# PolyU-IOR/HPR-LP-C

Hardware: AMD Instinct MI355X
Metric: HPR iterations/sec (FP64) (higher is better)
Workload: dtype f64

## Files before the change

### hpr-lp-c_amd/csrc/abi.cpp

```cpp
#include <algorithm>
#include <cmath>
#include <cstdlib>
#include <cstring>
#include <memory>
#include <mutex>
#include <iomanip>
#include <iostream>

#include "hprlp_amd.h"
#include "env.h"
#include "dist.h"
#include "presolve.h"
#include "reorder.h"
#include "solver.h"
#include "version.h"

using namespace hprlp;

struct hprlp_solver {
    Solver s;
    Comm *comm = nullptr;
    Comm *xcomm = nullptr;
    bool sharded = false;
    ~hprlp_solver() {}
// ... 1037 lines not shown
            out[3] = st.clusters; out[4] = st.components; out[5] = st.seconds;
        }
        return 0;
    } catch (const std::exception &e) {
        set_last_error(e.what());
        return -1;
    }
}

extern "C" int hprlp_row_block_plan(int m, int n, const int *rowptr, const int *col, int with_cuts, long out[6]) {
    try {
        if (m <= 0 || n <= 0 || !rowptr || !col || !out) throw std::runtime_error("bad arguments");
        row_block_plan_host(m, n, rowptr, col, with_cuts != 0, out);
        return 0;
    } catch (const std::exception &e) {
        set_last_error(e.what());
        return -1;
    }
}

extern "C" int hprlp_solver_get_scalars(hprlp_solver *h, double out[16]) {
    GUARD_BEGIN
    Solver &s = h->s;
    Ctrl ck;
    HIP_CHECK(hipStreamSynchronize(s.stream));
    HIP_CHECK(hipMemcpy(&ck, s.ctrl.p, sizeof(Ctrl), hipMemcpyDeviceToHost));
    const double v[16] = {s.b_scale, s.c_scale, s.norm_b, s.norm_c, s.norm_b_org, s.norm_c_org, s.sigma, s.lambda_max,
                          s.setup_time, s.scaling_time, s.power_time, static_cast<double>(s.power_iters),
                          static_cast<double>(ck.kx), static_cast<double>(ck.ky), 0, 0};
    for (int i = 0; i < 16; ++i) out[i] = v[i];
    return 0;
    GUARD_END(-1)
}

extern "C" int hprlp_solver_info(hprlp_solver *h, long out[8]) {
    GUARD_BEGIN
    Solver &s = h->s;
    s.finish_tiling();
    out[0] = s.m; out[1] = s.n; out[2] = s.A.view.nnz;
    out[3] = s.A.view.nblk; out[4] = s.AT.view.nblk;
    out[5] = s.A.view.grid(); out[6] = s.AT.view.grid();
    out[7] = (s.A.view.tiled.valid ? 1 : 0) + (s.AT.view.tiled.valid ? 2 : 0) + (s.use_small && !s.comm ? 4 : 0) + (s.perm_r.empty() ? 0 : 8);
    return 0;
    GUARD_END(-1)
}

extern "C" int hprlp_solver_set_detection(hprlp_solver *h, const hprlp_detection *det) {
    GUARD_BEGIN
    if (!h) throw std::runtime_error("null solver");
    if (h->sharded && det)
        throw std::runtime_error("hprlp_solver_set_detection: infeasibility detection runs on one GPU only; a sharded solver "
                                 "(hprlp_solver_create_dist* / _local*) refuses it");
    Detection d;
    detection_from(det, &d);
    h->s.detect = d;
    return 0;
    GUARD_END(-1)
}

extern "C" int hprlp_solver_set_start(hprlp_solver *h, const double *x0, const double *y0) {
    GUARD_BEGIN
    if (!h) throw std::runtime_error("null solver");
    if (h->sharded)
        throw std::runtime_error("hprlp_solver_set_start: warm start runs on one GPU only; a sharded solver (hprlp_solver_create_dist* / "
                                 "_local*) refuses it");
    check_start(x0, h->s.n, "x0");
    check_start(y0, h->s.m, "y0");
    h->s.set_start(x0, y0);
    return 0;
    GUARD_END(-1)
}

extern "C" int hprlp_solver_set_data(hprlp_solver *h, const double *c, const double *obj_constant, const double *AL, const double *AU,
                                     const double *l, const double *u) {
    GUARD_BEGIN
    if (!h) throw std::runtime_error("null solver");
    if (h->sharded)
        throw std::runtime_error("hprlp_solver_set_data: new data for a resident model runs on one GPU only; a sharded solver "
                                 "(hprlp_solver_create_dist* / _local*) refuses it");
    h->s.set_data(c, obj_constant, AL, AU, l, u);
    return 0;
    GUARD_END(-1)
}

extern "C" int hprlp_solver_resolve(hprlp_solver *h, double sigma, const double *x0, const double *y0, HPRLP_results *out,
                                    hprlp_trace_row *trace, int max_trace, int *n_trace) {
    GUARD_BEGIN
    if (!h || !out) throw std::runtime_error("null solver / result");
    if (h->sharded)
        throw std::runtime_error("hprlp_solver_resolve: a re-solve runs on one GPU only; a sharded solver (hprlp_solver_create_dist* / "
                                 "_local*) refuses it");
    if (std::isnan(sigma)) throw std::runtime_error("hprlp_solver_resolve: sigma is NaN");
    check_start(x0, h->s.n, "x0");
    check_start(y0, h->s.m, "y0");
    Solver &s = h->s;
    s.trace = reinterpret_cast<TraceRow *>(trace);
    s.trace_cap = trace ? max_trace : 0;
    try {
        s.resolve(sigma, x0, y0, out);
    } catch (...) {
        s.trace = nullptr;
        s.trace_cap = 0;
        throw;
    }
    if (n_trace) *n_trace = s.trace_n;
    s.trace = nullptr;
    s.trace_cap = 0;
    return 0;
    GUARD_END(-1)
}

extern "C" int hprlp_solver_data_seconds(hprlp_solver *h, double out[3]) {
    GUARD_BEGIN
    if (!h || !out) throw std::runtime_error("null solver / output");
    for (int i = 0; i < 3; ++i) out[i] = h->s.data_time[i];
    return 0;
    GUARD_END(-1)
}

extern "C" int hprlp_solver_get_certificate(hprlp_solver *h, hprlp_certificate *cert) {
    GUARD_BEGIN
    if (!h || !cert) throw std::runtime_error("null solver / certificate");
    if (!export_certificate(h->s.cert, cert, h->s.m, h->s.n)) throw std::runtime_error("host allocation of the certificate failed");
    return 0;
    GUARD_END(-1)
}

extern "C" int hprlp_solver_describe(hprlp_solver *h, char *buf, int cap) {
    GUARD_BEGIN
    if (!h || !buf || cap <= 0) throw std::runtime_error("null solver / buffer");
    Solver &s = h->s;
    s.finish_tiling();
    auto one = [](const char *name, const DeviceMatrix &M) {
        const TiledDev &t = M.view.tiled;
        std::string d = std::string(name) + ": ";
        if (!t.valid) {
            d += "stream kernel (k_spmv_fused, " + std::to_string(M.view.nblk) + " row blocks, " + std::to_string(M.view.nlong) + " split rows)";
            d += no_tiled_note(M.outcome.why);
            return d;
        }
        d += t.n_pieces > 0 ? "tiled, piece form (k_tiled_part + k_tiled_finish, " + std::to_string(t.n_pieces) + " pieces)"
             : t.rem_cap == kPbRemCap ? "tiled, all-remainder form (k_pb_fused, grid " + std::to_string(t.grid) + ")"
                                      : "tiled, fused (k_tiled_fused, grid " + std::to_string(t.grid) + ")";
        d += ", " + std::to_string(t.nsb) + " super-blocks, " + std::to_string(M.tiled.n_steps) + " steps";
        if (t.R != kTileRows || t.T != kTileCols) d += " (" + std::to_string(t.R) + " rows, tiles of " + std::to_string(t.T) + " columns)";
        const double all = static_cast<double>(M.tiled.dense_entries) + static_cast<double>(M.tiled.n_rem);
        if (all > 0) d += ", " + std::to_string(static_cast<int>(100.0 * M.tiled.dense_entries / all + 0.5)) + " % of the entries in staged tiles";
        if (t.f_rk) d += ", source-side run tables";
        if (t.f_work) d += ", pre-pass work list of " + std::to_string(t.n_work) + " workgroups for " + std::to_string(t.n_groups) + " source groups";
        if (t.side_nblk > 0) d += ", long rows aside (" + std::to_string(t.side_nblk) + " blocks through the stream kernel)";
        return d;
    };
    std::string d = one("A", s.A) + "; " + one("A^T", s.AT);
    if (s.use_small && !s.comm) d += "; normal iterations in the single-workgroup kernel (k_small_iterations)";
    if (!s.perm_r.empty()) d += "; locality ordering applied at set-up";
    if (!s.env_at_setup.empty()) d += "; switches: " + s.env_at_setup;
    if (!s.env_ignored_at_setup.empty()) d += "; ignored without HPRLP_TEST_HOOKS=1: " + s.env_ignored_at_setup;
    std::snprintf(buf, static_cast<size_t>(cap), "%s", d.c_str());
    return static_cast<int>(d.size());
    GUARD_END(-1)
}

extern "C" int hprlp_form_select(const hprlp_form_facts *facts, const hprlp_form_hooks *hooks, hprlp_form_decision *out) {
    try {
        if (!facts || !out) throw std::runtime_error("bad arguments");
        const char *missing = "";
        if (!form_select(*facts, hooks ? *hooks : FormHooks(), out, &missing))
            throw std::runtime_error(std::string("the rules ask for a fact that the record marks as not measured: ") + missing);
        return 0;
    } catch (const std::exception &e) {
        set_last_error(e.what());
        return -1;
    }
}

extern "C" int hprlp_solver_form_facts(hprlp_solver *h, int which, hprlp_form_facts out[2]) {
    GUARD_BEGIN
    if (!h || !out || which < 0 || which > 1) throw std::runtime_error("null solver / buffer, or no such matrix");
    h->s.finish_tiling();
    const DeviceMatrix &M = which ? h->s.AT : h->s.A;
    out[0] = M.facts;
    out[1] = M.facts_pb;
    return M.passes;
    GUARD_END(-1)
}

extern "C" int hprlp_tiled_host_check(int m, int n, const int *rowptr, const int *col, int R, int T, double min_dense, long out[6]) {
    try {
        if (m <= 0 || n <= 0 || !rowptr || !col || !out) throw std::runtime_error("bad arguments");
        tiled_host_check(m, n, rowptr, col, R, T, min_dense, out);
        return 0;
    } catch (const std::exception &e) {
        set_last_error(e.what());
        return -1;
    }
}

extern "C" int hprlp_env_switches(char *buf, int cap) {
    int count = 0;
    const EnvEntry *t = env_table(&count);
    std::string d;
    for (int i = 0; i < count; ++i) d += std::string(t[i].name) + "\t" + (t[i].kind == EnvKind::Integrator ? "integrator" : "hook") + "\t" + t[i].what + "\n";
    if (buf && cap > 0) std::snprintf(buf, static_cast<size_t>(cap), "%s", d.c_str());
    return static_cast<int>(d.size());
}

extern "C" int hprlp_solver_time_iterations(hprlp_solver *h, int warmup, int steps, int mode, double *total_ms,
                                            double *xhalf_ms, double *yhalf_ms) {
    GUARD_BEGIN
    Solver &s = h->s;
    if (steps <= 0) throw std::runtime_error("steps must be positive");
    s.run_normal(warmup);
    HIP_CHECK(hipStreamSynchronize(s.stream));
    hipEvent_t e0, e1;
    HIP_CHECK(hipEventCreate(&e0));
    HIP_CHECK(hipEventCreate(&e1));
    double tx = 0, ty = 0;
    float ms = 0;
    if (mode == 0) {
        HIP_CHECK(hipEventRecord(e0, s.stream));
        s.run_normal(steps);
        HIP_CHECK(hipEventRecord(e1, s.stream));
        HIP_CHECK(hipEventSynchronize(e1));
        HIP_CHECK(hipEventElapsedTime(&ms, e0, e1));
    } else if (mode == 2) {
        s.invalidate_far();
        std::vector<hipEvent_t> ev(static_cast<size_t>(steps) * 3);
        for (auto &e : ev) HIP_CHECK(hipEventCreate(&e));
        HIP_CHECK(hipEventRecord(e0, s.stream));
        for (int i = 0; i < steps; ++i) {
            HIP_CHECK(hipEventRecord(ev[3 * i], s.stream));
            launch_spmv_plain(s.AT.view, s.gy.p, s.sn1.p, nullptr, false, nullptr, 0, s.stream);
            HIP_CHECK(hipEventRecord(ev[3 * i + 1], s.stream));
            launch_spmv_plain(s.A.view, s.gxh.p, s.sm1.p, nullptr, false, nullptr, 0, s.stream);
            HIP_CHECK(hipEventRecord(ev[3 * i + 2], s.stream));
        }
        HIP_CHECK(hipEventRecord(e1, s.stream));
        HIP_CHECK(hipEventSynchronize(e1));
        HIP_CHECK(hipEventElapsedTime(&ms, e0, e1));
        for (int i = 0; i < steps; ++i) {
            float a = 0, b = 0;
            HIP_CHECK(hipEventElapsedTime(&a, ev[3 * i], ev[3 * i + 1]));
            HIP_CHECK(hipEventElapsedTime(&b, ev[3 * i + 1], ev[3 * i + 2]));
            tx += a;
            ty += b;
        }
        for (auto &e : ev) (void)hipEventDestroy(e);
    } else {
        std::vector<hipEvent_t> ev(static_cast<size_t>(steps) * 3);
        for (auto &e : ev) HIP_CHECK(hipEventCreate(&e));
        HIP_CHECK(hipEventRecord(e0, s.stream));
        for (int i = 0; i < steps; ++i) s.launch_normal_pair(i + 1 < steps, &ev[3 * static_cast<size_t>(i)], s.x_mode_of(i, steps));
        HIP_CHECK(hipEventRecord(e1, s.stream));
        HIP_CHECK(hipEventSynchronize(e1));
        HIP_CHECK(hipEventElapsedTime(&ms, e0, e1));
        for (int i = 0; i < steps; ++i) {
            float a = 0, b = 0;
            HIP_CHECK(hipEventElapsedTime(&a, ev[3 * i], ev[3 * i + 1]));
            HIP_CHECK(hipEventElapsedTime(&b, ev[3 * i + 1], ev[3 * i + 2]));
            tx += a;
            ty += b;
        }
        for (auto &e : ev) (void)hipEventDestroy(e);
    }
    (void)hipEventDestroy(e0);
    (void)hipEventDestroy(e1);
    if (total_ms) *total_ms = ms;
    if (xhalf_ms) *xhalf_ms = tx;
    if (yhalf_ms) *yhalf_ms = ty;
    return 0;
    GUARD_END(-1)
}
```

### hpr-lp-c_amd/csrc/env.cpp

```cpp
#include "env.h"

#include <cstdlib>
#include <cstring>
#include <stdexcept>

namespace hprlp {

static const EnvEntry kTable[] = {
    {"HPRLP_TEST_HOOKS", EnvKind::Integrator, "1: honour the test hooks below (tests/conftest.py and the tools/ scripts set it)"},
    {"HPRLP_TIMING", EnvKind::Integrator, "wall time of the set-up and solve phases on stderr"},
    {"HPRLP_NO_GRAPH", EnvKind::Integrator, "launch normal iterations eagerly instead of replaying hipGraphs (fall-back)"},
    {"HPRLP_NO_TILED", EnvKind::Integrator, "never build the column-tiled matrix copies: stream kernel everywhere (fall-back)"},
    {"HPRLP_NO_REORDER", EnvKind::Integrator, "no set-up time locality ordering of a large matrix"},
    {"HPRLP_NO_ALLOC_CACHE", EnvKind::Integrator, "do not keep freed device blocks for the next solver of the process"},
    {"HPRLP_DIST_TRANSPORT", EnvKind::Integrator, "shm: hprlp_dist_unique_id names a shared-memory segment (host-staged group of processes on one node) instead of RCCL ids"},
    {"HPRLP_NO_WARM_MODEL", EnvKind::Integrator, "the model constructors do NOT start the HIP runtime / device context / code objects (for a process that forks workers after building its models: a HIP context does not survive fork); the first solve pays for them as in the reference"},
    {"HPRLP_DIST_EXCHANGE", EnvKind::Hook, "sparse | allgather: force the multi-GPU exchange form (same value on every rank)"},
    {"HPRLP_NO_OVERLAP", EnvKind::Integrator, "multi-GPU: shards unsplit, exchange in line on the solver stream"},
    {"HPRLP_DIST_TIMEOUT_S", EnvKind::Integrator, "seconds a rank of the shared-memory transport waits for its peers before it fails (default 120)"},
    {"HPRLP_BATCH_CHUNK", EnvKind::Hook, "solve_batched with 64 or more problems: chunk width of the panels (default 64; narrower chunks map one chunk to each XCD -- measured slower, profiles/r03_tiled_decomposition.md section 6b)"},
    {"HPRLP_BATCH_GRID", EnvKind::Hook, "solve_batched: cap on the row blocks of the normal half-step kernels (read at every call; a small cap makes every workgroup's row loop wrap)"},
    {"HPRLP_BATCH_LAMBDA", EnvKind::Hook, "solve_batched: the batch's lambda_max from the caller (strtod; hand it over as a C99 hex float to keep every bit) instead of 1.01 x the power iteration's estimate (read at every call)"},
    {"HPRLP_COPY_PAUSE_US", EnvKind::Hook, "piece size and pause of the threaded copies of set-up (64 MB, 100 us)"},
    {"HPRLP_COPY_PIECE_MB", EnvKind::Hook, "piece size and pause of the threaded copies of set-up (64 MB, 100 us)"},
    {"HPRLP_DEVICE_TRANSPOSE_MIN", EnvKind::Hook, "build Aᵀ on the host / nonzero threshold of the device transpose (default 4 M)"},
    {"HPRLP_DIST_SELFTEST_FAIL", EnvKind::Hook, "tests only: the set-up self-test of the neighbour exchange reports a failure once (exercises the fall-back to the all-gather)"},
    {"HPRLP_DTON_MAX", EnvKind::Hook, "presolve: cap of the doubleton stage"},
    {"HPRLP_DTON_TRACE", EnvKind::Hook, "presolve: trace the doubleton stage on stderr"},
    {"HPRLP_GEN_FAR", EnvKind::Hook, "benchmark generator: share of a row's entries that fall anywhere (default 0.05)"},
    {"HPRLP_HOST_POWER_START", EnvKind::Hook, "power iteration's start vector made on the host also above 1e6 rows (default there: on the device)"},
    {"HPRLP_HOST_TILING", EnvKind::Hook, "build the tiled copies with the host builder (background threads, default min(16, cores)) instead of on the device"},
    {"HPRLP_HOST_TRANSPOSE", EnvKind::Hook, "build Aᵀ on the host / nonzero threshold of the device transpose (default 4 M)"},
    {"HPRLP_NO_BOUND_CODES", EnvKind::Hook, "the x-half always reads l[j] and u[j], the y-half AL[i] and AU[i] (default: one code byte per column / row says which of them is not a constant; an equality row reads one value)"},
    {"HPRLP_NO_FAR_PUSH", EnvKind::Hook, "always run the remainder pre-pass (k_far_products) instead of the hand-off from the producing half-step's epilogue"},
    {"HPRLP_NO_FAR_WORK", EnvKind::Hook, "the remainder pre-pass with one workgroup per source group also where one group holds several times the mean (default: a work list cuts heavy groups into chunks, tiled.h f_work)"},
    {"HPRLP_NO_PB_LONG_ROWS", EnvKind::Hook, "a matrix kept off the tiled forms for its long rows keeps the stream kernel also where its columns are not popular (default: all-remainder form, Solver::pb_fallback_wanted)"},
    {"HPRLP_NO_FUSED_NORMS", EnvKind::Hook, "the Ruiz row norms by their own passes instead of as a by-product of the preceding scaling pass (same bits)"},
    {"HPRLP_NO_LONG_SIDE", EnvKind::Hook, "a matrix with rows over 1024 entries keeps the stream kernel instead of being tiled with those rows kept aside"},
    {"HPRLP_NO_PB_FALLBACK", EnvKind::Hook, "unstructured large matrices keep the stream kernel instead of the tiled form without dense-tile requirement"},
    {"HPRLP_NO_PB_KERNEL", EnvKind::Hook, "run an all-remainder copy through k_tiled_fused's remainder steps instead of k_pb_fused (A/B)"},
    {"HPRLP_NO_REM2", EnvKind::Hook, "tiled build: no second remainder level"},
    {"HPRLP_NO_SETUP_OVERLAP", EnvKind::Hook, "set-up of a large model in line: no helper threads / copy streams for the value upload, the row blocks, A^T's row pointers and the model vectors (same bits either way)"},
    {"HPRLP_NO_SLAB_CUTS", EnvKind::Hook, "dense rows of a large matrix are not cut at the XCD eighths of the gathered vector (stream kernel)"},
    {"HPRLP_NO_SMALL", EnvKind::Hook, "do not use the single-workgroup kernel for Netlib-scale LPs"},
    {"HPRLP_NO_SMALL_POWER", EnvKind::Hook, "Netlib-scale LPs: power iteration by the regular kernels with the host test every 10th iteration (default: one launch of the single-workgroup kernel)"},
    {"HPRLP_NO_TILED_CR", EnvKind::Hook, "Curtis-Reid passes through the stream kernel also for matrices with a tiled copy (default: tiled kernel on a second value array of -log|a|)"},
    {"HPRLP_NT", EnvKind::Hook, "force default / nontemporal loads of the matrix in the stream kernel"},
    {"HPRLP_OVERLAP_COMM_FIRST", EnvKind::Hook, "tests only: with the in-process rank group, use RCCL's launch order (exchange enqueued before the local SpMV)"},
    {"HPRLP_PB_MIN_COLS", EnvKind::Hook, "gathered-vector length from which an unstructured matrix takes the all-remainder form (default 800 k columns, the crossover measured with k_pb_fused)"},
    {"HPRLP_PB_MIN_NNZ", EnvKind::Hook, "fewest entries for the all-remainder form"},
    {"HPRLP_PB_STAMPS", EnvKind::Hook, "developer build -DHPRLP_PB_PHASE_STAMPS=1: print k_pb_fused's phase times"},
    {"HPRLP_PIECES_ANYWAY", EnvKind::Hook, "attempt the tiled form although neighbouring rows gather from the same lines (<= 0.25 lines per entry) / keep the piece form although an XCD's rows gather from under 3 MB"},
    {"HPRLP_PRESOLVE_MAX_LINKS", EnvKind::Hook, "run one presolve stage alone / cut the chain after n links (tests, debugging)"},
    {"HPRLP_PRESOLVE_OFF", EnvKind::Hook, "switch presolve reductions / stages off (any subset; diagnostics)"},
    {"HPRLP_PRESOLVE_ONLY", EnvKind::Hook, "run one presolve stage alone / cut the chain after n links (tests, debugging)"},
    {"HPRLP_REORDER_CLUSTER", EnvKind::Hook, "knobs of the HOST reference path of the ordering (hprlp_locality_ordering): nodes per cluster, refinement sweeps, trimming percentage"},
    {"HPRLP_REORDER_HOST", EnvKind::Hook, "run the clustering of the locality ordering on the host (the reference form; default: on the device)"},
    {"HPRLP_REORDER_SWEEPS", EnvKind::Hook, "knobs of the HOST reference path of the ordering (hprlp_locality_ordering): nodes per cluster, refinement sweeps, trimming percentage"},
    {"HPRLP_REORDER_TRIM", EnvKind::Hook, "knobs of the HOST reference path of the ordering (hprlp_locality_ordering): nodes per cluster, refinement sweeps, trimming percentage"},
    {"HPRLP_SLACK_PIVOT", EnvKind::Hook, "pivot threshold of the costed slack-column substitution (default 0.5 of the row's largest entry)"},
    {"HPRLP_STORE_X", EnvKind::Hook, "every normal x-half reads and stores x (default for matrices with a tiled copy: inside a run of normal iterations x is rebuilt from x_hat and last_x by the next launch instead of travelling through memory)"},
    {"HPRLP_STREAM_NNZ", EnvKind::Hook, "row-block shape of the stream kernel (≤ 64 rows, ≤ 512 nonzeros per wave)"},
    {"HPRLP_STREAM_ROWS", EnvKind::Hook, "row-block shape of the stream kernel (≤ 64 rows, ≤ 512 nonzeros per wave)"},
    {"HPRLP_TILED_ANYWAY", EnvKind::Hook, "attempt the tiled form although neighbouring rows gather from the same lines (<= 0.25 lines per entry) / keep the piece form although an XCD's rows gather from under 3 MB"},
    {"HPRLP_TILED_MIN_COLS", EnvKind::Hook, "fewest columns for the tiled form (default 800 k, 2^19 for lowered super-blocks; 0 when HPRLP_TILED_MIN_ROWS is given)"},
    {"HPRLP_TILED_MIN_DENSE", EnvKind::Hook, "thresholds of the tiled copy (default 32·8192 rows, 0.5 of the entries in staged tiles)"},
    {"HPRLP_TILED_MIN_ROWS", EnvKind::Hook, "thresholds of the tiled copy (default 32·8192 rows, 0.5 of the entries in staged tiles)"},
    {"HPRLP_TILE_COLS", EnvKind::Hook, "force the tile width / super-block height of the tiled copies (default: Solver::choose_sb_rows)"},
    {"HPRLP_TILE_PIECES", EnvKind::Hook, "piece count of the tiled kernel's piece form (default: the chip's workgroup slots when the matrix has at most that many super-blocks; 0 = off)"},
    {"HPRLP_TILE_ROT", EnvKind::Hook, "alignment period of the rotated tile sweeps (default: mean window width of the matrix; 0 = ascending sweeps, i.e. CSR summation order)"},
    {"HPRLP_TILE_ROWS", EnvKind::Hook, "force the tile width / super-block height of the tiled copies (default: Solver::choose_sb_rows)"},
    {"HPRLP_TILE_STAMPS", EnvKind::Hook, "diagnostic instantiation of the piece kernel: shader-clock time per phase of a step on stderr when the solver is destroyed"},
    {"HPRLP_TILE_THREADS", EnvKind::Hook, "build the tiled copies with the host builder (background threads, default min(16, cores)) instead of on the device"},
    {"HPRLP_TILING_CHECK", EnvKind::Hook, "build them with both builders and fail on the first differing array element"},
    {"HPRLP_WG_TIMES", EnvKind::Hook, "diagnostic: per-workgroup wall-clock stamps of the fused tiled kernel on stderr"},
    {"HPRLP_WG_TIMES_DUMP", EnvKind::Hook, "per-workgroup stamps of the normal half-step kernels only, with the CU each ran on; raw table for tools/wgtimes_analyze.py"},
};

const EnvEntry *env_table(int *count) {
    if (count) *count = static_cast<int>(sizeof(kTable) / sizeof(kTable[0]));
    return kTable;
}

static bool hooks_on() {
    const char *h = std::getenv("HPRLP_TEST_HOOKS");
    return h && h[0] == '1';
}

const char *env_get(const char *name) {
    for (const EnvEntry &e : kTable) {
        if (std::strcmp(e.name, name) != 0) continue;
        if (e.kind == EnvKind::Hook && !hooks_on()) return nullptr;
        return std::getenv(name);
    }
    throw std::logic_error(std::string("environment switch missing from env.cpp's table: ") + name);
}

std::string env_in_effect(std::string *ignored_out) {
    std::string on, off;
    const bool hooks = hooks_on();
    for (const EnvEntry &e : kTable) {
        const char *v = std::getenv(e.name);
        if (!v || std::strcmp(e.name, "HPRLP_TEST_HOOKS") == 0) continue;
        std::string &dst = (e.kind == EnvKind::Hook && !hooks) ? off : on;
        if (!dst.empty()) dst += ' ';
        dst += std::string(e.name) + "=" + v;
    }
    if (ignored_out) *ignored_out = off;
    return on;
}

}
```

### hpr-lp-c_amd/csrc/kernels.h

```cpp
#pragma once

#include <hip/hip_runtime.h>

#include "tiled.h"

namespace hprlp {

constexpr int kWave = 64;
constexpr int kWavesPerBlock = 4;
constexpr int kThreads = kWave * kWavesPerBlock;
constexpr int kStreamW = 512;
constexpr int kStreamRows = 64;
constexpr int kLongRow = 64;
constexpr int kSplitRow = 4096;
constexpr int kNumScalars = 32;

enum Slot : int {
    S_CX = 0,
    S_YOBJ_Y = 1,
    S_XZ = 2,
    S_RD2 = 3,
    S_RP2 = 4,
    S_ADX_DY = 5,
    S_DY2 = 6,
    S_DX2 = 7,
    S_MOVE_X2 = 8,
    S_MOVE_Y2 = 9,
    S_LU2 = 10,
    S_PW_ZZ = 11,
    S_PW_QZ = 12,
    S_PW_ERR2 = 13,
    S_NB2 = 14,
    S_NC2 = 15,
    S_TMP0 = 16,
    S_TMP1 = 17,
    S_SMALL_PW_LAMBDA = 18,
    S_SMALL_PW_ITERS = 19,
    S_RAY_DY = 20,
    S_RAY_CD = 21,
    S_RAY_VY = 22,
    S_RAY_WD = 23,
    S_RAY_YN = 24,
    S_RAY_DN = 25,
    S_RAY_DZ = 26,
    S_RAY_VZ = 27,
    S_RAY_WQ = 28,
    S_DATA_B_ORG = 20,
    S_DATA_C_ORG = 21,
    S_DATA_B_PRE = 22,
    S_DATA_C_PRE = 23,
    S_DATA_NB = 24,
    S_DATA_NC = 25,
};

struct CsrDev {
    int rows = 0, cols = 0;
    int nnz = 0;
    int nt = 1;
    const int *rowptr = nullptr;
    const int *col = nullptr;
    double *val = nullptr;
    const int4 *blk = nullptr;
    int nblk = 0;
    TiledDev tiled;
    const int4 *longrows = nullptr;
    int nlong = 0;
    double *long_partial = nullptr;
    int csr_grid() const { return (nblk + kWavesPerBlock - 1) / kWavesPerBlock; }
    int finish_grid() const { return (nlong + kThreads - 1) / kThreads; }
    int tiled_finish_grid() const { return (rows + kThreads - 1) / kThreads; }
    int grid() const { return tiled.valid ? (tiled.n_pieces > 0 ? tiled_finish_grid() : tiled.grid) : csr_grid() + finish_grid(); }
};

struct Ctrl {
    double sigma, lam_sigma, inv_lam_sigma, inv_sigma;
    int kx, ky;
    int pad0, pad1;
};

struct FarPush {
    const int *gptr = nullptr;
    const double *val = nullptr;
    const int *pos = nullptr;
    const uint16_t *lcol = nullptr;
    double *P = nullptr;
    const int *rptr = nullptr, *rk = nullptr, *rp = nullptr;
};

struct XHalfArgs {
    const double *y_full;
    double *x, *x_hat;
    const double *l, *u, *c, *last_x;
    double *x_bar, *z_bar, *x_temp;
    Ctrl *ctrl;
    double *partials;
    int stride;
    FarPush push;
    bool far_ready = false;
    const unsigned char *lu_code = nullptr;
    int x_mode = 0;
};
constexpr int kXRebuild = 1, kXNoStore = 2;
constexpr unsigned kLoadL = 1u, kLoadU = 2u, kZeroL = 4u;
void launch_bound_codes(int n, const double *l, const double *u, unsigned char *code, hipStream_t s);

struct YHalfArgs {
    const double *xhat_full;
    double *y;
    const double *AL, *AU, *last_y;
    double *y_bar, *y_obj, *y_temp;
    Ctrl *ctrl;
    double *partials;
    int stride;
    FarPush push;
    bool far_ready = false;
    const unsigned char *row_code = nullptr;
};
constexpr unsigned kLoadLo = 1u, kLoadHi = 2u, kRowEq = 4u;
void launch_row_codes(int m, const double *AL, const double *AU, unsigned char *code, hipStream_t s);

struct FinalizeItem {
    const double *partials;
    int count;
    int slot;
    int max = 0;
};
struct FinalizeArgs {
    FinalizeItem item[8];
    int n;
};

bool launch_x_half(const CsrDev &AT, const XHalfArgs &a, bool check, hipStream_t s);
bool launch_y_half(const CsrDev &A, const YHalfArgs &a, bool check, hipStream_t s);
FarPush far_push_of(const CsrDev &consumer);
void launch_x_half_base(const CsrDev &AT_remote, const XHalfArgs &a, const double *base, hipStream_t s);
void launch_y_half_base(const CsrDev &A_remote, const YHalfArgs &a, const double *base, hipStream_t s);

void launch_resid_d(const CsrDev &AT, const double *ybar_full, const double *c, const double *z_bar,
                    const double *col_norm, double *partials, hipStream_t s);
void launch_resid_p(const CsrDev &A, const double *xbar_full, const double *xtemp_full, const double *AL,
                    const double *AU, const double *row_norm, const double *y_temp, bool with_gap,
                    double *partials, int stride, hipStream_t s);
void launch_gap(const CsrDev &A, const double *xtemp_full, const double *y_temp, double *partials, hipStream_t s);
bool launch_spmv_push(const CsrDev &M, const double *v_full, double *out, const FarPush &push, hipStream_t s);
void launch_spmv_plain(const CsrDev &M, const double *v_full, double *out, const double *q, bool with_dots,
                       double *partials, int stride, hipStream_t s, bool far_ready = false);

void launch_finalize(const FinalizeArgs &f, double *scalars, hipStream_t s);

constexpr int kRayFormAccs = 6;
struct RayFormArgs {
    int n, m;
    const double *x_bar, *y_bar;
    double *prev_x, *prev_y, *ds, *ys;
    const double *l, *u, *c, *col_norm, *AL, *AU, *row_norm;
    double b_scale, c_scale;
};
void launch_ray_form(const RayFormArgs &a, double *partials, int nblocks, hipStream_t s);
void launch_ray_col(const CsrDev &AT, const double *ys_full, const double *l, const double *u, const double *col_norm, double b_scale,
                    double c_scale, double *partials, hipStream_t s);
void launch_ray_row(const CsrDev &A, const double *ds_full, const double *AL, const double *AU, const double *row_norm, double b_scale,
                    double *partials, hipStream_t s);

struct StartInArgs {
    int n, m;
    const double *x0, *y0;
    const int *pc, *pr;
    const double *l, *u, *col_norm, *AL, *AU, *row_norm;
    double b_scale, c_scale;
    double *x, *last_x, *x_hat, *x_bar, *y, *last_y, *y_bar;
};
void launch_start_in(const StartInArgs &a, hipStream_t s);
void launch_start_col(const CsrDev &AT, const double *ybar_full, const double *c, const double *l, const double *u,
                      const double *x_bar, double *z_bar, double *partials, hipStream_t s);
void launch_start_row(const CsrDev &A, const double *xbar_full, const double *AL, const double *AU, const double *y_bar,
                      double *y_obj, double *partials, hipStream_t s);

void launch_movement(int n, int m, const double *x_bar, const double *last_x, double *x_temp, const double *y_bar,
                     const double *last_y, double *y_temp, double *partials, int stride, int nblocks, hipStream_t s);
void launch_restart_copy(int n, int m, const double *x_bar, double *x, double *last_x, const double *y_bar,
                         double *y, double *last_y, Ctrl *ctrl, hipStream_t s);
void launch_lu(int n, const double *x_bar, const double *l, const double *u, const double *col_norm, double *x_temp,
               double *partials, int nblocks, hipStream_t s);
void launch_set_ctrl(Ctrl *ctrl, double sigma, double lambda_max, int reset_k, hipStream_t s);

void launch_cr_log_update(const CsrDev &M, const double *other_full, double *result, hipStream_t s, const double *tval_log = nullptr,
                          const double *fval_log = nullptr);
bool cr_runs_tiled(const CsrDev &M);
void launch_exp_clamp(double *v, int n, hipStream_t s);
void launch_row_norm(const CsrDev &M, double *result, int norm, hipStream_t s);
double launch_line_density(const int *rowptr, const int *col, int rows, hipStream_t s);
int launch_longest_row(const int *rowptr, int rows, hipStream_t s, int limit = 0, long *entries_in_long = nullptr);
int launch_heaviest_block(const int *rowptr, int rows, int height, hipStream_t s);
void launch_scale_matrix(const CsrDev &M, const double *rowvec, const double *colvec_full, bool row_first,
                         bool divide, hipStream_t s, double *next_max_norm = nullptr);
void launch_vec_scale(double *x, const double *s, int n, bool divide, hipStream_t s_);
void launch_vec_scal(double *x, double a, int n, hipStream_t s);
void launch_fill(double *x, double a, int n, hipStream_t s);
void launch_bnorm2(const double *AL, const double *AU, int m, double *partials, int nblocks, hipStream_t s);
void launch_norm2(const double *x, int n, double *partials, int nblocks, hipStream_t s);

void launch_check_columns(long nnz, int cols, const int *col, int *bad, hipStream_t s);
void launch_pw_start(int m, unsigned long long seed, long long offset, double *z, hipStream_t s);
void launch_pw_normalize(const double *z, double *q, int m, const double *scalars, hipStream_t s);
void launch_pw_err(const double *z, const double *q, int m, const double *scalars, double *partials, int nblocks,
                   hipStream_t s);

struct DataInArgs {
    int m, nc, nb;
    const double *AL_in, *AU_in, *c_in, *l_in, *u_in;
    const int *pc, *pr;
    const double *row_norm, *col_norm;
    double *AL, *AU, *c, *l, *u;
    double *partials;
    int stride;
};
void launch_data_in(const DataInArgs &a, hipStream_t s);
struct DataBcArgs {
    int m, nc, nb;
    int use_bc;
    const double *scalars;
    double *AL, *AU, *c, *l, *u;
    unsigned char *row_code, *lu_code;
    double *partials;
    int stride;
};
void launch_data_bc(const DataBcArgs &a, hipStream_t s);

void launch_unscale(int n, int m, const double *x_bar, const double *y_bar, const double *z_bar,
                    const double *col_norm, const double *row_norm, double b_scale, double c_scale, double *xo,
                    double *yo, double *zo, hipStream_t s);

constexpr int kSmallMaxK = 12;
constexpr int kSmallMaxR = 2;
constexpr int kSmallMaxRow = 256;
struct SmallArgs {
    int m, n, nnz;
    const int *A_rowptr, *AT_rowptr;
    const double *AT_val;
    const int *ent_ij;
    const int *ent_posA;
    const int *order_x, *order_y;
    double *x, *x_hat, *y;
    const double *l, *u, *c, *last_x, *AL, *AU, *last_y;
    Ctrl *ctrl;
};
bool small_path_fits(int m, int n, long nnz, int max_row_A, int max_row_AT);
void launch_small_iterations(const SmallArgs &a, int count, hipStream_t s);
void launch_small_power(const SmallArgs &a, const double *z0, int max_iter, double tol, double *out, hipStream_t s);

void device_transpose(int rows, int cols, long nnz, const int *rowptr, const int *col, const double *val, int *trp,
                      int *tci, double *tv, hipStream_t s);

void device_split_columns(int rows, long nnz, const int *rowptr, const int *col, const double *val, int lo, int hi, DBuf<int> &rp_loc,
                          DBuf<int> &col_loc, DBuf<double> &val_loc, DBuf<int> &rp_rem, DBuf<int> &col_rem, DBuf<double> &val_rem,
                          hipStream_t s);

void launch_pack(const double *src, const int *idx, double *dst, int n, hipStream_t s);
void launch_scatter(double *dst, const int *idx, const double *src, int n, hipStream_t s);

constexpr int kReduceBlocks = 512;

}
```

### hpr-lp-c_amd/csrc/kernels.hip

```cpp
#include "kernels.h"

#include <algorithm>
#include <vector>
#include <cmath>
#include <type_traits>

namespace hprlp {

__device__ __forceinline__ double wave_sum(double v) {
#pragma unroll
    for (int off = 32; off > 0; off >>= 1) v += __shfl_xor(v, off, kWave);
    return v;
}

__device__ __forceinline__ double wave_max(double v) {
#pragma unroll
    for (int off = 32; off > 0; off >>= 1) v = fmax(v, __shfl_xor(v, off, kWave));
    return v;
}

template <int NACC, int NW, int NMAX = 0>
__device__ __forceinline__ void block_store_partials_in(double (&acc)[NACC], double *partials, int stride, double (*red)[NACC > 0 ? NACC : 1]) {
    const int wave = threadIdx.x >> 6, lane = threadIdx.x & 63;
#pragma unroll
// ... 442 lines not shown
            const int el = tid + k * NT;
            if (el < cnt) prod[el] = pv[k];
        }
        uint32_t code[K];
        {
            const int shift = K * tid - min(K * tid, max(cnt - K, 0));
#pragma unroll
            for (int u = 0; u < K; ++u) code[u] = cv[u];
            if (shift > 0 && shift < K) {
#pragma unroll
                for (int u = 0; u < K; ++u) {
                    uint32_t c = 0;
#pragma unroll
                    for (int q = 0; q < K; ++q) c = (q == u + shift) ? cv[q] : c;
                    code[u] = c;
                }
            }
        }
        if (s + 1 < s1) issue(nxt);
        lds_barrier();
        const int nv = min(max(cnt - K * tid, 0), K);
        uint32_t row[K];
        double pr[K];
#pragma unroll
        for (int u = 0; u < K; ++u) {
            const bool ok = u < nv;
            row[u] = ok ? (code[u] & 0xffffu) : (u == 0 ? NOROW : row[u - 1]);
            pr[u] = ok ? prod[code[u] >> 16] : 0.0;
        }
        double run = pr[0], head = 0.0;
        bool single = true;
#pragma unroll
        for (int u = 1; u < K; ++u) {
            if (row[u] != row[u - 1]) {
                if (single) {
                    head = run;
                    single = false;
                } else {
                    acc[row[u - 1]] += run;
                }
                run = pr[u];
            } else {
                run += pr[u];
            }
        }
        const uint32_t rf = row[0], rl = row[K - 1];
        const uint32_t rl_prev = __shfl_up(rl, 1, 64);
        const bool open_in = lane > 0 && rf == rl_prev && rf != NOROW;
        double v = run;
        int f = (single && open_in) ? 0 : 1;
#pragma unroll
        for (int off = 1; off < 64; off <<= 1) {
            const double vu = __shfl_up(v, off, 64);
            const int fu = __shfl_up(f, off, 64);
            if (lane >= off && !f) {
                v += vu;
                f |= fu;
            }
        }
        const double v_prev = __shfl_up(v, 1, 64);
        const double carry = open_in ? v_prev : 0.0;
        const int next_open = __shfl_down(static_cast<int>(open_in), 1, 64);
        if (!single) acc[rf] += carry + head;
        const double tail = single ? carry + run : run;
        if (lane == 63) {
            bnd_row[wave] = rl;
            bnd_val[wave] = tail;
        } else if (!next_open && rl != NOROW) {
            acc[rl] += tail;
        }
        lds_barrier();
        if (tid < NW) {
            const uint32_t rw = bnd_row[tid];
            bool last_one = rw != NOROW;
            double tot = 0.0;
#pragma unroll
            for (int w = 0; w < NW; ++w) {
                const bool same = bnd_row[w] == rw;
                if (w <= tid && same) tot += bnd_val[w];
                if (w > tid && same) last_one = false;
            }
            if (last_one) acc[rw] += tot;
        }
        st = nxt;
    }
}

template <class Epi, bool PUSH>
__device__ __forceinline__ void epilogue_rows(const Epi &epi, double *acc, double (&racc)[Epi::NACC > 0 ? Epi::NACC : 1], int r0, int nr, int tid) {
    constexpr int NT = kTileThreads, B = 4;
    for (int i0 = tid; i0 < nr; i0 += B * NT) {
        typename Epi::Row rw[B];
        double sv[B][1];
#pragma unroll
        for (int u = 0; u < B; ++u) {
            const int i = min(i0 + u * NT, nr - 1);
            rw[u] = epi.load_row(r0 + i);
            sv[u][0] = acc[i];
        }
#pragma unroll
        for (int u = 0; u < B; ++u) {
            const int i = i0 + u * NT;
            if (i < nr) {
                if constexpr (PUSH) acc[i] = epi.apply(r0 + i, rw[u], sv[u], racc);
                else epi.apply(r0 + i, rw[u], sv[u], racc);
            }
        }
    }
}

__device__ __forceinline__ void push_products(const FarPush &f, const double *vals, int pb, int pe, int tid) {
    constexpr int NT = kTileThreads, U = 4;
    if (pb >= pe) return;
    double a4[U];
    int p4[U];
    uint16_t c4[U];
    auto load_batch = [&](int k0) {
#pragma unroll
        for (int u = 0; u < U; ++u) {
            const int z = min(k0 + u * NT, pe - 1);
            a4[u] = __builtin_nontemporal_load(f.val + z);
            p4[u] = __builtin_nontemporal_load(f.pos + z);
            c4[u] = __builtin_nontemporal_load(f.lcol + z);
        }
    };
    int k = pb + tid;
    load_batch(k);
    for (; k < pe; k += U * NT) {
        double prd[U];
        int ps[U];
#pragma unroll
        for (int u = 0; u < U; ++u) {
            prd[u] = a4[u] * vals[c4[u]];
            ps[u] = p4[u];
        }
        const int kn = k + U * NT;
        if (kn < pe) load_batch(kn);
#pragma unroll
        for (int u = 0; u < U; ++u)
            if (k + u * NT < pe) f.P[ps[u]] = prd[u];
    }
}

__device__ __forceinline__ int run_position(const int *tab_k, const int *tab_p, int nr, int k) {
    int lo = 0, hi = nr - 1;
    while (lo < hi) {
        const int mid = (lo + hi + 1) >> 1;
        if (tab_k[mid] <= k) lo = mid;
        else hi = mid - 1;
    }
    return tab_p[lo] + (k - tab_k[lo]);
}

__device__ __forceinline__ void push_products_runs(const FarPush &f, const double *vals, int *tab, int g, int pb, int pe, int tid) {
    constexpr int NT = kTileThreads, U = 4;
    if (pb >= pe) return;
    const int r0 = f.rptr[g], nr = f.rptr[g + 1] - r0;
    int *tab_k = tab, *tab_p = tab + kPbRunTabCap;
    double a4[U];
    uint16_t c4[U];
    auto load_batch = [&](int k0) {
#pragma unroll
        for (int u = 0; u < U; ++u) {
            const int z = min(k0 + u * NT, pe - 1);
            a4[u] = __builtin_nontemporal_load(f.val + z);
            c4[u] = __builtin_nontemporal_load(f.lcol + z);
        }
    };
    int k = pb + tid;
    load_batch(k);
    for (int i = tid; i < nr; i += NT) {
        tab_k[i] = f.rk[r0 + i];
        tab_p[i] = f.rp[r0 + i];
    }
    lds_barrier();
    int ps[U];
#pragma unroll
    for (int u = 0; u < U; ++u) ps[u] = run_position(tab_k, tab_p, nr, min(k + u * NT, pe - 1));
    for (; k < pe; k += U * NT) {
        double prd[U];
        int pc[U];
#pragma unroll
        for (int u = 0; u < U; ++u) {
            prd[u] = a4[u] * vals[c4[u]];
            pc[u] = ps[u];
        }
        const int kn = k + U * NT;
        if (kn < pe) load_batch(kn);
#pragma unroll
        for (int u = 0; u < U; ++u)
            if (k + u * NT < pe) f.P[pc[u]] = prd[u];
        if (kn < pe) {
#pragma unroll
            for (int u = 0; u < U; ++u) ps[u] = run_position(tab_k, tab_p, nr, min(kn + u * NT, pe - 1));
        }
    }
}

template <class Epi, bool REP, bool PUSH = false, bool NARROW = false>
__global__ void __launch_bounds__(kTileThreads, 4) k_tiled_fused(CsrDev A, Epi epi) {
    static_assert(Epi::NV == 1, "the tiled kernel stages one gathered vector");
    constexpr int NT = kTileThreads, RMAX = kTileRows, T = kTileCols;
    constexpr int NACC = Epi::NACC;
    __shared__ double acc[RMAX];
    __shared__ __attribute__((aligned(16))) double ytile[T];
    const TiledDev &t = A.tiled;
    const int tid = threadIdx.x;
    const int R = t.R;
    const int per = t.per, slots = gridDim.x / 8;
    const int slot = blockIdx.x / 8;
    double racc[NACC > 0 ? NACC : 1];
#pragma unroll
    for (int i = 0; i < (NACC > 0 ? NACC : 1); ++i) racc[i] = 0.0;
    epi.begin();
    int wg_round = 0;
    const bool wg_stamp = t.wgtimes && tid == 0 && (t.wg_filter == 0 || (PUSH && NACC == 0));
    if (wg_stamp) t.wgtimes[blockIdx.x * 8] = wall_clock64();
    for (int q = slot; q < per; q += slots) {
        const int sb = (blockIdx.x % 8) * per + q;
        if (sb >= t.nsb) break;
        const double *__restrict__ vec = epi.gv[0];
        lds_barrier();
        const int ncols = A.cols;
        for (int i = tid; i < R; i += NT) acc[i] = 0.0;
        const int s0 = t.sb_ptr[sb], smid = t.sb_mid[sb], s1 = t.sb_ptr[sb + 1];
        if (s0 < smid) tiled_sweep<HPRLP_SWEEP_ED, HPRLP_SWEEP_TD, REP, false, LogTerm<Epi>::value, NARROW ? kTileColsNarrow : kTileCols>(t, s0, smid - s0, t.steps[s0].rot, smid - s0, vec, ncols, acc, ytile, tid);
        remainder_steps<kTileRemK>(t, smid, s1, acc, ytile, ytile + kTileRemCap, tid);
        lds_barrier();
        const int r0 = sb * R;
        const int nr = min(R, A.rows - r0);
        int pb = 0, pe = 0;
        if constexpr (PUSH) {
            pb = epi.push.gptr[sb];
            pe = epi.push.gptr[sb + 1];
        }
        epilogue_rows<Epi, PUSH>(epi, acc, racc, r0, nr, tid);
        if constexpr (PUSH) {
            lds_barrier();
            push_products(epi.push, acc, pb, pe, tid);
        }
        if (wg_stamp && ++wg_round <= 5) t.wgtimes[blockIdx.x * 8 + wg_round] = wall_clock64();
    }
    if (wg_stamp) {
        t.wgtimes[blockIdx.x * 8 + 7] = wall_clock64();
        const unsigned hw = __builtin_amdgcn_s_getreg((31 << 11) | 4), xcc = __builtin_amdgcn_s_getreg((31 << 11) | 20);
        t.wgtimes[blockIdx.x * 8 + 6] = (static_cast<unsigned long long>(xcc & 0xfu) << 32) | hw;
    }
    if constexpr (NACC > 0) {
        __syncthreads();
        block_store_partials_in<NACC, kTileThreads / kWave, MaxAccs<Epi>::value>(racc, epi.partials, epi.stride, reinterpret_cast<double(*)[NACC]>(ytile));
    }
}

template <class Epi, bool PUSH = false>
__global__ void __launch_bounds__(kTileThreads, 4) k_pb_fused(CsrDev A, Epi epi) {
    static_assert(Epi::NV == 1, "one gathered vector");
    constexpr int NT = kTileThreads, K = kPbRemK, CAP = kPbRemCap, NW = kTileThreads / 64;
    constexpr int NACC = Epi::NACC;
    __shared__ double acc[kPbRowsMax];
    __shared__ __attribute__((aligned(16))) double prod[CAP];
    __shared__ double bnd[3 * NW];
    const TiledDev &t = A.tiled;
    const int tid = threadIdx.x;
    const int R = t.R;
    const int per = t.per, slots = gridDim.x / 8;
    const int slot = blockIdx.x / 8;
    double racc[NACC > 0 ? NACC : 1];
#pragma unroll
    for (int i = 0; i < (NACC > 0 ? NACC : 1); ++i) racc[i] = 0.0;
    epi.begin();
#if HPRLP_PB_PHASE_STAMPS
    unsigned long long ph[8] = {0, 0, 0, 0, 0, 0, 0, 0}, tq = wall_clock64(), tk0 = tq;
#define PB_STAMP(i) do { const unsigned long long now_ = wall_clock64(); ph[i] += now_ - tq; tq = now_; } while (0)
#else
#define PB_STAMP(i) do { } while (0)
#endif
    for (int q = slot; q < per; q += slots) {
        const int sb = (blockIdx.x % 8) * per + q;
        if (sb >= t.nsb) break;
        lds_barrier();
        for (int i = tid; i < R; i += NT) acc[i] = 0.0;
        const int smid = t.sb_mid[sb], s1 = t.sb_ptr[sb + 1];
        remainder_steps<K>(t, smid, s1, acc, prod, bnd, tid);
        lds_barrier();
        PB_STAMP(4);
        const int r0 = sb * R;
        const int nr = min(R, A.rows - r0);
        int pb = 0, pe = 0;
        if constexpr (PUSH) {
            pb = epi.push.gptr[sb];
            pe = epi.push.gptr[sb + 1];
        }
        epilogue_rows<Epi, PUSH>(epi, acc, racc, r0, nr, tid);
        PB_STAMP(5);
        if constexpr (PUSH) {
            lds_barrier();
            if (epi.push.rk) push_products_runs(epi.push, acc, reinterpret_cast<int *>(prod), sb, pb, pe, tid);
            else push_products(epi.push, acc, pb, pe, tid);
        }
        PB_STAMP(6);
    }
#if HPRLP_PB_PHASE_STAMPS
    if (t.wgtimes && tid == 0 && PUSH && NACC == 0) {
        ph[7] = wall_clock64() - tk0;
        for (int i = 0; i < 8; ++i) t.wgtimes[blockIdx.x * 8 + i] = ph[i];
    }
#endif
#undef PB_STAMP
    if constexpr (NACC > 0) {
        __syncthreads();
        block_store_partials_in<NACC, kTileThreads / kWave, MaxAccs<Epi>::value>(racc, epi.partials, epi.stride, reinterpret_cast<double(*)[NACC]>(prod));
    }
}

template <bool REP, bool STAMP = false, bool NARROW = false>
__global__ void __launch_bounds__(kTileThreads, 4) k_tiled_part(CsrDev A, const double *__restrict__ vec) {
    constexpr int NT = kTileThreads, RMAX = kTileRows, T = kTileCols;
    __shared__ double acc[RMAX];
    __shared__ __attribute__((aligned(16))) double ytile[T];
    const TiledDev &t = A.tiled;
    const int tid = threadIdx.x;
    const int R = t.R;
    const int per = (t.n_pieces + 7) / 8;
    const int pc = (blockIdx.x % 8) * per + blockIdx.x / 8;
    if (pc >= t.n_pieces) return;
    for (int sg = t.piece_ptr[pc]; sg < t.piece_ptr[pc + 1]; ++sg) {
        const int4 d = t.segs[sg];
        const int sb = d.x;
        lds_barrier();
        for (int i = tid; i < R; i += NT) acc[i] = 0.0;
        const int s0 = t.sb_ptr[sb], smid = t.sb_mid[sb], s1 = t.sb_ptr[sb + 1];
        unsigned long long *st = STAMP ? t.stamps + static_cast<size_t>(pc) * 16 : nullptr;
        unsigned long long c0 = 0, c1 = 0, c2 = 0;
        if (STAMP) c0 = __builtin_amdgcn_s_memtime();
        if (d.z > 0) tiled_sweep<3, 2, REP, STAMP, false, NARROW ? kTileColsNarrow : kTileCols>(t, s0, smid - s0, d.y, d.z, vec, A.cols, acc, ytile, tid, st);
        if (STAMP) c1 = __builtin_amdgcn_s_memtime();
        if (d.w) remainder_steps<kTileRemK>(t, smid, s1, acc, ytile, ytile + kTileRemCap, tid);
        lds_barrier();
        if (STAMP) c2 = __builtin_amdgcn_s_memtime();
        double *out = t.parts + static_cast<size_t>(sg) * R;
        for (int i = tid; i < R; i += NT) out[i] = acc[i];
        if (STAMP && tid == 0) {
            st[8] += c1 - c0;
            st[9] += c2 - c1;
            st[10] += __builtin_amdgcn_s_memtime() - c2;
        }
    }
}

template <class Epi>
__global__ void __launch_bounds__(kThreads) k_tiled_finish(CsrDev A, Epi epi) {
    constexpr int NACC = Epi::NACC;
    const int R = A.tiled.R;
    double racc[NACC > 0 ? NACC : 1];
#pragma unroll
    for (int i = 0; i < (NACC > 0 ? NACC : 1); ++i) racc[i] = 0.0;
    epi.begin();
    const int r = blockIdx.x * kThreads + threadIdx.x;
    if (r < A.rows) {
        const int sb = r / R;
        const int a = A.tiled.slot_ptr[sb], b = A.tiled.slot_ptr[sb + 1];
        const double *p = A.tiled.parts + (r - sb * R);
        double sum = 0.0;
        for (int k = a; k < b; ++k) sum = (k == a) ? p[static_cast<size_t>(k) * R] : sum + p[static_cast<size_t>(k) * R];
        const double sv[1] = {sum};
        typename Epi::Row rw = epi.load_row(r);
        epi.apply(r, rw, sv, racc);
    }
    if constexpr (NACC > 0) block_store_partials<NACC, kWavesPerBlock, MaxAccs<Epi>::value>(racc, epi.partials, epi.stride);
}

__global__ void __launch_bounds__(kThreads) k_tiled_refresh(long n, const int *perm, const double *csr_val, double *out) {
    const long i = static_cast<long>(blockIdx.x) * kThreads + threadIdx.x;
    if (i < n) {
        const int p = perm[i];
        out[i] = p >= 0 ? csr_val[p] : 0.0;
    }
}

void launch_tiled_refresh(const DeviceTiled &t, const double *csr_val, hipStream_t s) {
    if (t.n_tile > 0)
        hipLaunchKernelGGL(k_tiled_refresh, dim3(static_cast<unsigned>((t.n_tile + kThreads - 1) / kThreads)), dim3(kThreads), 0, s,
                           t.n_tile, t.tperm.p, csr_val, t.tval.p);
    if (t.n_rem > 0 && t.f_val.p)
        hipLaunchKernelGGL(k_tiled_refresh, dim3(static_cast<unsigned>((t.n_rem + kThreads - 1) / kThreads)), dim3(kThreads), 0, s,
                           t.n_rem, t.f_perm.p, csr_val, t.f_val.p);
}

__global__ void __launch_bounds__(kThreads) k_tiled_refresh_log(long n, const int *perm, const double *csr_val, double *out) {
    const long i = static_cast<long>(blockIdx.x) * kThreads + threadIdx.x;
    if (i < n) {
        const int p = perm[i];
        out[i] = p >= 0 ? -log(fmax(fabs(csr_val[p]), 1e-300)) : __builtin_nan("");
    }
}

void launch_tiled_refresh_log(const DeviceTiled &t, const double *csr_val, double *tval_log, double *fval_log, hipStream_t s) {
    if (t.n_tile > 0)
        hipLaunchKernelGGL(k_tiled_refresh_log, dim3(static_cast<unsigned>((t.n_tile + kThreads - 1) / kThreads)), dim3(kThreads), 0, s,
                           t.n_tile, t.tperm.p, csr_val, tval_log);
    if (t.n_rem > 0 && t.f_val.p)
        hipLaunchKernelGGL(k_tiled_refresh_log, dim3(static_cast<unsigned>((t.n_rem + kThreads - 1) / kThreads)), dim3(kThreads), 0, s,
                           t.n_rem, t.f_perm.p, csr_val, fval_log);
}

__device__ __forceinline__ bool far_work_item(const TiledDev &t, int &g, int &b, int &e) {
    const int items = t.f_work ? t.n_work : t.n_groups;
    const int per = (items + 7) / 8;
    const int w = (blockIdx.x % 8) * per + blockIdx.x / 8;
    if (w >= items) return false;
    if (t.f_work) {
        const int4 d = t.f_work[w];
        g = d.x; b = d.y; e = d.z;
    } else {
        g = w; b = t.f_gptr[w]; e = t.f_gptr[w + 1];
    }
    return b < e;
}

template <bool LOGTERM = false>
__global__ void __launch_bounds__(kFarThreads) k_far_products(TiledDev t, const double *__restrict__ vec, int ncols) {
    __shared__ double v[kFarGroup];
    const int G = t.G;
    int g, b, e;
    if (!far_work_item(t, g, b, e)) return;
    const int c0 = g * G, tid = threadIdx.x;
    const int w = min(G, ncols - c0);
    constexpr int U = 4;
    double a[U];
    int pos[U];
    uint16_t lc[U];
    int k = b + tid;
    auto load_batch = [&](int k0) {
#pragma unroll
        for (int u = 0; u < U; ++u) {
            const int q = min(k0 + u * kFarThreads, e - 1);
            a[u] = __builtin_nontemporal_load(t.f_val + q);
            pos[u] = __builtin_nontemporal_load(t.f_pos + q);
            lc[u] = __builtin_nontemporal_load(t.f_lcol + q);
        }
    };
    load_batch(k);
    {
        constexpr int S = kFarGroup / kFarThreads;
        double sv[S];
#pragma unroll
        for (int i = 0; i < S; ++i)
            if (i * kFarThreads < G) sv[i] = vec[c0 + min(tid + i * kFarThreads, w - 1)];
#pragma unroll
        for (int i = 0; i < S; ++i)
            if (i * kFarThreads < G) v[tid + i * kFarThreads] = sv[i];
    }
    __syncthreads();
    for (; k < e; k += U * kFarThreads) {
        double pr[U];
        int ps[U];
#pragma unroll
        for (int u = 0; u < U; ++u) {
            pr[u] = LOGTERM ? a[u] - v[lc[u]] : a[u] * v[lc[u]];
            ps[u] = pos[u];
        }
        const int kn = k + U * kFarThreads;
        if (kn < e) load_batch(kn);
#pragma unroll
        for (int u = 0; u < U; ++u)
            if (k + u * kFarThreads < e) t.P[ps[u]] = pr[u];
    }
}

template <bool LOGTERM = false>
__global__ void __launch_bounds__(kFarThreads) k_far_products_runs(TiledDev t, const double *__restrict__ vec, int ncols) {
    __shared__ double v[kPbRowsMax];
    __shared__ int tab[2 * kPbRunTabCap];
    const int G = t.G;
    int g, b, e;
    if (!far_work_item(t, g, b, e)) return;
    const int c0 = g * G, tid = threadIdx.x;
    const int w = min(G, ncols - c0);
    const int r0 = t.f_rptr[g], nr = t.f_rptr[g + 1] - r0;
    int *tab_k = tab, *tab_p = tab + kPbRunTabCap;
    constexpr int U = 4;
    double a[U];
    uint16_t lc[U];
    int k = b + tid;
    auto load_batch = [&](int k0) {
#pragma unroll
        for (int u = 0; u < U; ++u) {
            const int q = min(k0 + u * kFarThreads, e - 1);
            a[u] = __builtin_nontemporal_load(t.f_val + q);
            lc[u] = __builtin_nontemporal_load(t.f_lcol + q);
        }
    };
    load_batch(k);
    for (int i = tid; i < G; i += kFarThreads) v[i] = vec[c0 + min(i, w - 1)];
    for (int i = tid; i < nr; i += kFarThreads) {
        tab_k[i] = t.f_rk[r0 + i];
        tab_p[i] = t.f_rp[r0 + i];
    }
    __syncthreads();
    int ps[U];
#pragma unroll
    for (int u = 0; u < U; ++u) ps[u] = run_position(tab_k, tab_p, nr, min(k + u * kFarThreads, e - 1));
    for (; k < e; k += U * kFarThreads) {
        double pr[U];
        int pc[U];
#pragma unroll
        for (int u = 0; u < U; ++u) {
            pr[u] = LOGTERM ? a[u] - v[lc[u]] : a[u] * v[lc[u]];
            pc[u] = ps[u];
        }
        const int kn = k + U * kFarThreads;
        if (kn < e) load_batch(kn);
#pragma unroll
        for (int u = 0; u < U; ++u)
            if (k + u * kFarThreads < e) t.P[pc[u]] = pr[u];
        if (kn < e) {
#pragma unroll
            for (int u = 0; u < U; ++u) ps[u] = run_position(tab_k, tab_p, nr, min(kn + u * kFarThreads, e - 1));
        }
    }
}

template <bool LOGTERM>
static void launch_far_products(const TiledDev &t, const double *vec, int ncols, hipStream_t s) {
    const dim3 grid(((t.f_work ? t.n_work : t.n_groups) + 7) / 8 * 8);
    if (t.f_rk && t.G <= kPbRowsMax) hipLaunchKernelGGL(k_far_products_runs<LOGTERM>, grid, dim3(kFarThreads), 0, s, t, vec, ncols);
    else hipLaunchKernelGGL(k_far_products<LOGTERM>, grid, dim3(kFarThreads), 0, s, t, vec, ncols);
}


template <bool CHECK, bool STREAMED = false>
struct XEpi {
    static constexpr int NV = 1;
    static constexpr int NACC = CHECK ? 3 : 0;
    const double *gv[1];
    double *x, *x_hat;
    const double *l, *u, *c, *last_x;
    double *x_bar, *z_bar, *x_temp;
    Ctrl *ctrl;
    double *partials;
    int stride;
    double sigma, f1, f2;
    FarPush push;
    const unsigned char *lu_code;
    int x_mode;
    double f1p, f2p;
    static constexpr bool kPublishes = true;
    static constexpr bool kSkipsX = !CHECK && STREAMED;
    struct Row {
        double xi, ci, li, ui, lx;
    };
    __device__ __forceinline__ void begin() {
        const int k = ctrl->kx;
        sigma = ctrl->sigma;
        f1 = 1.0 / (static_cast<double>(k) + 2.0);
        f2 = 1.0 - f1;
        f1p = 1.0 / (static_cast<double>(k - 1) + 2.0);
        f2p = 1.0 - f1p;
        if (blockIdx.x == 0 && threadIdx.x == 0) ctrl->ky = k;
    }
    __device__ __forceinline__ Row load_row(int r) const {
        constexpr bool NT = STREAMED && HPRLP_EPI_NT >= 1;
        auto ld = [](const double *p) { return NT ? __builtin_nontemporal_load(p) : *p; };
        double li, ui;
        if (lu_code) {
            const unsigned cd = NT ? __builtin_nontemporal_load(lu_code + r) : lu_code[r];
            li = (cd & kLoadL) ? ld(l + r) : ((cd & kZeroL) ? 0.0 : -__builtin_huge_val());
            ui = (cd & kLoadU) ? ld(u + r) : __builtin_huge_val();
        } else {
            li = ld(l + r);
            ui = ld(u + r);
        }
        const double lx = ld(last_x + r);
        if constexpr (kSkipsX) {
            if (x_mode & kXRebuild) return Row{f2p * ld(x_hat + r) + f1p * lx, ld(c + r), li, ui, lx};
        }
        return Row{ld(x + r), ld(c + r), li, ui, lx};
    }
    __device__ __forceinline__ double apply(int r, const Row &w, const double (&s)[1], double (&acc)[CHECK ? 3 : 1]) const {
        const double gc = s[0] - w.ci;
        const double zt = w.xi + sigma * gc;
        const double xb = fmin(w.ui, fmax(w.li, zt));
        const double xh = 2.0 * xb - w.xi;
        const double xn = f2 * xh + f1 * w.lx;
        {
            if constexpr (STREAMED && HPRLP_EPI_NT >= 2) __builtin_nontemporal_store(xh, x_hat + r);
            else x_hat[r] = xh;
            if (!kSkipsX || !(x_mode & kXNoStore)) {
                if constexpr (STREAMED && HPRLP_EPI_NT >= 1) __builtin_nontemporal_store(xn, x + r);
                else x[r] = xn;
            }
        }
        if constexpr (CHECK) {
            const double zb = (xb - zt) / sigma;
            const double dx = xb - xh;
            z_bar[r] = zb;
            x_bar[r] = xb;
            x_temp[r] = dx;
            acc[0] += w.ci * xb;
            acc[1] += xb * zb;
            acc[2] += dx * dx;
        }
        return xh;
    }
};

template <bool CHECK, bool STREAMED = false>
struct YEpi {
    static constexpr int NV = 1;
    static constexpr int NACC = CHECK ? 2 : 0;
    const double *gv[1];
    double *y;
    const double *AL, *AU, *last_y;
    double *y_bar, *y_obj, *y_temp;
    Ctrl *ctrl;
    double *partials;
    int stride;
    double fact1, fact2, hf1, hf2;
    FarPush push;
    const unsigned char *row_code;
    static constexpr bool kPublishes = true;
    struct Row {
        double yi, lo, hi, ly;
    };
    __device__ __forceinline__ void begin() {
        const int k = ctrl->ky;
        fact1 = ctrl->lam_sigma;
        fact2 = ctrl->inv_lam_sigma;
        hf1 = 1.0 / (static_cast<double>(k) + 2.0);
        hf2 = 1.0 - hf1;
        if (blockIdx.x == 0 && threadIdx.x == 0) ctrl->kx = k + 1;
    }
    __device__ __forceinline__ Row load_row(int r) const {
        constexpr bool NT = STREAMED && HPRLP_EPI_NT >= 1;
        auto ld = [](const double *p) { return NT ? __builtin_nontemporal_load(p) : *p; };
        double lo, hi;
        if (row_code) {
            const unsigned cd = NT ? __builtin_nontemporal_load(row_code + r) : row_code[r];
            hi = (cd & kLoadHi) ? ld(AU + r) : __builtin_huge_val();
            lo = (cd & kLoadLo) ? ld(AL + r) : ((cd & kRowEq) ? hi : -__builtin_huge_val());
        } else {
            lo = ld(AL + r);
            hi = ld(AU + r);
        }
        return Row{ld(y + r), lo, hi, ld(last_y + r)};
    }
    __device__ __forceinline__ double apply(int r, const Row &w, const double (&s)[1], double (&acc)[CHECK ? 2 : 1]) const {
        const double v = s[0] - fact1 * w.yi;
        const double d = fmax(w.lo - v, fmin(w.hi - v, 0.0));
        const double yb = fact2 * d;
        const double yh = 2.0 * yb - w.yi;
        const double yn = hf2 * yh + hf1 * w.ly;
        if constexpr (STREAMED && HPRLP_EPI_NT >= 2) __builtin_nontemporal_store(yn, y + r);
        else y[r] = yn;
        if constexpr (CHECK) {
            const double dy = yb - yh;
            const double yo = v + d;
            y_temp[r] = dy;
            y_bar[r] = yb;
            y_obj[r] = yo;
            acc[0] += yo * yb;
            acc[1] += dy * dy;
        }
        return yn;
    }
};

struct RdEpi {
    static constexpr int NV = 1;
    static constexpr int NACC = 1;
    const double *gv[1];
    const double *c, *z_bar, *col_norm;
    double *partials;
    int stride;
    struct Row {
        double ci, zi, cn;
    };
    __device__ __forceinline__ void begin() {}
    __device__ __forceinline__ Row load_row(int r) const { return Row{c[r], z_bar[r], col_norm[r]}; }
    __device__ __forceinline__ void apply(int, const Row &w, const double (&s)[1], double (&acc)[1]) const {
        const double rd = (w.ci - s[0] - w.zi) * w.cn;
        acc[0] += rd * rd;
    }
};

template <bool GAP>
struct RpEpi {
    static constexpr int NV = GAP ? 2 : 1;
    static constexpr int NACC = GAP ? 2 : 1;
    const double *gv[GAP ? 2 : 1];
    const double *AL, *AU, *row_norm, *y_temp;
    double *partials;
    int stride;
    struct Row {
        double lo, hi, rn, dy;
    };
    __device__ __forceinline__ void begin() {}
    __device__ __forceinline__ Row load_row(int r) const {
        return Row{AL[r], AU[r], row_norm[r], GAP ? y_temp[r] : 0.0};
    }
    __device__ __forceinline__ void apply(int, const Row &w, const double (&s)[GAP ? 2 : 1],
                                          double (&acc)[GAP ? 2 : 1]) const {
        const double v = s[0];
        const double rp = fmax(fmin(w.hi - v, 0.0), w.lo - v) * w.rn;
        acc[0] += rp * rp;
        if constexpr (GAP) acc[1] += s[1] * w.dy;
    }
};

struct GapEpi {
    static constexpr int NV = 1;
    static constexpr int NACC = 1;
    const double *gv[1];
    const double *y_temp;
    double *partials;
    int stride;
    struct Row {
        double dy;
    };
    __device__ __forceinline__ void begin() {}
    __device__ __forceinline__ Row load_row(int r) const { return Row{y_temp[r]}; }
// ... 106 lines not shown
        const double z = ((d > 0.0 && isfinite(w.lo)) || (d < 0.0 && isfinite(w.hi))) ? d : 0.0;
        z_bar[r] = z;
        acc[0] += w.ci * w.xb;
        acc[1] += (z > 0.0 ? w.lo : (z < 0.0 ? w.hi : 0.0)) * z;
    }
};

struct StartRowEpi {
    static constexpr int NV = 1;
    static constexpr int NACC = 1;
    const double *gv[1];
    const double *AL, *AU, *y_bar;
    double *y_obj;
    double *partials;
    int stride;
    struct Row {
        double lo, hi, yb;
    };
    __device__ __forceinline__ void begin() {}
    __device__ __forceinline__ Row load_row(int r) const { return Row{AL[r], AU[r], y_bar[r]}; }
    __device__ __forceinline__ void apply(int r, const Row &w, const double (&s)[1], double (&acc)[1]) const {
        const double yo = w.yb > 0.0 ? w.lo : (w.yb < 0.0 ? w.hi : fmin(fmax(s[0], w.lo), w.hi));
        y_obj[r] = yo;
        acc[0] += yo * w.yb;
    }
};

template <class Epi>
__global__ void __launch_bounds__(kThreads) k_long_finish(CsrDev A, Epi epi, int main_grid) {
    constexpr int NV = Epi::NV;
    constexpr int NACC = Epi::NACC;
    double acc[NACC > 0 ? NACC : 1];
#pragma unroll
    for (int i = 0; i < (NACC > 0 ? NACC : 1); ++i) acc[i] = 0.0;
    epi.begin();
    const int i = blockIdx.x * kThreads + threadIdx.x;
    if (i < A.nlong) {
        const int4 d = A.longrows[i];
        double s[NV];
#pragma unroll
        for (int v = 0; v < NV; ++v) s[v] = 0.0;
        for (int c = d.y; c < d.z; ++c) {
#pragma unroll
            for (int v = 0; v < NV; ++v) s[v] += A.long_partial[static_cast<size_t>(c) * 2 + v];
        }
        typename Epi::Row rw = epi.load_row(d.x);
        epi.apply(d.x, rw, s, acc);
    }
    if constexpr (NACC > 0) {
        block_store_partials<NACC, kWavesPerBlock, MaxAccs<Epi>::value>(acc, epi.partials + main_grid, epi.stride);
    }
}

template <class Epi, class = void>
struct Publishes : std::false_type {};
template <class Epi>
struct Publishes<Epi, std::void_t<decltype(Epi::kPublishes)>> : std::true_type {};

template <class Epi>
struct WithBase : Epi {
    const double *base;
    struct Row {
        typename Epi::Row w;
        double b;
    };
    __device__ __forceinline__ Row load_row(int r) const { return Row{Epi::load_row(r), base[r]}; }
    __device__ __forceinline__ auto apply(int r, const Row &w, const double (&s)[1], double (&acc)[Epi::NACC > 0 ? Epi::NACC : 1]) const {
        const double t[1] = {w.b + s[0]};
        return Epi::apply(r, w.w, t, acc);
    }
};

struct SideEpi {
    static constexpr int NV = 1;
    static constexpr int NACC = 0;
    const double *gv[1];
    const int *rows;
    double *base;
    struct Row {};
    __device__ __forceinline__ void begin() {}
    __device__ __forceinline__ Row load_row(int) const { return Row{}; }
    __device__ __forceinline__ void apply(int r, const Row &, const double (&s)[1], double (&)[1]) const { base[rows[r]] = s[0]; }
};

template <class Epi>
static bool launch_tiled(const CsrDev &M, const Epi &e, hipStream_t s, bool far_ready);

template <class Epi>
static bool launch_fused(const CsrDev &M, const Epi &e, hipStream_t s, bool far_ready = false) {
    if (M.nblk <= 0) return false;
    if constexpr (Epi::NV == 1) {
        if (M.tiled.valid) {
            if (M.tiled.side_nblk > 0) {
                CsrDev S = M;
                S.tiled.valid = false;
                S.blk = M.tiled.side_blk;
                S.nblk = M.tiled.side_nblk;
                S.longrows = M.tiled.side_long;
                S.nlong = M.tiled.side_nlong;
                S.long_partial = M.tiled.side_partial;
                SideEpi se{{e.gv[0]}, M.tiled.side_rows, M.tiled.base};
                hipLaunchKernelGGL(k_spmv_fused<SideEpi>, dim3(S.csr_grid()), dim3(kThreads), 0, s, S, se);
                if (S.nlong > 0) hipLaunchKernelGGL(k_long_finish<SideEpi>, dim3(S.finish_grid()), dim3(kThreads), 0, s, S, se, S.csr_grid());
                WithBase<Epi> wb{e, M.tiled.base};
                return launch_tiled(M, wb, s, far_ready);
            }
            return launch_tiled(M, e, s, far_ready);
        }
    }
    hipLaunchKernelGGL(k_spmv_fused<Epi>, dim3(M.csr_grid()), dim3(kThreads), 0, s, M, e);
    if (M.nlong > 0)
        hipLaunchKernelGGL(k_long_finish<Epi>, dim3(M.finish_grid()), dim3(kThreads), 0, s, M, e, M.csr_grid());
    return false;
}

template <class Epi>
static bool launch_tiled(const CsrDev &M, const Epi &e, hipStream_t s, bool far_ready) {
    if (M.tiled.n_groups > 0 && !far_ready)
        launch_far_products<false>(M.tiled, e.gv[0], M.cols, s);
    const bool narrow = M.tiled.T == kTileColsNarrow;
    if (M.tiled.rem_cap == kPbRemCap) {
        if constexpr (Publishes<Epi>::value) {
            if (e.push.gptr) {
                hipLaunchKernelGGL((k_pb_fused<Epi, true>), dim3(M.tiled.grid), dim3(kTileThreads), 0, s, M, e);
                return true;
            }
        }
        hipLaunchKernelGGL((k_pb_fused<Epi, false>), dim3(M.tiled.grid), dim3(kTileThreads), 0, s, M, e);
        return false;
    }
    if (M.tiled.n_pieces > 0) {
        const dim3 grid((M.tiled.n_pieces + 7) / 8 * 8);
        if (narrow) hipLaunchKernelGGL((k_tiled_part<false, false, true>), grid, dim3(kTileThreads), 0, s, M, e.gv[0]);
        else if (M.tiled.stamps) hipLaunchKernelGGL((k_tiled_part<false, true>), grid, dim3(kTileThreads), 0, s, M, e.gv[0]);
        else if (M.tiled.repeats) hipLaunchKernelGGL(k_tiled_part<true>, grid, dim3(kTileThreads), 0, s, M, e.gv[0]);
        else hipLaunchKernelGGL(k_tiled_part<false>, grid, dim3(kTileThreads), 0, s, M, e.gv[0]);
        hipLaunchKernelGGL(k_tiled_finish<Epi>, dim3(M.tiled_finish_grid()), dim3(kThreads), 0, s, M, e);
        return false;
    }
    if constexpr (Publishes<Epi>::value) {
        if (e.push.gptr) {
            if (narrow) hipLaunchKernelGGL((k_tiled_fused<Epi, false, true, true>), dim3(M.tiled.grid), dim3(kTileThreads), 0, s, M, e);
            else if (M.tiled.repeats) hipLaunchKernelGGL((k_tiled_fused<Epi, true, true>), dim3(M.tiled.grid), dim3(kTileThreads), 0, s, M, e);
            else hipLaunchKernelGGL((k_tiled_fused<Epi, false, true>), dim3(M.tiled.grid), dim3(kTileThreads), 0, s, M, e);
            return true;
        }
    }
    if (narrow) hipLaunchKernelGGL((k_tiled_fused<Epi, false, false, true>), dim3(M.tiled.grid), dim3(kTileThreads), 0, s, M, e);
    else if (M.tiled.repeats) hipLaunchKernelGGL((k_tiled_fused<Epi, true>), dim3(M.tiled.grid), dim3(kTileThreads), 0, s, M, e);
    else hipLaunchKernelGGL((k_tiled_fused<Epi, false>), dim3(M.tiled.grid), dim3(kTileThreads), 0, s, M, e);
    return false;
}

FarPush far_push_of(const CsrDev &consumer) {
    FarPush f;
    if (consumer.tiled.valid && consumer.tiled.n_groups > 0) {
        f.gptr = consumer.tiled.f_gptr;
        f.val = consumer.tiled.f_val;
        f.pos = consumer.tiled.f_pos;
        f.lcol = consumer.tiled.f_lcol;
        f.P = consumer.tiled.P;
        if (consumer.tiled.f_rk) {
            f.rptr = consumer.tiled.f_rptr;
            f.rk = consumer.tiled.f_rk;
            f.rp = consumer.tiled.f_rp;
        }
    }
    return f;
}

bool launch_x_half(const CsrDev &AT, const XHalfArgs &a, bool check, hipStream_t s) {
    if (check) {
        XEpi<true> e{{a.y_full}, a.x, a.x_hat, a.l, a.u, a.c, a.last_x, a.x_bar, a.z_bar, a.x_temp, a.ctrl, a.partials, a.stride, 0, 0, 0, a.push, a.lu_code};
        return launch_fused(AT, e, s, a.far_ready);
    }
    if (AT.tiled.valid) {
        XEpi<false, true> e{{a.y_full}, a.x, a.x_hat, a.l, a.u, a.c, a.last_x, nullptr, nullptr, nullptr, a.ctrl, nullptr, 0, 0, 0, 0, a.push, a.lu_code, a.x_mode};
        return launch_fused(AT, e, s, a.far_ready);
    }
    XEpi<false> e{{a.y_full}, a.x, a.x_hat, a.l, a.u, a.c, a.last_x, nullptr, nullptr, nullptr, a.ctrl, nullptr, 0, 0, 0, 0, a.push, a.lu_code};
    return launch_fused(AT, e, s, a.far_ready);
}

bool launch_y_half(const CsrDev &A, const YHalfArgs &a, bool check, hipStream_t s) {
    if (check) {
        YEpi<true> e{{a.xhat_full}, a.y, a.AL, a.AU, a.last_y, a.y_bar, a.y_obj, a.y_temp, a.ctrl, a.partials, a.stride, 0, 0, 0, 0, a.push, a.row_code};
        return launch_fused(A, e, s, a.far_ready);
    }
    if (A.tiled.valid) {
        YEpi<false, true> e{{a.xhat_full}, a.y, a.AL, a.AU, a.last_y, nullptr, nullptr, nullptr, a.ctrl, nullptr, 0, 0, 0, 0, 0, a.push, a.row_code};
        return launch_fused(A, e, s, a.far_ready);
    }
    YEpi<false> e{{a.xhat_full}, a.y, a.AL, a.AU, a.last_y, nullptr, nullptr, nullptr, a.ctrl, nullptr, 0, 0, 0, 0, 0, a.push, a.row_code};
    return launch_fused(A, e, s, a.far_ready);
}


void launch_x_half_base(const CsrDev &AT_remote, const XHalfArgs &a, const double *base, hipStream_t s) {
    WithBase<XEpi<false>> e{{{a.y_full}, a.x, a.x_hat, a.l, a.u, a.c, a.last_x, nullptr, nullptr, nullptr, a.ctrl, nullptr, 0, 0, 0, 0, FarPush{}, a.lu_code}, base};
    launch_fused(AT_remote, e, s);
}

void launch_y_half_base(const CsrDev &A_remote, const YHalfArgs &a, const double *base, hipStream_t s) {
    WithBase<YEpi<false>> e{{{a.xhat_full}, a.y, a.AL, a.AU, a.last_y, nullptr, nullptr, nullptr, a.ctrl, nullptr, 0, 0, 0, 0, 0, FarPush{}}, base};
    launch_fused(A_remote, e, s);
}

void launch_resid_d(const CsrDev &AT, const double *ybar_full, const double *c, const double *z_bar,
                    const double *col_norm, double *partials, hipStream_t s) {
    RdEpi e{{ybar_full}, c, z_bar, col_norm, partials, AT.grid()};
    launch_fused(AT, e, s);
}

void launch_resid_p(const CsrDev &A, const double *xbar_full, const double *xtemp_full, const double *AL,
                    const double *AU, const double *row_norm, const double *y_temp, bool with_gap,
                    double *partials, int stride, hipStream_t s) {
    if (with_gap && A.tiled.valid) {
        RpEpi<false> e{{xbar_full}, AL, AU, row_norm, nullptr, partials, stride};
        launch_fused(A, e, s);
        GapEpi g{{xtemp_full}, y_temp, partials + stride, stride};
        launch_fused(A, g, s);
    } else if (with_gap) {
        RpEpi<true> e{{xbar_full, xtemp_full}, AL, AU, row_norm, y_temp, partials, stride};
        launch_fused(A, e, s);
    } else {
        RpEpi<false> e{{xbar_full}, AL, AU, row_norm, nullptr, partials, stride};
        launch_fused(A, e, s);
    }
}

void launch_gap(const CsrDev &A, const double *xtemp_full, const double *y_temp, double *partials, hipStream_t s) {
    GapEpi e{{xtemp_full}, y_temp, partials, A.grid()};
    launch_fused(A, e, s);
}

bool launch_spmv_push(const CsrDev &M, const double *v_full, double *out, const FarPush &push, hipStream_t s) {
    PlainPushEpi e{{v_full}, out, push};
    return launch_fused(M, e, s);
}

void launch_spmv_plain(const CsrDev &M, const double *v_full, double *out, const double *q, bool with_dots,
                       double *partials, int stride, hipStream_t s, bool far_ready) {
    if (with_dots) {
        PlainEpi<true> e{{v_full}, out, q, partials, stride};
        launch_fused(M, e, s, far_ready);
    } else if (far_ready) {
        PlainEpi<false> e{{v_full}, out, nullptr, nullptr, 0};
        launch_fused(M, e, s, true);
    } else {
        PlainEpi<false> e{{v_full}, out, nullptr, nullptr, 0};
        launch_fused(M, e, s);
    }
}

void launch_ray_col(const CsrDev &AT, const double *ys_full, const double *l, const double *u, const double *col_norm, double b_scale,
                    double c_scale, double *partials, hipStream_t s) {
    RayColEpi e{{ys_full}, l, u, col_norm, b_scale, c_scale, partials, AT.grid()};
    launch_fused(AT, e, s);
}

void launch_ray_row(const CsrDev &A, const double *ds_full, const double *AL, const double *AU, const double *row_norm, double b_scale,
                    double *partials, hipStream_t s) {
    RayRowEpi e{{ds_full}, AL, AU, row_norm, b_scale, partials, A.grid()};
    launch_fused(A, e, s);
}

void launch_start_col(const CsrDev &AT, const double *ybar_full, const double *c, const double *l, const double *u,
                      const double *x_bar, double *z_bar, double *partials, hipStream_t s) {
    StartColEpi e{{ybar_full}, c, l, u, x_bar, z_bar, partials, AT.grid()};
    launch_fused(AT, e, s);
}

void launch_start_row(const CsrDev &A, const double *xbar_full, const double *AL, const double *AU, const double *y_bar,
                      double *y_obj, double *partials, hipStream_t s) {
    StartRowEpi e{{xbar_full}, AL, AU, y_bar, y_obj, partials, A.grid()};
    launch_fused(A, e, s);
}

static_assert(kWavesPerBlock == 4, "k_finalize's sum adds the four waves' partials in a fixed order");
__global__ void __launch_bounds__(kThreads) k_finalize(FinalizeArgs f, double *scalars) {
    const FinalizeItem it = f.item[blockIdx.x];
    __shared__ double red[kWavesPerBlock];
    if (it.max) {
        double v = 0.0;
        for (int i = threadIdx.x; i < it.count; i += kThreads) v = fmax(v, it.partials[i]);
        v = wave_max(v);
        if ((threadIdx.x & 63) == 0) red[threadIdx.x >> 6] = v;
        __syncthreads();
        if (threadIdx.x == 0) {
            double m = red[0];
            for (int w = 1; w < kWavesPerBlock; ++w) m = fmax(m, red[w]);
            scalars[it.slot] = m;
        }
        return;
    }
    double v = 0.0;
    for (int i = threadIdx.x; i < it.count; i += kThreads) v += it.partials[i];
    v = wave_sum(v);
    if ((threadIdx.x & 63) == 0) red[threadIdx.x >> 6] = v;
    __syncthreads();
    if (threadIdx.x == 0) scalars[it.slot] = ((red[0] + red[1]) + red[2]) + red[3];
}

void launch_finalize(const FinalizeArgs &f, double *scalars, hipStream_t s) {
    if (f.n <= 0) return;
    hipLaunchKernelGGL(k_finalize, dim3(f.n), dim3(kThreads), 0, s, f, scalars);
}

__global__ void __launch_bounds__(kThreads) k_movement(int n, int m, const double *x_bar, const double *last_x,
                                                      double *x_temp, const double *y_bar, const double *last_y,
                                                      double *y_temp, double *partials, int stride) {
    double acc[2] = {0.0, 0.0};
    const int tid = blockIdx.x * kThreads + threadIdx.x, nth = gridDim.x * kThreads;
    for (int i = tid; i < n; i += nth) {
        const double d = 1.0 * x_bar[i] + (-1.0) * last_x[i];
        x_temp[i] = d;
        acc[0] += d * d;
    }
    for (int i = tid; i < m; i += nth) {
        const double d = 1.0 * y_bar[i] + (-1.0) * last_y[i];
        y_temp[i] = d;
        acc[1] += d * d;
    }
    block_store_partials<2>(acc, partials, stride);
}

void launch_movement(int n, int m, const double *x_bar, const double *last_x, double *x_temp, const double *y_bar,
                     const double *last_y, double *y_temp, double *partials, int stride, int nblocks, hipStream_t s) {
    hipLaunchKernelGGL(k_movement, dim3(nblocks), dim3(kThreads), 0, s, n, m, x_bar, last_x, x_temp, y_bar, last_y,
                       y_temp, partials, stride);
// ... 425 lines not shown
        const int j = lane + kWave * t;
        if (j < nz) {
            c[t] = __builtin_nontemporal_load(col + j);
            v[t] = __builtin_nontemporal_load(val + j);
        }
    }
    int rs = 0, re = 0;
    if (lane < nr) {
        rs = M.rowptr[r0 + lane] - k0;
        re = M.rowptr[r0 + lane + 1] - k0;
    }
#pragma unroll
    for (int t = 0; t < PER; ++t)
        if (lane + kWave * t < nz) cv[t] = colvec[c[t]];
    if (lane < nr) {
        const double rv = rowvec[r0 + lane];
        for (int j = rs; j < re; ++j) rsv[wave][j] = rv;
    }
    wave_lds_sync();
#pragma unroll
    for (int t = 0; t < PER; ++t) {
        const int j = lane + kWave * t;
        if (j < nz) {
            const double nv = scale_entry<ROW_FIRST, DIVIDE>(v[t], rsv[wave][j], cv[t]);
            __builtin_nontemporal_store(nv, val + j);
            if (NEXT) rsv[wave][j] = fabs(nv);
        }
    }
    if (NEXT) {
        wave_lds_sync();
        if (lane < nr) {
            double acc = 0.0;
            for (int j = rs; j < re; ++j) {
                const double a = rsv[wave][j];
                if (acc < a) acc = a;
            }
            next_norm[r0 + lane] = norm_result(acc);
        }
    }
}

template <bool ROW_FIRST, bool DIVIDE, bool NEXT>
__global__ void __launch_bounds__(kThreads) k_scale_long_rows(CsrDev M, const double *rowvec, const double *colvec, double *next_norm) {
    __shared__ double red[kWavesPerBlock];
    const int r = M.longrows[blockIdx.x].x;
    const double rv = rowvec[r];
    double acc = 0.0;
    for (int k = M.rowptr[r] + threadIdx.x; k < M.rowptr[r + 1]; k += kThreads) {
        const double nv = scale_entry<ROW_FIRST, DIVIDE>(M.val[k], rv, colvec[M.col[k]]);
        M.val[k] = nv;
        if (NEXT && acc < fabs(nv)) acc = fabs(nv);
    }
    if (NEXT) {
#pragma unroll
        for (int off = 32; off > 0; off >>= 1) {
            const double o = __shfl_xor(acc, off);
            if (acc < o) acc = o;
        }
        if ((threadIdx.x & 63) == 0) red[threadIdx.x >> 6] = acc;
        __syncthreads();
        if (threadIdx.x == 0) {
            for (int w = 1; w < kWavesPerBlock; ++w)
                if (acc < red[w]) acc = red[w];
            next_norm[r] = norm_result(acc);
        }
    }
}

template <bool ROW_FIRST, bool DIVIDE, bool NEXT>
static void launch_scale_matrix_t(const CsrDev &M, const double *rowvec, const double *colvec_full, double *next_norm, hipStream_t s) {
    hipLaunchKernelGGL((k_scale_matrix<ROW_FIRST, DIVIDE, NEXT>), dim3(M.csr_grid()), dim3(kThreads), 0, s, M, rowvec, colvec_full, next_norm);
    if (M.nlong > 0)
        hipLaunchKernelGGL((k_scale_long_rows<ROW_FIRST, DIVIDE, NEXT>), dim3(M.nlong), dim3(kThreads), 0, s, M, rowvec, colvec_full, next_norm);
}

void launch_scale_matrix(const CsrDev &M, const double *rowvec, const double *colvec_full, bool row_first,
                         bool divide, hipStream_t s, double *next_max_norm) {
    if (M.rows <= 0 || M.nblk <= 0) return;
    if (next_max_norm) {
        if (row_first && divide) launch_scale_matrix_t<true, true, true>(M, rowvec, colvec_full, next_max_norm, s);
        else if (row_first && !divide) launch_scale_matrix_t<true, false, true>(M, rowvec, colvec_full, next_max_norm, s);
        else if (!row_first && divide) launch_scale_matrix_t<false, true, true>(M, rowvec, colvec_full, next_max_norm, s);
        else launch_scale_matrix_t<false, false, true>(M, rowvec, colvec_full, next_max_norm, s);
        return;
    }
    if (row_first && divide) launch_scale_matrix_t<true, true, false>(M, rowvec, colvec_full, nullptr, s);
    else if (row_first && !divide) launch_scale_matrix_t<true, false, false>(M, rowvec, colvec_full, nullptr, s);
    else if (!row_first && divide) launch_scale_matrix_t<false, true, false>(M, rowvec, colvec_full, nullptr, s);
    else launch_scale_matrix_t<false, false, false>(M, rowvec, colvec_full, nullptr, s);
}

__global__ void __launch_bounds__(kThreads) k_vec_scale(double *x, const double *s, int n, int divide) {
    const int i = blockIdx.x * kThreads + threadIdx.x;
    if (i < n) x[i] = divide ? x[i] / s[i] : x[i] * s[i];
}
void launch_vec_scale(double *x, const double *sv, int n, bool divide, hipStream_t s) {
    if (n <= 0) return;
    hipLaunchKernelGGL(k_vec_scale, dim3((n + kThreads - 1) / kThreads), dim3(kThreads), 0, s, x, sv, n, divide ? 1 : 0);
}

__global__ void __launch_bounds__(kThreads) k_vec_scal(double *x, double a, int n) {
    const int i = blockIdx.x * kThreads + threadIdx.x;
    if (i < n) x[i] = x[i] * a;
}
void launch_vec_scal(double *x, double a, int n, hipStream_t s) {
    if (n <= 0) return;
    hipLaunchKernelGGL(k_vec_scal, dim3((n + kThreads - 1) / kThreads), dim3(kThreads), 0, s, x, a, n);
}

__global__ void __launch_bounds__(kThreads) k_fill(double *x, double a, int n) {
    const int i = blockIdx.x * kThreads + threadIdx.x;
    if (i < n) x[i] = a;
}
void launch_fill(double *x, double a, int n, hipStream_t s) {
    if (n <= 0) return;
    hipLaunchKernelGGL(k_fill, dim3((n + kThreads - 1) / kThreads), dim3(kThreads), 0, s, x, a, n);
}

__global__ void __launch_bounds__(kThreads) k_bnorm2(const double *AL, const double *AU, int m, double *partials) {
    double acc[1] = {0.0};
    const int tid = blockIdx.x * kThreads + threadIdx.x, nth = gridDim.x * kThreads;
    for (int i = tid; i < m; i += nth) {
        double a = AL[i], b = AU[i];
        a = isinf(a) ? 0.0 : a;
        b = isinf(b) ? 0.0 : b;
        const double v = fmax(fabs(a), fabs(b));
        acc[0] += v * v;
    }
    block_store_partials<1>(acc, partials, gridDim.x);
}
void launch_bnorm2(const double *AL, const double *AU, int m, double *partials, int nblocks, hipStream_t s) {
    hipLaunchKernelGGL(k_bnorm2, dim3(nblocks), dim3(kThreads), 0, s, AL, AU, m, partials);
}

__global__ void __launch_bounds__(kThreads) k_norm2(const double *x, int n, double *partials) {
    double acc[1] = {0.0};
    const int tid = blockIdx.x * kThreads + threadIdx.x, nth = gridDim.x * kThreads;
    for (int i = tid; i < n; i += nth) acc[0] += x[i] * x[i];
    block_store_partials<1>(acc, partials, gridDim.x);
}
void launch_norm2(const double *x, int n, double *partials, int nblocks, hipStream_t s) {
    hipLaunchKernelGGL(k_norm2, dim3(nblocks), dim3(kThreads), 0, s, x, n, partials);
}

__global__ void __launch_bounds__(kThreads) k_bound_codes(int n, const double *l, const double *u, unsigned char *code) {
    const int j = blockIdx.x * kThreads + threadIdx.x;
    if (j >= n) return;
    const double lj = l[j], uj = u[j];
    const bool l_zero = __double_as_longlong(lj) == 0, l_minf = lj == -__builtin_huge_val(), u_pinf = uj == __builtin_huge_val();
    code[j] = static_cast<unsigned char>((l_zero || l_minf ? 0u : kLoadL) | (u_pinf ? 0u : kLoadU) | (l_zero ? kZeroL : 0u));
}
void launch_bound_codes(int n, const double *l, const double *u, unsigned char *code, hipStream_t s) {
    if (n > 0) hipLaunchKernelGGL(k_bound_codes, dim3((n + kThreads - 1) / kThreads), dim3(kThreads), 0, s, n, l, u, code);
}

__global__ void __launch_bounds__(kThreads) k_row_codes(int m, const double *AL, const double *AU, unsigned char *code) {
    const int i = blockIdx.x * kThreads + threadIdx.x;
    if (i >= m) return;
    const double lo = AL[i], hi = AU[i];
    const bool lo_minf = lo == -__builtin_huge_val(), hi_pinf = hi == __builtin_huge_val();
    const bool eq = !hi_pinf && __double_as_longlong(lo) == __double_as_longlong(hi);
    code[i] = static_cast<unsigned char>((lo_minf || eq ? 0u : kLoadLo) | (hi_pinf ? 0u : kLoadHi) | (eq ? kRowEq : 0u));
}
void launch_row_codes(int m, const double *AL, const double *AU, unsigned char *code, hipStream_t s) {
    if (m > 0) hipLaunchKernelGGL(k_row_codes, dim3((m + kThreads - 1) / kThreads), dim3(kThreads), 0, s, m, AL, AU, code);
}

__global__ void __launch_bounds__(kThreads) k_check_columns(long nnz, int cols, const int *__restrict__ col, int *bad) {
    const long stride = static_cast<long>(gridDim.x) * kThreads;
    int b = 0;
    for (long k = static_cast<long>(blockIdx.x) * kThreads + threadIdx.x; k < nnz; k += stride) b |= (col[k] < 0 || col[k] >= cols);
    if (b) *bad = 1;
}
void launch_check_columns(long nnz, int cols, const int *col, int *bad, hipStream_t s) {
    if (nnz > 0) hipLaunchKernelGGL(k_check_columns, dim3(static_cast<unsigned>(std::min<long>((nnz + kThreads - 1) / kThreads, 8192))), dim3(kThreads), 0, s, nnz, cols, col, bad);
}

__global__ void __launch_bounds__(kThreads) k_pw_start(int m, unsigned long long seed, long long offset, double *z) {
    const int i = blockIdx.x * kThreads + threadIdx.x;
    if (i >= m) return;
    auto mix = [](unsigned long long x) {
        unsigned long long v = x + 0x9E3779B97F4A7C15ULL;
        v = (v ^ (v >> 30)) * 0xBF58476D1CE4E5B9ULL;
        v = (v ^ (v >> 27)) * 0x94D049BB133111EBULL;
        return v ^ (v >> 31);
    };
    const unsigned long long base = seed * 0x100000001B3ULL, g = static_cast<unsigned long long>(offset + i);
    const unsigned long long h1 = mix(base + 2 * g), h2 = mix(base + 2 * g + 1);
    const double two53 = 1.0 / 9007199254740992.0, twopi = 6.283185307179586476925286766559;
    const double u1 = static_cast<double>((h1 >> 11) + 1) * two53, u2 = static_cast<double>(h2 >> 11) * two53;
    z[i] = sqrt(-2.0 * log(u1)) * cos(twopi * u2) + 1e-8;
}
void launch_pw_start(int m, unsigned long long seed, long long offset, double *z, hipStream_t s) {
    if (m > 0) hipLaunchKernelGGL(k_pw_start, dim3((m + kThreads - 1) / kThreads), dim3(kThreads), 0, s, m, seed, offset, z);
}

__global__ void __launch_bounds__(kThreads) k_pw_normalize(const double *z, double *q, int m, const double *scalars) {
    const double invn = 1.0 / sqrt(scalars[S_PW_ZZ] + 2.220446049250313e-16);
    const int tid = blockIdx.x * kThreads + threadIdx.x, nth = gridDim.x * kThreads;
    for (int i = tid; i < m; i += nth) q[i] = invn * z[i];
}
void launch_pw_normalize(const double *z, double *q, int m, const double *scalars, hipStream_t s) {
    hipLaunchKernelGGL(k_pw_normalize, dim3(vec_grid(m)), dim3(kThreads), 0, s, z, q, m, scalars);
}

__global__ void __launch_bounds__(kThreads) k_pw_err(const double *z, const double *q, int m, const double *scalars,
                                                    double *partials) {
    const double lambda = scalars[S_PW_QZ];
    double acc[1] = {0.0};
    const int tid = blockIdx.x * kThreads + threadIdx.x, nth = gridDim.x * kThreads;
    for (int i = tid; i < m; i += nth) {
        const double d = -lambda * q[i] + 1.0 * z[i];
        acc[0] += d * d;
    }
    block_store_partials<1>(acc, partials, gridDim.x);
}
void launch_pw_err(const double *z, const double *q, int m, const double *scalars, double *partials, int nblocks,
                   hipStream_t s) {
    hipLaunchKernelGGL(k_pw_err, dim3(nblocks), dim3(kThreads), 0, s, z, q, m, scalars, partials);
}

__global__ void __launch_bounds__(kThreads) k_ray_form(RayFormArgs a, double *partials) {
    double acc[kRayFormAccs] = {0.0, 0.0, 0.0, 0.0, 0.0, 0.0};
    const int tid = blockIdx.x * kThreads + threadIdx.x, nth = gridDim.x * kThreads;
    for (int j = tid; j < a.n; j += nth) {
        const double xb = a.x_bar[j];
        const double ds = xb - a.prev_x[j];
        a.prev_x[j] = xb;
        a.ds[j] = ds;
        const double cn = a.col_norm[j];
        const double d = (ds / cn) * a.b_scale;
        acc[1] += ((a.c[j] * cn) * a.c_scale) * d;
        if (isfinite(a.l[j])) acc[3] = fmax(acc[3], -d);
        if (isfinite(a.u[j])) acc[3] = fmax(acc[3], d);
        acc[5] = fmax(acc[5], fabs(d));
    }
    for (int i = tid; i < a.m; i += nth) {
        const double yb = a.y_bar[i];
        const double ys = yb - a.prev_y[i];
        a.prev_y[i] = yb;
        a.ys[i] = ys;
        const double rn = a.row_norm[i];
        const double y = (ys / rn) * a.c_scale;
        if (y > 0.0) {
            const double lo = a.AL[i];
            if (isfinite(lo)) acc[0] += ((lo * rn) * a.b_scale) * y;
            else acc[2] = fmax(acc[2], y);
        } else if (y < 0.0) {
            const double hi = a.AU[i];
            if (isfinite(hi)) acc[0] += ((hi * rn) * a.b_scale) * y;
            else acc[2] = fmax(acc[2], -y);
        }
        acc[4] = fmax(acc[4], fabs(y));
    }
    block_store_partials<kRayFormAccs, kWavesPerBlock, 4>(acc, partials, gridDim.x);
}
void launch_ray_form(const RayFormArgs &a, double *partials, int nblocks, hipStream_t s) {
    hipLaunchKernelGGL(k_ray_form, dim3(nblocks), dim3(kThreads), 0, s, a, partials);
}

__global__ void __launch_bounds__(kThreads) k_start_in(StartInArgs a) {
    const int tid = blockIdx.x * kThreads + threadIdx.x, nth = gridDim.x * kThreads;
    for (int j = tid; j < a.n; j += nth) {
        const double v = a.x0 ? a.x0[a.pc ? a.pc[j] : j] : 0.0;
        const double xs = fmin(fmax((v * a.col_norm[j]) / a.b_scale, a.l[j]), a.u[j]);
        a.x[j] = xs;
        a.last_x[j] = xs;
        a.x_hat[j] = xs;
        a.x_bar[j] = xs;
    }
    for (int i = tid; i < a.m; i += nth) {
        const double v = a.y0 ? a.y0[a.pr ? a.pr[i] : i] : 0.0;
        double ys = (v * a.row_norm[i]) / a.c_scale;
        if (!isfinite(a.AL[i])) ys = fmin(ys, 0.0);
        if (!isfinite(a.AU[i])) ys = fmax(ys, 0.0);
        a.y[i] = ys;
        a.last_y[i] = ys;
        a.y_bar[i] = ys;
    }
}
void launch_start_in(const StartInArgs &a, hipStream_t s) {
    hipLaunchKernelGGL(k_start_in, dim3(vec_grid(a.n > a.m ? a.n : a.m)), dim3(kThreads), 0, s, a);
}

__global__ void __launch_bounds__(kThreads) k_data_in(DataInArgs a) {
    double acc[4] = {0.0, 0.0, 0.0, 0.0};
    const int tid = blockIdx.x * kThreads + threadIdx.x, nth = gridDim.x * kThreads;
    for (int i = tid; i < a.m; i += nth) {
        const int src = a.pr ? a.pr[i] : i;
        const double lo = a.AL_in[src], hi = a.AU_in[src], rn = a.row_norm[i];
        const double v = fmax(fabs(isinf(lo) ? 0.0 : lo), fabs(isinf(hi) ? 0.0 : hi));
        acc[0] += v * v;
        const double los = lo / rn, his = hi / rn;
        a.AL[i] = los;
        a.AU[i] = his;
        const double w = fmax(fabs(isinf(los) ? 0.0 : los), fabs(isinf(his) ? 0.0 : his));
        acc[2] += w * w;
    }
    for (int j = tid; j < a.nc; j += nth) {
        const double v = a.c_in[a.pc ? a.pc[j] : j];
        acc[1] += v * v;
        const double vs = v / a.col_norm[j];
        a.c[j] = vs;
        acc[3] += vs * vs;
    }
    for (int j = tid; j < a.nb; j += nth) {
// ... 122 lines not shown
```

### hpr-lp-c_amd/csrc/solver.cpp

```cpp
#include "solver.h"
#include "env.h"

#include <algorithm>
#include <cmath>
#include <cstdio>
#include <cstdlib>
#include <cstring>
#include <functional>
#include <iomanip>
#include <iostream>
#include <limits>
#include <thread>

#include "dist.h"
#include "reorder.h"

namespace hprlp {

constexpr int kMaxGraphIters = 64;
constexpr int kDeviceStartRows = 1000000;
constexpr int kPowerBlockKey = -10;

struct RowCuts {
    std::vector<int> rows;
// ... 1161 lines not shown
        launch_vec_scale(c.p, t2, n_loc, true, stream);
        launch_vec_scale(l.p, t2, n_loc, false, stream);
        launch_vec_scale(u.p, t2, n_loc, false, stream);
    }

    if (prm.use_bc_scaling) {
        b_scale = 1.0 + std::sqrt(bnorm_sq(this));
        c_scale = 1.0 + std::sqrt(reduce_sum_sq(c.p, n_loc));
        const double bs = 1.0 / b_scale, cs = 1.0 / c_scale;
        launch_vec_scal(AU.p, bs, m_loc, stream);
        launch_vec_scal(AL.p, bs, m_loc, stream);
        launch_vec_scal(l.p, bs, n_loc, stream);
        launch_vec_scal(u.p, bs, n_loc, stream);
        launch_vec_scal(c.p, cs, n_loc, stream);
    } else {
        b_scale = 1.0;
        c_scale = 1.0;
    }
    norm_b = std::sqrt(bnorm_sq(this));
    norm_c = std::sqrt(reduce_sum_sq(c.p, n_loc));
    finish_tiling();
    A.refresh_tiled(stream);
    AT.refresh_tiled(stream);
    refresh_bound_codes();
    HIP_CHECK(hipMemsetAsync(gsm.p, 0, sizeof(double) * m_pad, stream));
    HIP_CHECK(hipMemsetAsync(gsn.p, 0, sizeof(double) * n_pad, stream));
    HIP_CHECK(hipStreamSynchronize(stream));
    scaling_time = time_since(t0);
    scaled = true;
}

double Solver::power_iteration(int max_iter, double tol, int *iters) {
    finish_tiling();
    invalidate_far();
    const auto t0 = time_now();
    double *q = gsm.p + row_off, *ATq = gsn.p + col_off, *z = sm1.p;
    const bool host_start = env_get("HPRLP_HOST_POWER_START") != nullptr;
    if (m_loc > kDeviceStartRows && perm_r.empty() && !host_start) {
        launch_pw_start(m_loc, 1ULL, row_off, z, stream);
    } else {
        std::vector<double> z0(static_cast<size_t>(std::max(m_loc, 1)));
        power_start_vector(m_loc, 1ULL, row_off, z0.data());
        if (!perm_r.empty()) {
            std::vector<double> zp(z0.size());
            for (int i = 0; i < m_loc; ++i) zp[i] = z0[perm_r[i]];
            z0.swap(zp);
        }
        HIP_CHECK(hipMemcpyAsync(z, z0.data(), sizeof(double) * m_loc, hipMemcpyHostToDevice, stream));
        HIP_CHECK(hipStreamSynchronize(stream));
    }
    const bool no_small_power = env_get("HPRLP_NO_SMALL_POWER") != nullptr;
    if (use_small && !comm && !no_small_power) {
        const SmallArgs a{m, n, A.view.nnz, A.view.rowptr, AT.view.rowptr, AT.view.val, small_ij.p, small_posA.p,
                          small_order_x.p, small_order_y.p, x.p, x_hat, y, l.p, u.p, c.p, last_x.p, AL.p, AU.p, last_y.p, ctrl.p};
        HIP_CHECK(hipMemsetAsync(scal.p + S_SMALL_PW_LAMBDA, 0, 2 * sizeof(double), stream));
        launch_small_power(a, z, max_iter, tol, scal.p + S_SMALL_PW_LAMBDA, stream);
        fetch_scalars();
        const double lambda_dev = scal_h[S_SMALL_PW_LAMBDA];
        const int done_dev = static_cast<int>(scal_h[S_SMALL_PW_ITERS]);
        if (done_dev > 0 && std::isfinite(lambda_dev) && lambda_dev > 0.0) {
            if (iters) *iters = done_dev;
            power_iters = done_dev;
            power_time = time_since(t0);
            return lambda_dev;
        }
        if (verbose) std::cerr << "[hprlp] single-launch power iteration returned lambda = " << lambda_dev << " after " << done_dev
                               << " iterations: falling back to the regular kernels" << std::endl;
    }
    launch_norm2(z, m_loc, part_v.p, kReduceBlocks, stream);
    FinalizeArgs f0{};
    f0.n = 1;
    f0.item[0] = {part_v.p, kReduceBlocks, S_PW_ZZ};
    launch_finalize(f0, scal.p, stream);
    allreduce_slots(this, S_PW_ZZ, 1);

    double lambda = 1.0;
    int done = max_iter;
    const int gridA = A.view.grid();
    auto one_iteration = [&]() {
        launch_pw_normalize(z, q, m_loc, scal.p, stream);
        gather(gsm.p, true);
        const bool push_pays = A.view.tiled.valid && static_cast<double>(A.tiled.n_rem) >= 0.3 * static_cast<double>(A.view.nnz);
        const bool handed = launch_spmv_push(AT.view, gsm.p, ATq, push_pays ? push_into(A, AT) : FarPush{}, stream);
        gather(gsn.p, false);
        launch_spmv_plain(A.view, gsn.p, z, q, true, part_y.p, stride_y, stream, handed);
        FinalizeArgs f{};
        f.n = 2;
        f.item[0] = {part_y.p, gridA, S_PW_ZZ};
        f.item[1] = {part_y.p + stride_y, gridA, S_PW_QZ};
        launch_finalize(f, scal.p, stream);
        allreduce_slots(this, S_PW_ZZ, 2);
    };
    auto error_terms = [&]() {
        launch_pw_err(z, q, m_loc, scal.p, part_v.p, kReduceBlocks, stream);
        FinalizeArgs fe{};
        fe.n = 1;
        fe.item[0] = {part_v.p, kReduceBlocks, S_PW_ERR2};
        launch_finalize(fe, scal.p, stream);
        allreduce_slots(this, S_PW_ERR2, 1);
    };
    hipGraphExec_t block = nullptr;
    if (use_graph && max_iter >= 10) {
        auto it = graphs.find(kPowerBlockKey);
        if (it != graphs.end()) {
            block = it->second;
        } else {
            hipGraph_t g = nullptr;
            HIP_CHECK(hipStreamBeginCapture(stream, hipStreamCaptureModeThreadLocal));
            for (int k = 0; k < 10; ++k) one_iteration();
            error_terms();
            HIP_CHECK(hipStreamEndCapture(stream, &g));
            HIP_CHECK(hipGraphInstantiate(&block, g, nullptr, nullptr, 0));
            HIP_CHECK(hipGraphDestroy(g));
            graphs[kPowerBlockKey] = block;
        }
    }
    for (int i = 1; i <= max_iter; ++i) {
        if (block && i % 10 == 1 && i + 9 <= max_iter) {
            HIP_CHECK(hipGraphLaunch(block, stream));
            i += 9;
        } else {
            one_iteration();
            if (i % 10 == 0) error_terms();
        }
        if (i % 10 == 0) {
            fetch_scalars();
            lambda = scal_h[S_PW_QZ];
            const double err = std::sqrt(scal_h[S_PW_ERR2]);
            if (err < tol) {
                done = i;
                break;
            }
        }
    }
    if (iters) *iters = done;
    power_iters = done;
    HIP_CHECK(hipMemsetAsync(gsm.p, 0, sizeof(double) * m_pad, stream));
    HIP_CHECK(hipMemsetAsync(gsn.p, 0, sizeof(double) * n_pad, stream));
    HIP_CHECK(hipStreamSynchronize(stream));
    power_time = time_since(t0);
    return lambda;
}

void Solver::set_sigma_lambda(double sigma_, double lambda_, bool reset_k) {
    sigma = sigma_;
    lambda_max = lambda_;
    launch_set_ctrl(ctrl.p, sigma, lambda_max, reset_k ? 1 : 0, stream);
}

void Solver::read_hooks() {
    hook_no_far_push = env_get("HPRLP_NO_FAR_PUSH") && env_get("HPRLP_NO_FAR_PUSH")[0] == '1';
    hook_no_bound_codes = env_get("HPRLP_NO_BOUND_CODES") != nullptr;
    hook_store_x = env_get("HPRLP_STORE_X") != nullptr;
}

void Solver::refresh_bound_codes() {
    if (hook_no_bound_codes) return;
    if (n_loc > 0) {
        if (lu_code.n != static_cast<size_t>(n_loc)) lu_code.alloc(static_cast<size_t>(n_loc));
        launch_bound_codes(n_loc, l.p, u.p, lu_code.p, stream);
    }
    if (m_loc > 0) {
        if (row_code.n != static_cast<size_t>(m_loc)) row_code.alloc(static_cast<size_t>(m_loc));
        launch_row_codes(m_loc, AL.p, AU.p, row_code.p, stream);
    }
}

void Solver::reset_iterates() {
    if (y_exchange_pending) throw std::runtime_error("reset_iterates: an exchange is still pending");
    invalidate_far();
    auto zero = [&](double *p, size_t n) {
        if (p && n > 0) HIP_CHECK(hipMemsetAsync(p, 0, sizeof(double) * n, stream));
    };
    zero(x.p, x.n); zero(last_x.p, last_x.n); zero(z_bar.p, z_bar.n);
    zero(last_y.p, last_y.n); zero(y_obj.p, y_obj.n); zero(y_temp.p, y_temp.n);
    zero(gy.p, gy.n); zero(gyb.p, gyb.n); zero(gsm.p, gsm.n);
    zero(gxh.p, gxh.n); zero(gxb.p, gxb.n); zero(gxt.p, gxt.n); zero(gsn.p, gsn.n);
    zero(sm1.p, sm1.n); zero(sn1.p, sn1.n);
    zero(scal.p, scal.n);
    HIP_CHECK(hipMemsetAsync(ctrl.p, 0, sizeof(Ctrl), stream));
    HIP_CHECK(hipStreamSynchronize(stream));
}

void Solver::init_iteration_state() {
    finish_tiling();
    invalidate_far();
    refresh_bound_codes();
    if (overlap_enabled && !overlap_ready) prepare_overlap();
    const double s0 = (norm_b > 1e-8 && norm_c > 1e-8) ? norm_b / norm_c : 1.0;
    set_sigma_lambda(s0, lambda_max, true);
}

static void split_shard(const DeviceMatrix &M, int lo, int hi, Solver::SplitShard *out, hipStream_t s) {
    const int rows = M.view.rows, cols = M.view.cols;
    device_split_columns(rows, M.view.nnz, M.rowptr.p, M.col.p, M.val.p, lo, hi, out->loc.rowptr, out->loc.col, out->loc.val,
                         out->rem.rowptr, out->rem.col, out->rem.val, s);
    std::vector<int> rp(static_cast<size_t>(rows) + 1);
    out->loc.rowptr.download(rp.data(), rp.size());
    out->loc.describe(rows, cols, rp.data(), nullptr, nullptr);
    out->rem.rowptr.download(rp.data(), rp.size());
    out->rem.describe(rows, cols, rp.data(), nullptr, nullptr);
    out->loc.finish_tiling(s);
    out->rem.finish_tiling(s);
    out->part.alloc_zero(static_cast<size_t>(std::max(rows, 1)));
    if (out->loc.view.tiled.valid) out->loc.view.tiled.grid = 8 * out->loc.view.tiled.per;
}

void Solver::ensure_comm_stream() {
    if (!comm_stream) {
        int prio_low = 0, prio_high = 0;
        HIP_CHECK(hipDeviceGetStreamPriorityRange(&prio_low, &prio_high));
        HIP_CHECK(hipStreamCreateWithPriority(&comm_stream, hipStreamDefault, prio_high));
        HIP_CHECK(hipEventCreateWithFlags(&ev_ready, hipEventDisableTiming));
        HIP_CHECK(hipEventCreateWithFlags(&ev_done_x, hipEventDisableTiming));
        HIP_CHECK(hipEventCreateWithFlags(&ev_done_y, hipEventDisableTiming));
    }
}

void Solver::prepare_overlap() {
    finish_tiling();
    HIP_CHECK(hipStreamSynchronize(stream));
    ensure_comm_stream();
    ovAT.reset(new SplitShard);
    split_shard(AT, row_off, row_off + m_loc, ovAT.get(), stream);
    ovA.reset(new SplitShard);
    split_shard(A, col_off, col_off + n_loc, ovA.get(), stream);
    HIP_CHECK(hipDeviceSynchronize());
    overlap_ready = true;
}

FarPush Solver::push_into(const DeviceMatrix &consumer, const DeviceMatrix &producer) const {
    const TiledDev &pt = producer.view.tiled;
    if (hook_no_far_push || comm || !pt.valid || pt.n_pieces > 0) return FarPush{};
    if (consumer.view.tiled.valid && consumer.view.tiled.G != pt.R) return FarPush{};
    return far_push_of(consumer.view);
}

int Solver::x_mode_of(int i, int count) const {
    if (hook_store_x || overlap_enabled || !AT.view.tiled.valid) return 0;
    return (i > 0 ? kXRebuild : 0) | (i + 1 < count ? kXNoStore : 0);
}

void Solver::launch_normal_pair(bool more_follow, hipEvent_t *ev, int x_mode) {
    XHalfArgs xa{gy.p, x.p, x_hat, l.p, u.p, c.p, last_x.p, nullptr, nullptr, nullptr, ctrl.p, nullptr, 0};
    xa.lu_code = lu_code.p;
    xa.x_mode = x_mode;
    YHalfArgs ya{gxh.p, y, AL.p, AU.p, last_y.p, nullptr, nullptr, nullptr, ctrl.p, nullptr, 0};
    ya.row_code = row_code.p;
    if (ev) HIP_CHECK(hipEventRecord(ev[0], stream));
    if (!overlap_enabled) {
        xa.push = push_into(A, AT);
        xa.far_ready = far_AT_ready;
        far_A_ready = launch_x_half(AT.view, xa, false, stream);
        if (ev) HIP_CHECK(hipEventRecord(ev[1], stream));
        gather(gxh.p, false);
        ya.push = push_into(AT, A);
        ya.far_ready = far_A_ready;
        far_AT_ready = launch_y_half(A.view, ya, false, stream);
        if (ev) HIP_CHECK(hipEventRecord(ev[2], stream));
        gather(gy.p, true);
        return;
    }
    invalidate_far();
    if (!overlap_ready) prepare_overlap();
    auto exchange_beside = [&](double *gbuf, bool is_m, hipEvent_t done, const CsrDev *local, double *part) {
        HIP_CHECK(hipEventRecord(ev_ready, stream));
        const bool spmv_first = overlap_spmv_first;
        if (local && spmv_first) launch_spmv_plain(*local, gbuf, part, nullptr, false, nullptr, 0, stream);
        HIP_CHECK(hipStreamWaitEvent(comm_stream, ev_ready, 0));
        gather_on(gbuf, is_m, comm_stream);
        HIP_CHECK(hipEventRecord(done, comm_stream));
        if (local && !spmv_first) launch_spmv_plain(*local, gbuf, part, nullptr, false, nullptr, 0, stream);
    };
    if (y_exchange_pending) {
        if (!overlap_spmv_first)
            launch_spmv_plain(ovAT->loc.view, gy.p, ovAT->part.p, nullptr, false, nullptr, 0, stream);
        HIP_CHECK(hipStreamWaitEvent(stream, ev_done_y, 0));
        launch_x_half_base(ovAT->rem.view, xa, ovAT->part.p, stream);
        y_exchange_pending = false;
    } else {
        launch_x_half(AT.view, xa, false, stream);
    }
    if (ev) HIP_CHECK(hipEventRecord(ev[1], stream));
    exchange_beside(gxh.p, false, ev_done_x, &ovA->loc.view, ovA->part.p);
    HIP_CHECK(hipStreamWaitEvent(stream, ev_done_x, 0));
    launch_y_half_base(ovA->rem.view, ya, ovA->part.p, stream);
    if (ev) HIP_CHECK(hipEventRecord(ev[2], stream));
    exchange_beside(gy.p, true, ev_done_y, more_follow && overlap_spmv_first ? &ovAT->loc.view : nullptr, ovAT->part.p);
    if (more_follow) y_exchange_pending = true;
    else HIP_CHECK(hipStreamWaitEvent(stream, ev_done_y, 0));
}

void Solver::step(bool check) {
    finish_tiling();
    if (!check) {
        launch_normal_pair();
        return;
    }
    XHalfArgs xa{gy.p, x.p, x_hat, l.p, u.p, c.p, last_x.p, x_bar, z_bar.p, x_temp, ctrl.p, part_x.p, stride_x};
    xa.lu_code = lu_code.p;
    xa.push = push_into(A, AT);
    xa.far_ready = far_AT_ready;
    far_A_ready = launch_x_half(AT.view, xa, true, stream);
    gather(gxh.p, false);
    YHalfArgs ya{gxh.p, y, AL.p, AU.p, last_y.p, y_bar, y_obj.p, y_temp.p, ctrl.p, part_y.p, stride_y};
    ya.row_code = row_code.p;
    ya.push = push_into(AT, A);
    ya.far_ready = far_A_ready;
    far_AT_ready = launch_y_half(A.view, ya, true, stream);
    gather(gy.p, true);
    FinalizeArgs f{};
    const int gx = AT.view.grid(), gyy = A.view.grid();
    f.n = 5;
    f.item[0] = {part_x.p, gx, S_CX};
    f.item[1] = {part_x.p + stride_x, gx, S_XZ};
    f.item[2] = {part_x.p + 2 * static_cast<size_t>(stride_x), gx, S_DX2};
    f.item[3] = {part_y.p, gyy, S_YOBJ_Y};
    f.item[4] = {part_y.p + stride_y, gyy, S_DY2};
    launch_finalize(f, scal.p, stream);
}

hipGraphExec_t Solver::graph_for(int len) {
    auto it = graphs.find(len);
    if (it != graphs.end()) return it->second;
    hipGraph_t g = nullptr;
    hipGraphExec_t ge = nullptr;
    far_AT_ready = false;
    HIP_CHECK(hipStreamBeginCapture(stream, hipStreamCaptureModeThreadLocal));
    for (int i = 0; i < len; ++i) launch_normal_pair(false, nullptr, x_mode_of(i, len));
    HIP_CHECK(hipStreamEndCapture(stream, &g));
    graph_end_A = far_A_ready;
    graph_end_AT = far_AT_ready;
    invalidate_far();
    HIP_CHECK(hipGraphInstantiate(&ge, g, nullptr, nullptr, 0));
    HIP_CHECK(hipGraphDestroy(g));
    graphs[len] = ge;
    return ge;
}

void Solver::run_normal(int count) {
    if (count <= 0) return;
    finish_tiling();
    if (use_small && !comm) {
        const SmallArgs a{m, n, A.view.nnz, A.view.rowptr, AT.view.rowptr, AT.view.val, small_ij.p, small_posA.p,
                          small_order_x.p, small_order_y.p, x.p, x_hat, y, l.p, u.p, c.p, last_x.p, AL.p, AU.p, last_y.p, ctrl.p};
        launch_small_iterations(a, count, stream);
        return;
    }
    if (!use_graph) {
        for (int i = 0; i < count; ++i) launch_normal_pair(i + 1 < count, nullptr, x_mode_of(i, count));
        return;
    }
    while (count > 0) {
        const int len = std::min(count, kMaxGraphIters);
        HIP_CHECK(hipGraphLaunch(graph_for(len), stream));
        far_A_ready = graph_end_A;
        far_AT_ready = graph_end_AT;
        count -= len;
    }
}

void Solver::run_normal_then_check(int count) {
    run_normal(count);
    step(true);
}

static double weighted_norm_from(Solver *s, double dot_adx_dy, double dy2, double dx2) {
    const double dot_prod = 2.0 * dot_adx_dy;
    double wn = s->sigma * (s->lambda_max * dy2) + dx2 / s->sigma + dot_prod;
    if (wn < 0) {
        if (s->verbose)
            std::cout << "The estimated maximum eigenvalue is too small! Current value is " << s->lambda_max << "\n";
        s->lambda_max = -(dot_prod + dx2 / s->sigma) / (s->sigma * dy2) * 1.05;
        if (s->verbose) std::cout << "The new estimated maximum eigenvalue is " << s->lambda_max << "\n";
        wn = std::sqrt(-(dot_prod + dx2 / s->sigma) * 0.05);
        s->set_sigma_lambda(s->sigma, s->lambda_max, false);
    } else {
        wn = std::sqrt(wn);
    }
    return wn;
}

void Solver::compute_residuals(int iter, bool compute_gap, Residuals *r, RestartState *rs, bool *ray) {
    invalidate_far();
    finish_tiling();
    const int gx = AT.view.grid(), gyy = A.view.grid();
    const int rstride = std::max(stride_x, stride_y);
    gather(gyb.p, true);
    gather(gxb.p, false);
    if (compute_gap) gather(gxt.p, false);
    FinalizeArgs f{};
    launch_resid_d(AT.view, gyb.p, c.p, z_bar.p, col_norm.p, part_x.p, stream);
    f.item[f.n++] = {part_x.p, gx, S_RD2};
    launch_resid_p(A.view, gxb.p, gxt.p, AL.p, AU.p, row_norm.p, y_temp.p, compute_gap, part_r.p, rstride, stream);
    f.item[f.n++] = {part_r.p, gyy, S_RP2};
    if (compute_gap) f.item[f.n++] = {part_r.p + rstride, gyy, S_ADX_DY};
    if (iter == 0) {
        launch_lu(n_loc, x_bar, l.p, u.p, col_norm.p, x_temp, part_v.p, kReduceBlocks, stream);
// ... 200 lines not shown
    FinalizeArgs f{};
    const int form_slots[kRayFormAccs] = {S_RAY_DY, S_RAY_CD, S_RAY_VY, S_RAY_WD, S_RAY_YN, S_RAY_DN};
    for (int k = 0; k < kRayFormAccs; ++k) f.item[f.n++] = {pf + static_cast<size_t>(k) * kReduceBlocks, kReduceBlocks, form_slots[k], k >= 2};
    launch_finalize(f, scal.p, stream);
    invalidate_far();
    launch_ray_col(AT.view, ray_y.p, l.p, u.p, col_norm.p, b_scale, c_scale, pc, stream);
    launch_ray_row(A.view, ray_d.p, AL.p, AU.p, row_norm.p, b_scale, pr, stream);
    FinalizeArgs g{};
    g.item[g.n++] = {pc, gx, S_RAY_DZ, 0};
    g.item[g.n++] = {pc + gx, gx, S_RAY_VZ, 1};
    g.item[g.n++] = {pr, gyy, S_RAY_WQ, 1};
    launch_finalize(g, scal.p, stream);
    return true;
}

RayScalars Solver::ray_scalars() {
    return RayScalars{scal_h[S_RAY_DY] + scal_h[S_RAY_DZ], std::max(scal_h[S_RAY_VY], scal_h[S_RAY_VZ]), scal_h[S_RAY_CD],
                      std::max(scal_h[S_RAY_WD], scal_h[S_RAY_WQ]), scal_h[S_RAY_YN], scal_h[S_RAY_DN]};
}

void Solver::collect_certificate(int kind, int iter) {
    cert = Certificate();
    std::vector<double> rn(static_cast<size_t>(m_loc)), cn(static_cast<size_t>(n_loc));
    HIP_CHECK(hipMemcpyAsync(rn.data(), row_norm.p, sizeof(double) * m_loc, hipMemcpyDeviceToHost, stream));
    HIP_CHECK(hipMemcpyAsync(cn.data(), col_norm.p, sizeof(double) * n_loc, hipMemcpyDeviceToHost, stream));
    auto unpermute = [](std::vector<double> &v, const std::vector<int> &perm) {
        if (perm.empty() || v.empty()) return;
        const std::vector<double> tmp(v);
        for (size_t i = 0; i < perm.size(); ++i) v[perm[i]] = tmp[i];
    };
    if (kind == 1) {
        invalidate_far();
        launch_spmv_plain(AT.view, ray_y.p, sn1.p, nullptr, false, nullptr, 0, stream);
        cert.y.resize(static_cast<size_t>(m_loc));
        cert.z.resize(static_cast<size_t>(n_loc));
        HIP_CHECK(hipMemcpyAsync(cert.y.data(), ray_y.p, sizeof(double) * m_loc, hipMemcpyDeviceToHost, stream));
        HIP_CHECK(hipMemcpyAsync(cert.z.data(), sn1.p, sizeof(double) * n_loc, hipMemcpyDeviceToHost, stream));
    } else {
        cert.d.resize(static_cast<size_t>(n_loc));
        HIP_CHECK(hipMemcpyAsync(cert.d.data(), ray_d.p, sizeof(double) * n_loc, hipMemcpyDeviceToHost, stream));
    }
    HIP_CHECK(hipStreamSynchronize(stream));
    finish_certificate(&cert, kind, iter, ray_scalars(), rn.data(), cn.data(), b_scale, c_scale);
    unpermute(cert.y, perm_r);
    unpermute(cert.z, perm_c);
    unpermute(cert.d, perm_c);
}

void Solver::set_start(const double *x0, const double *y0) {
    if (comm) throw std::runtime_error("warm start runs on one GPU only (sharded solver)");
    if (y_exchange_pending) throw std::runtime_error("set_start: an exchange is still pending");
    const auto t0 = time_now();
    finish_tiling();
    invalidate_far();
    DBuf<double> dx, dy;
    DBuf<int> dpc, dpr;
    if (x0 && n_loc > 0) {
        dx.alloc(static_cast<size_t>(n_loc));
        HIP_CHECK(hipMemcpyAsync(dx.p, x0, sizeof(double) * n_loc, hipMemcpyHostToDevice, stream));
    }
    if (y0 && m_loc > 0) {
        dy.alloc(static_cast<size_t>(m_loc));
        HIP_CHECK(hipMemcpyAsync(dy.p, y0, sizeof(double) * m_loc, hipMemcpyHostToDevice, stream));
    }
    if (!perm_c.empty() && dx.p) {
        dpc.alloc(perm_c.size());
        HIP_CHECK(hipMemcpyAsync(dpc.p, perm_c.data(), sizeof(int) * perm_c.size(), hipMemcpyHostToDevice, stream));
    }
    if (!perm_r.empty() && dy.p) {
        dpr.alloc(perm_r.size());
        HIP_CHECK(hipMemcpyAsync(dpr.p, perm_r.data(), sizeof(int) * perm_r.size(), hipMemcpyHostToDevice, stream));
    }
    const StartInArgs a{n_loc, m_loc, dx.p, dy.p, dpc.p, dpr.p, l.p, u.p, col_norm.p, AL.p, AU.p, row_norm.p, b_scale, c_scale,
                        x.p, last_x.p, x_hat, x_bar, y, last_y.p, y_bar};
    launch_start_in(a, stream);
    const int gx = AT.view.grid(), gyy = A.view.grid();
    launch_start_col(AT.view, gyb.p, c.p, l.p, u.p, x_bar, z_bar.p, part_x.p, stream);
    launch_start_row(A.view, gxb.p, AL.p, AU.p, y_bar, y_obj.p, part_r.p, stream);
    FinalizeArgs f{};
    f.item[f.n++] = {part_x.p, gx, S_CX};
    f.item[f.n++] = {part_x.p + gx, gx, S_XZ};
    f.item[f.n++] = {part_r.p, gyy, S_YOBJ_Y};
    launch_finalize(f, scal.p, stream);
    HIP_CHECK(hipStreamSynchronize(stream));
    start_time = time_since(t0);
}

void Solver::set_data(const double *c_, const double *obj_constant_, const double *AL_, const double *AU_, const double *l_, const double *u_) {
    if (comm) throw std::runtime_error("new data for a resident model runs on one GPU only (sharded solver)");
    if (!scaled) throw std::runtime_error("set_data: the solver has not been scaled yet (hprlp_solver_scale comes first)");
    const bool bounds = AL_ || AU_ || l_ || u_;
    if (bounds && !(AL_ && AU_ && l_ && u_))
        throw std::runtime_error("set_data: AL, AU, l and u are given together or not at all (b_scale couples them)");
    auto no_nan = [](const double *v, long len, const char *what) {
        for (long i = 0; v && i < len; ++i)
            if (std::isnan(v[i])) throw std::runtime_error(std::string("set_data: ") + what + "[" + std::to_string(i) + "] is NaN");
    };
    no_nan(c_, n, "c"); no_nan(AL_, m, "AL"); no_nan(AU_, m, "AU"); no_nan(l_, n, "l"); no_nan(u_, n, "u");
    if (obj_constant_ && std::isnan(*obj_constant_)) throw std::runtime_error("set_data: obj_constant is NaN");
    data_time[0] = data_time[1] = data_time[2] = 0.0;
    if (obj_constant_) obj_constant = *obj_constant_;
    if (!c_ && !bounds) return;
    const auto t0 = time_now();
    const int mb = bounds ? m_loc : 0, nb = bounds ? n_loc : 0, nc = c_ ? n_loc : 0;
    const size_t total = 2 * static_cast<size_t>(mb) + 2 * static_cast<size_t>(nb) + static_cast<size_t>(nc);
    if (data_stage.n < total) data_stage.alloc(total);
    double *dAL = data_stage.p, *dAU = dAL + mb, *dl = dAU + mb, *du = dl + nb, *dc = du + nb;
    const struct { const double *src; double *dst; int len; } parts[5] = {{AL_, dAL, mb}, {AU_, dAU, mb}, {l_, dl, nb}, {u_, du, nb}, {c_, dc, nc}};
    if (total * sizeof(double) < kDeviceCacheMinBytes) {
        data_pack.resize(total);
        for (const auto &q : parts)
            if (q.len > 0) std::memcpy(data_pack.data() + (q.dst - data_stage.p), q.src, sizeof(double) * q.len);
        HIP_CHECK(hipMemcpyAsync(data_stage.p, data_pack.data(), sizeof(double) * total, hipMemcpyHostToDevice, stream));
    } else {
        for (const auto &q : parts)
            if (q.len > 0) HIP_CHECK(hipMemcpyAsync(q.dst, q.src, sizeof(double) * q.len, hipMemcpyHostToDevice, stream));
    }
    if (!perm_r.empty() && !perm_r_dev.p) {
        perm_r_dev.alloc(perm_r.size());
        perm_c_dev.alloc(perm_c.size());
        HIP_CHECK(hipMemcpyAsync(perm_r_dev.p, perm_r.data(), sizeof(int) * perm_r.size(), hipMemcpyHostToDevice, stream));
        HIP_CHECK(hipMemcpyAsync(perm_c_dev.p, perm_c.data(), sizeof(int) * perm_c.size(), hipMemcpyHostToDevice, stream));
    }
    if (!data_part.p) data_part.alloc_zero(static_cast<size_t>(4) * kReduceBlocks);
    unsigned char *rc = nullptr, *lc = nullptr;
    if (!hook_no_bound_codes && bounds) {
        if (row_code.n != static_cast<size_t>(m_loc) || lu_code.n != static_cast<size_t>(n_loc)) {
            for (auto &kv : graphs) (void)hipGraphExecDestroy(kv.second);
            graphs.clear();
            HIP_CHECK(hipStreamSynchronize(stream));
            row_code.alloc(static_cast<size_t>(m_loc));
            lu_code.alloc(static_cast<size_t>(n_loc));
        }
        rc = row_code.p;
        lc = lu_code.p;
    }
    data_time[0] = time_since(t0);
    const auto t1 = time_now();
    const DataInArgs in{mb, nc, nb, dAL, dAU, dc, dl, du, perm_c_dev.p, perm_r_dev.p, row_norm.p, col_norm.p,
                        AL.p, AU.p, c.p, l.p, u.p, data_part.p, kReduceBlocks};
    launch_data_in(in, stream);
    FinalizeArgs f{};
    if (bounds) {
        f.item[f.n++] = {data_part.p, kReduceBlocks, S_DATA_B_ORG};
        f.item[f.n++] = {data_part.p + 2 * static_cast<size_t>(kReduceBlocks), kReduceBlocks, S_DATA_B_PRE};
    }
    if (c_) {
        f.item[f.n++] = {data_part.p + kReduceBlocks, kReduceBlocks, S_DATA_C_ORG};
        f.item[f.n++] = {data_part.p + 3 * static_cast<size_t>(kReduceBlocks), kReduceBlocks, S_DATA_C_PRE};
    }
    launch_finalize(f, scal.p, stream);
    const DataBcArgs bc{mb, nc, nb, prm.use_bc_scaling ? 1 : 0, scal.p, AL.p, AU.p, c.p, l.p, u.p, rc, lc, data_part.p, kReduceBlocks};
    launch_data_bc(bc, stream);
    FinalizeArgs g{};
    if (bounds) g.item[g.n++] = {data_part.p, kReduceBlocks, S_DATA_NB};
    if (c_) g.item[g.n++] = {data_part.p + kReduceBlocks, kReduceBlocks, S_DATA_NC};
    launch_finalize(g, scal.p, stream);
    fetch_scalars();
    if (bounds) {
        norm_b_org = 1.0 + std::sqrt(scal_h[S_DATA_B_ORG]);
        b_scale = prm.use_bc_scaling ? 1.0 + std::sqrt(scal_h[S_DATA_B_PRE]) : 1.0;
        norm_b = std::sqrt(scal_h[S_DATA_NB]);
    }
    if (c_) {
        norm_c_org = 1.0 + std::sqrt(scal_h[S_DATA_C_ORG]);
        c_scale = prm.use_bc_scaling ? 1.0 + std::sqrt(scal_h[S_DATA_C_PRE]) : 1.0;
        norm_c = std::sqrt(scal_h[S_DATA_NC]);
    }
    invalidate_far();
    if (data_stage.cap_bytes >= kDeviceCacheMinBytes) data_stage.release();
    data_time[1] = time_since(t1);
    data_time[2] = time_since(t0);
    data_since_run += data_time[2];
}

void Solver::resolve(double sigma_, const double *x0, const double *y0, HPRLP_results *out) {
    if (comm) throw std::runtime_error("re-solve runs on one GPU only (sharded solver)");
    reset_iterates();
    init_iteration_state();
    if (sigma_ > 0.0) set_sigma_lambda(sigma_, lambda_max, true);
    if (x0 || y0) set_start(x0, y0);
    time_base = data_since_run;
    try {
        solve_loop(out);
    } catch (...) {
        time_base = -1.0;
        throw;
    }
    time_base = -1.0;
    collect_solution(out);
}

}
```

### hpr-lp-c_amd/csrc/solver.h

```cpp
#pragma once

#include <string>
#include <vector>

#include <functional>
#include <future>
#include <map>
#include <memory>

#include "common.h"
#include "env.h"
#include "dist.h"
#include "kernels.h"
#include "hpr_rules.h"
#include "form_select.h"

namespace hprlp {

HPRLP_batched_results solve_batched_impl(const LP_info_cpu *model, int batch_size, const HPRLP_FLOAT *C, const HPRLP_FLOAT *AL,
                                         const HPRLP_FLOAT *AU, const HPRLP_FLOAT *l, const HPRLP_FLOAT *u,
                                         const HPRLP_FLOAT *obj_constants, const HPRLP_parameters *param, const Detection *det,
                                         std::vector<Certificate> *certs, const HPRLP_FLOAT *X0 = nullptr,
                                         const HPRLP_FLOAT *Y0 = nullptr);
HPRLP_batched_results make_batched_error(const char *status, int m, int n, int B);

struct TraceRow {
    int iter, restart_flag;
    double err_Rp, err_Rd, primal_obj, dual_obj, gap, kkt, sigma, current_gap, lambda_max;
};

struct DeviceMatrix {
    DBuf<int> rowptr, col;
    DBuf<double> val;
    DBuf<int4> blk, longrows;
    DBuf<double> long_partial;
    DeviceTiled tiled;
    int sb_rows = kTileRows, far_group = kTileRows;
    int rem_cap = kTileRemCap;
    int tile_cols = kTileCols;
    CsrDev view;
    std::future<std::shared_ptr<TiledHost>> tiling;
    int planned_grid = 0;
    void upload(int rows, int cols, const int *rp, const int *ci, const double *v, std::shared_ptr<void> keep = nullptr);
    void describe(int rows, int cols, const int *rp, const int *ci, std::shared_ptr<void> keep, double min_dense_override = -1.0);
    void describe_when(int rows, int cols, long nnz, std::shared_future<const int *> rp_ready, const int *ci, std::shared_ptr<void> keep,
                       double min_dense_override, std::future<void> *values_ready);
    void build_tiled_copy(int rows, int cols, int nnz, double long_row_share, const std::function<const int *()> &host_rp, const int *ci,
                          std::shared_ptr<void> keep, double min_dense_override, const std::function<void()> &join_values, struct PhaseTimer &pt);
    int longest_row = 0;
    FormOutcome outcome;
    FormFacts facts = blank_form_facts(), facts_pb = blank_form_facts();
    int passes = 0;
    double xcd_gather_bytes = 0.0;
    void finish_tiling(hipStream_t s);
    void refresh_tiled(hipStream_t s);
};

std::vector<int4> build_row_blocks(int rows, const int *rowptr, std::vector<int4> *longrows);
void row_block_plan_host(int rows, int cols, const int *rp, const int *ci, bool with_cuts, long out[6]);

struct HaloPlan {
    bool sparse = false;
    int nsend = 0, nrecv = 0;
    long total_requests = 0;
    DBuf<int> send_idx, recv_idx;
    DBuf<double> sendbuf, recvbuf;
    std::vector<P2P> ops;
    void build(Comm *comm, const int *cols, long nnz, int total, int chunk, hipStream_t s);
};

struct Solver {
    HPRLP_parameters prm;
    int m = 0, n = 0;
    int m_loc = 0, n_loc = 0;
    int row_off = 0, col_off = 0;
    int m_pad = 0, n_pad = 0;
    double obj_constant = 0.0;
    bool verbose = true;
    hipStream_t stream = nullptr;
    Comm *comm = nullptr;
    Comm *xcomm = nullptr;

    DeviceMatrix A, AT;
    std::vector<int> perm_r, perm_c;
    double reorder_time = 0.0, reorder_before = 0.0, reorder_after = 0.0;
    bool allow_reorder = true;
    bool try_reorder(const LP_info_cpu *model);
    void choose_sb_rows(const LP_info_cpu *model);
    void choose_pb_rows(DeviceMatrix &M, DeviceMatrix &other, int rows, int other_rows);
    bool pb_fallback_wanted(DeviceMatrix &M, const int *other_rowptr, int other_rows);
    bool far_A_ready = false, far_AT_ready = false;
    bool graph_end_A = false, graph_end_AT = false;
    void invalidate_far() { far_A_ready = far_AT_ready = false; }
    FarPush push_into(const DeviceMatrix &consumer, const DeviceMatrix &producer) const;
    HaloPlan halo_m, halo_n;
    DBuf<double> AL, AU, l, u, c, row_norm, col_norm;
    DBuf<unsigned char> row_code;
    DBuf<unsigned char> lu_code;
    void refresh_bound_codes();
    DBuf<double> x, last_x, z_bar, last_y, y_obj, y_temp;
    DBuf<double> gy, gxh, gxb, gyb, gxt, gsn, gsm;
    double *y = nullptr, *x_hat = nullptr, *x_bar = nullptr, *y_bar = nullptr, *x_temp = nullptr;
    DBuf<double> sm1, sn1;
    DBuf<Ctrl> ctrl;
    DBuf<double> scal;
    HBuf<double> scal_h;
    DBuf<double> part_x, part_y, part_r, part_v;
    int stride_x = 0, stride_y = 0;

    double b_scale = 1, c_scale = 1, norm_b = 0, norm_c = 0, norm_b_org = 1, norm_c_org = 1;
    double sigma = 1.0, lambda_max = 1.0;
    double setup_time = 0, scaling_time = 0, power_time = 0;
    double fetch_enqueue_s = 0, fetch_wait_s = 0;
    long fetches = 0;
    int power_iters = 0;
    bool use_graph = true;
    bool use_small = false;
    int max_row_A = 0, max_row_AT = 0;
    DBuf<int> small_order_x, small_order_y;
    DBuf<int> small_ij, small_posA;

    Detection detect;
    DBuf<double> ray_prev_x, ray_prev_y, ray_d, ray_y, ray_part;
    bool ray_have_prev = false;
    Certificate cert;
    void ray_begin();
    bool ray_test();
    RayScalars ray_scalars();
    void collect_certificate(int kind, int iter);

    void set_start(const double *x0, const double *y0);
    double start_time = 0.0;

    void set_data(const double *c_, const double *obj_constant_, const double *AL_, const double *AU_, const double *l_, const double *u_);
    void resolve(double sigma_, const double *x0, const double *y0, HPRLP_results *out);
    double data_time[3] = {0.0, 0.0, 0.0};
    double data_since_run = 0.0;
    double time_base = -1.0;
    bool scaled = false;
    DBuf<double> data_stage, data_part;
    DBuf<int> perm_r_dev, perm_c_dev;
    std::vector<double> data_pack;

    std::map<int, hipGraphExec_t> graphs;
    TraceRow *trace = nullptr;
    int trace_cap = 0, trace_n = 0;

    Solver() = default;
    ~Solver();
    Solver(const Solver &) = delete;

    void setup(const LP_info_cpu *model, const HPRLP_parameters *param);
    void setup_shard(int m_glob, int n_glob, int row_off_, int m_loc_, int col_off_, int n_loc_, const int *Arp,
                     const int *Aci, const double *Av, const int *ATrp, const int *ATci, const double *ATv,
                     const double *AL_, const double *AU_, const double *l_, const double *u_, const double *c_,
                     double obj_constant_, const HPRLP_parameters *param, Comm *comm_);
    void scale();
    double power_iteration(int max_iter, double tol, int *iters);
    void init_iteration_state();
    void set_sigma_lambda(double sigma_, double lambda_, bool reset_k);
    void reset_iterates();
    void step(bool check);
    void run_normal(int count);
    void run_normal_then_check(int count);
    void fetch_scalars();
    void compute_residuals(int iter, bool compute_gap, Residuals *r, RestartState *rs, bool *ray = nullptr);
    double weighted_norm_after_restart();
    void update_sigma_and_restart(RestartState *rs, const Residuals &r);
    void solve_loop(HPRLP_results *out);
    void collect_solution(HPRLP_results *out);
    double reduce_sum_sq(const double *v, int n_local);
    void verify_exchange();
    void gather(double *gbuf, bool is_m) { gather_on(gbuf, is_m, stream); }
    void gather_on(double *gbuf, bool is_m, hipStream_t s);

    struct SplitShard {
        DeviceMatrix loc, rem;
        DBuf<double> part;
    };
    std::unique_ptr<SplitShard> ovA, ovAT;
    hipStream_t comm_stream = nullptr;
    hipEvent_t ev_ready = nullptr, ev_done_x = nullptr, ev_done_y = nullptr;
    std::string env_at_setup, env_ignored_at_setup;
    bool hook_no_far_push = false, hook_no_bound_codes = false, hook_store_x = false;
    void read_hooks();
    bool overlap_enabled = false, overlap_ready = false, y_exchange_pending = false;
    bool overlap_spmv_first = false;
    void prepare_overlap();
    void ensure_comm_stream();
    void allreduce_scalars();
    void finish_tiling();

    void launch_normal_pair(bool more_follow = false, hipEvent_t *ev = nullptr, int x_mode = 0);
    int x_mode_of(int i, int count) const;

   private:
    void alloc_work();
    hipGraphExec_t graph_for(int len);
};

}
```

### hpr-lp-c_amd/csrc/tiled.h

```cpp
#pragma once

#include <hip/hip_runtime.h>

#include <cstdint>
#include <vector>

#include "common.h"

namespace hprlp {

constexpr int kTileThreads = 512;
constexpr int kTileRows = 8192;
constexpr int kTileCols = 2048;
constexpr int kTileColsNarrow = 1024;
constexpr int kTileChunk = 4;
constexpr int kTileStepCap = kTileThreads * kTileChunk;
constexpr int kTileRemK = 4;
constexpr int kTileRemCap = (kTileThreads - 4) * kTileRemK;
constexpr int kTileRemRun = 16;
#ifndef HPRLP_PB_REM_K
#define HPRLP_PB_REM_K 8
#endif
constexpr int kPbRemK = HPRLP_PB_REM_K;
constexpr int kPbRemCap = kTileThreads * kPbRemK;
constexpr int kPbRowsMax = 4096;
constexpr int kPbRunTabCap = 3072;
constexpr int kTileMaxRow = 1024;
constexpr int kTileDenseMin = 256;
static_assert(kTileRemCap % kTileRemK == 0 && kTileRemCap + (kTileThreads / 64) * 3 / 2 <= kTileCols, "tile buffer too small for the remainder scratch");
constexpr int kTileRowBits = 13;
constexpr int kTileRowsMin = 1024;
static_assert((1 << kTileRowBits) == kTileRows && kTileCols <= (1 << (24 - kTileRowBits)) && kTileChunk == 4,
              "entry codes are 24 bits: 13 of local row, 11 of local column, four per chunk");
inline uint32_t tile_code(int lcol, int row) { return (static_cast<uint32_t>(lcol) << kTileRowBits) | static_cast<uint32_t>(row); }

struct PackLayout {
    int n1 = 0, n2 = 0, n3 = 0, n4 = 0;
    int u3 = 0, u2 = 0, r1 = 0, c2 = 0;
    __host__ __device__ void set(int a1, int a2, int a3, int a4) {
        n1 = a1; n2 = a2; n3 = a3; n4 = a4;
        u3 = n1 < n3 ? n1 : n3;
        c2 = (n2 + 1) / 2;
        const int left = n1 - u3;
        u2 = (n2 & 1) ? (left < 2 ? left : 2) : 0;
        r1 = left - u2;
    }
    __host__ __device__ int entries() const { return kTileChunk * (n4 + n3 + c2 + (r1 + 3) / 4); }
    __host__ __device__ int pos(int L, int j) const {
        if (L == 4) return 4 * j;
        if (L == 3) return 4 * (n4 + j);
        if (L == 2) return 4 * (n4 + n3 + j / 2) + 2 * (j & 1);
        if (j < u3) return 4 * (n4 + j) + 3;
        j -= u3;
        if (j < u2) return 4 * (n4 + n3 + n2 / 2) + 2 + j;
        j -= u2;
        return 4 * (n4 + n3 + c2) + j;
    }
    __host__ __device__ int pads_after(int L, int j) const {
        if (L == 3) return j >= u3 ? 1 : 0;
        if (L == 2) return ((n2 & 1) && j == n2 - 1) ? (u2 == 0 ? 2 : 0) : 0;
        if (L == 1) {
            if (j < u3) return 0;
            j -= u3;
            if (j < u2) return (u2 == 1) ? 1 : 0;
            j -= u2;
            return (j == r1 - 1) ? (4 - (r1 & 3)) & 3 : 0;
        }
        return 0;
    }
};

#ifndef HPRLP_TILE_LAYERS
#define HPRLP_TILE_LAYERS 4
#endif
#ifndef HPRLP_TILE_LAYER_MIN
#define HPRLP_TILE_LAYER_MIN 1024
#endif
constexpr int kTileLayers = HPRLP_TILE_LAYERS;
constexpr int kTileLayerMin = HPRLP_TILE_LAYER_MIN;

constexpr int kTileResidentPerCu = 2;
constexpr int kFarGroup = kTileRows;
constexpr int kFarThreads = 512;
constexpr long kFarWorkMin = 32768;
constexpr long kFarWorkOverMean = 4;

struct TileStep {
    int col0;
    int e_begin;
    int e_end;
    int rot;
};

struct TiledDev {
    bool valid = false;
    int R = kTileRows;
    int rem_cap = kTileRemCap;
    int T = kTileCols;
    int G = kTileRows;
    int nsb = 0;
    int per = 0;
    int grid = 0;
    bool repeats = false;
    int n_pieces = 0;
    const int *piece_ptr = nullptr;
    const int4 *segs = nullptr;
    const int *slot_ptr = nullptr;
    double *parts = nullptr;
    const int4 *side_blk = nullptr;
    int side_nblk = 0;
    const int4 *side_long = nullptr;
    int side_nlong = 0;
    double *side_partial = nullptr;
    const int *side_rows = nullptr;
    double *base = nullptr;
    unsigned long long *stamps = nullptr;
    unsigned long long *wgtimes = nullptr;
    int wg_filter = 0;
    const int *sb_ptr = nullptr;
    const int *sb_mid = nullptr;
    const TileStep *steps = nullptr;
    const double *tval = nullptr;
    const uint32_t *tidx3 = nullptr;
    double *P = nullptr;
    const uint32_t *rq = nullptr;
    int n_groups = 0;
    const int *f_gptr = nullptr;
    const double *f_val = nullptr;
    const int *f_pos = nullptr;
    const uint16_t *f_lcol = nullptr;
    const int *f_rptr = nullptr;
    const int *f_rk = nullptr;
    const int *f_rp = nullptr;
    int f_maxruns = 0;
    const int4 *f_work = nullptr;
    int n_work = 0;
};

struct TiledHost {
    std::vector<int> sb_ptr, sb_mid;
    std::vector<TileStep> steps;
    struct Piece {
        std::vector<uint32_t> tidx;
        std::vector<int> tperm;
        std::vector<int> rcol, rperm;
        std::vector<uint16_t> rrow;
    };
    std::vector<Piece> pieces;
    size_t n_tile = 0, n_rem = 0;
    long dense_entries = 0;
    long padding = 0;
};

bool build_tiled(int rows, int cols, const int *rowptr, const int *col, TiledHost *out, int min_rows,
                 double min_dense_fraction, int R = kTileRows, int T = kTileCols, int rem_cap = kTileRemCap);

void tiled_host_check(int rows, int cols, const int *rp, const int *ci, int R, int T, double min_dense, long out[6]);

void compact_without_rows(long nnz, int rows, const int *rp_dev, const int *rp_c_dev, const int *col_dev, int *col_c, int *map_c, hipStream_t s);

struct DeviceTiled {
    DBuf<int> sb_ptr, sb_mid, tperm, rperm, rcol;
    DBuf<TileStep> steps;
    DBuf<uint32_t> tidx;
    DBuf<uint32_t> tidx3;
    DBuf<uint16_t> rrow;
    DBuf<double> tval;
    DBuf<double> P, f_val;
    DBuf<uint32_t> rq;
    DBuf<int> f_gptr, f_pos, f_perm;
    DBuf<int> f_rptr, f_rk, f_rp;
    DBuf<int4> f_work;
    DBuf<uint16_t> f_lcol;
    TiledDev view;
    long n_tile = 0, n_rem = 0;
    double rem_top_share = 0.0;
    long dense_entries = 0, padding = 0;
    int n_steps = 0;
    void upload(const TiledHost &h, int R = kTileRows, int T = kTileCols, int rem_cap = kTileRemCap);
    void pack_indices(hipStream_t s);
    void build_far(int cols, hipStream_t s, int G = kTileRows);
    void finish_schedule(hipStream_t s);
    int rot_period = 0;
    DBuf<double> parts;
    DBuf<int> piece_ptr, slot_ptr;
    DBuf<unsigned long long> stamps;
    void dump_stamps() const;
    DBuf<unsigned long long> wgtimes;
    DBuf<int4> side_blk, side_long;
    DBuf<int> side_rows;
    DBuf<double> side_partial, base;
    void set_side(int rows, const int *rowptr_host, const std::vector<int> &long_rows);
    void compose_perms(const int *map_dev, hipStream_t s);
    void dump_wgtimes() const;
    DBuf<int4> segs;
    bool build_on_device(int rows, int cols, long nnz, const int *rowptr, const int *col, int min_rows,
                         double min_dense_fraction, hipStream_t s, int R = kTileRows, int T = kTileCols, int rem_cap = kTileRemCap);
    void compare_with(const TiledHost &h) const;
};

void launch_tiled_refresh(const DeviceTiled &t, const double *csr_val, hipStream_t s);
void launch_tiled_refresh_log(const DeviceTiled &t, const double *csr_val, double *tval_log, double *fval_log, hipStream_t s);

}
```

### hpr-lp-c_amd/csrc/tiled_build.hip

```cpp
#include <algorithm>
#include <functional>
#include <cstdlib>
#include <hipcub/hipcub.hpp>

#include <vector>

#include "common.h"
#include "env.h"
#include "kernels.h"
#include "tiled.h"

namespace hprlp {

namespace {

constexpr int K = kTileChunk;
constexpr int kRowBits = kTileRowBits;

__device__ __forceinline__ int row_of_entry(const int *__restrict__ rowptr, int rows, int k) {
    int lo = 0, hi = rows;
    while (hi - lo > 1) {
        const int mid = lo + ((hi - lo) >> 1);
        if (rowptr[mid] <= k) lo = mid;
        else hi = mid;
// ... 650 lines not shown
    f_lcol[f] = static_cast<uint16_t>(rcol[e] - g * G);
    f_perm[f] = rperm[e];
}

__global__ void __launch_bounds__(kThreads) k_far_gptr(int ngroups, int n, const unsigned long long *__restrict__ skey, int *__restrict__ gptr) {
    const int g = blockIdx.x * kThreads + threadIdx.x;
    if (g > ngroups) return;
    int lo = 0, hi = n;
    while (lo < hi) {
        const int mid = lo + ((hi - lo) >> 1);
        if (static_cast<int>(skey[mid] >> 32) < g) lo = mid + 1;
        else hi = mid;
    }
    gptr[g] = lo;
}

__global__ void __launch_bounds__(kThreads) k_far_run_flags(int n, const unsigned long long *__restrict__ skey, const int *__restrict__ f_pos,
                                                           int *__restrict__ flag) {
    const int f = blockIdx.x * kThreads + threadIdx.x;
    if (f >= n) return;
    flag[f] = (f == 0 || (skey[f] >> 32) != (skey[f - 1] >> 32) || f_pos[f] != f_pos[f - 1] + 1) ? 1 : 0;
}

__global__ void __launch_bounds__(kThreads) k_far_run_fill(int n, const int *__restrict__ flag, const int *__restrict__ run_excl,
                                                          const int *__restrict__ f_pos, int *__restrict__ rk, int *__restrict__ rp) {
    const int f = blockIdx.x * kThreads + threadIdx.x;
    if (f >= n || !flag[f]) return;
    rk[run_excl[f]] = f;
    rp[run_excl[f]] = f_pos[f];
}

__global__ void __launch_bounds__(kThreads) k_far_rptr(int ngroups, int n, int nruns, const int *__restrict__ gptr, const int *__restrict__ run_excl,
                                                      int *__restrict__ rptr, int *__restrict__ maxruns) {
    const int g = blockIdx.x * kThreads + threadIdx.x;
    if (g > ngroups) return;
    const int f = gptr[g];
    rptr[g] = f < n ? run_excl[f] : nruns;
    if (g < ngroups) {
        const int f1 = gptr[g + 1];
        const int r1 = f1 < n ? run_excl[f1] : nruns;
        atomicMax(maxruns, r1 - rptr[g]);
    }
}

void sort_pairs(DBuf<unsigned long long> &kin, DBuf<unsigned long long> &kout, DBuf<int> &vin, DBuf<int> &vout, int n, int end_bit, hipStream_t s) {
    size_t bytes = 0;
    HIP_CHECK(hipcub::DeviceRadixSort::SortPairs(nullptr, bytes, kin.p, kout.p, vin.p, vout.p, n, 0, end_bit, s));
    DBuf<char> tmp(bytes + 16);
    HIP_CHECK(hipcub::DeviceRadixSort::SortPairs(tmp.p, bytes, kin.p, kout.p, vin.p, vout.p, n, 0, end_bit, s));
    HIP_CHECK(hipStreamSynchronize(s));
}

int bits_for(long v) {
    int b = 1;
    while ((1L << b) <= v) ++b;
    return b;
}

}

void DeviceTiled::build_far(int cols, hipStream_t s, int G) {
    static_assert(kFarGroup <= 65536 && kTileRemCap <= 65536 && kTileRows <= 65536, "16-bit local columns, slots and rows");
    if (G < 64 || G > kFarGroup) throw std::runtime_error("remainder lists: unsupported source-group size");
    view.G = G;
    view.P = nullptr;
    view.rq = nullptr;
    view.n_groups = 0;
    if (!view.valid || n_rem <= 0) {
        rcol.release(); rrow.release(); rperm.release();
        return;
    }
    const int n = static_cast<int>(n_rem), nsb = view.nsb;
    const int ngroups = (cols + G - 1) / G;
    DBuf<int> step_of(static_cast<size_t>(n)), sb_of(static_cast<size_t>(n));
    const char *no2 = env_get("HPRLP_NO_REM2");
    hipLaunchKernelGGL(k_far_step_of, dim3(nsb), dim3(kThreads), 0, s, nsb, sb_ptr.p, sb_mid.p, steps.p, rrow.p, step_of.p, sb_of.p, !(no2 && no2[0] == '1'));
    if (env_get("HPRLP_TIMING")) {
        std::vector<TileStep> hs(static_cast<size_t>(n_steps));
        std::vector<int> hp(static_cast<size_t>(nsb) + 1), hm(static_cast<size_t>(nsb));
        HIP_CHECK(hipStreamSynchronize(s));
        steps.download(hs.data(), hs.size());
        sb_ptr.download(hp.data(), hp.size());
        sb_mid.download(hm.data(), hm.size());
        long rem_steps = 0, marked = 0, most = 0;
        for (int sb = 0; sb < nsb; ++sb) {
            most = std::max<long>(most, hp[sb + 1] - hm[sb]);
            for (int q = hm[sb]; q < hp[sb + 1]; ++q) {
                ++rem_steps;
                marked += hs[q].col0 != 0;
            }
        }
        std::fprintf(stderr, "[timing]   remainder: %ld steps (most in one super-block: %ld), %ld with a long run of one row\n", rem_steps, most, marked);
    }
    DBuf<unsigned long long> kin(static_cast<size_t>(n)), kout(static_cast<size_t>(n));
    DBuf<int> vin(static_cast<size_t>(n)), e_of_p(static_cast<size_t>(n));
    hipLaunchKernelGGL(k_far_key_p, dim3(grid_for(n)), dim3(kThreads), 0, s, n, G, sb_of.p, rcol.p, kin.p, vin.p);
    sort_pairs(kin, kout, vin, e_of_p, n, 32 + bits_for(nsb), s);
    sb_of.release();
    DBuf<int> p_sorted(static_cast<size_t>(n));
    hipLaunchKernelGGL(k_far_key_q, dim3(grid_for(n)), dim3(kThreads), 0, s, n, step_of.p, e_of_p.p, kin.p, vin.p);
    sort_pairs(kin, kout, vin, p_sorted, n, 32 + bits_for(n_steps), s);
    rq.alloc_zero(static_cast<size_t>(n) + 8);
    hipLaunchKernelGGL(k_far_fill_q, dim3(grid_for(n)), dim3(kThreads), 0, s, n, kout.p, p_sorted.p, steps.p, rrow.p, rq.p);
    HIP_CHECK(hipStreamSynchronize(s));
    step_of.release();
    hipLaunchKernelGGL(k_far_key_f, dim3(grid_for(n)), dim3(kThreads), 0, s, n, G, e_of_p.p, rcol.p, kin.p, vin.p);
    sort_pairs(kin, kout, vin, p_sorted, n, 32 + bits_for(ngroups), s);
    f_pos.alloc_zero(static_cast<size_t>(n) + 8);
    f_lcol.alloc_zero(static_cast<size_t>(n) + 8);
    f_perm.alloc(static_cast<size_t>(n) + 8);
    f_val.alloc_zero(static_cast<size_t>(n) + 8);
    f_gptr.alloc(static_cast<size_t>(ngroups) + 1);
    hipLaunchKernelGGL(k_far_fill_f, dim3(grid_for(n)), dim3(kThreads), 0, s, n, G, kout.p, p_sorted.p, rcol.p, rperm.p, f_pos.p, f_lcol.p, f_perm.p);
    hipLaunchKernelGGL(k_far_gptr, dim3(grid_for(ngroups + 1)), dim3(kThreads), 0, s, ngroups, n, kout.p, f_gptr.p);
    P.alloc_zero(static_cast<size_t>(n) + 8);
    HIP_CHECK(hipStreamSynchronize(s));
    {
        std::vector<int> gp(static_cast<size_t>(ngroups) + 1);
        f_gptr.download(gp.data(), gp.size());
        const long cap = std::max<long>(kFarWorkMin, kFarWorkOverMean * static_cast<long>(n) / std::max(ngroups, 1));
        int heaviest = 0;
        for (int g = 0; g < ngroups; ++g) heaviest = std::max(heaviest, gp[g + 1] - gp[g]);
        {
            std::vector<int> sz(static_cast<size_t>(ngroups));
            for (int g = 0; g < ngroups; ++g) sz[g] = gp[g + 1] - gp[g];
            const int k = std::max(1, std::min(ngroups, static_cast<int>((2L << 20) / (8L * G))));
            std::nth_element(sz.begin(), sz.begin() + (k - 1), sz.end(), std::greater<int>());
            long top = 0;
            for (int g = 0; g < k; ++g) top += sz[g];
            rem_top_share = static_cast<double>(top) / static_cast<double>(n);
        }
        view.f_work = nullptr;
        view.n_work = 0;
        f_work.release();
        if (heaviest > cap && !env_get("HPRLP_NO_FAR_WORK")) {
            std::vector<int4> wl;
            wl.reserve(static_cast<size_t>(ngroups) + 64);
            for (int g = 0; g < ngroups; ++g) {
                const long b = gp[g], e = gp[g + 1];
                if (e <= b) continue;
                const long parts = (e - b + cap - 1) / cap, per = (e - b + parts - 1) / parts;
                for (long q = b; q < e; q += per) wl.push_back(make_int4(g, static_cast<int>(q), static_cast<int>(std::min(e, q + per)), 0));
            }
            f_work.alloc(wl.size());
            f_work.upload(wl.data(), wl.size());
            view.f_work = f_work.p;
            view.n_work = static_cast<int>(wl.size());
            if (env_get("HPRLP_TIMING"))
                std::fprintf(stderr, "[timing]   pre-pass work list: %d workgroups for %d source groups (heaviest group %d entries, chunks of at most %ld)\n",
                             view.n_work, ngroups, heaviest, cap);
        }
    }
    view.f_rptr = view.f_rk = view.f_rp = nullptr;
    view.f_maxruns = 0;
    if (view.rem_cap == kPbRemCap) {
        DBuf<int> flag(static_cast<size_t>(n)), excl(static_cast<size_t>(n));
        hipLaunchKernelGGL(k_far_run_flags, dim3(grid_for(n)), dim3(kThreads), 0, s, n, kout.p, f_pos.p, flag.p);
        size_t bytes = 0;
        HIP_CHECK(hipcub::DeviceScan::ExclusiveSum(nullptr, bytes, flag.p, excl.p, n, s));
        {
            DBuf<char> tmp(bytes + 16);
            HIP_CHECK(hipcub::DeviceScan::ExclusiveSum(tmp.p, bytes, flag.p, excl.p, n, s));
            HIP_CHECK(hipStreamSynchronize(s));
        }
        int last_excl = 0, last_flag = 0;
        HIP_CHECK(hipMemcpy(&last_excl, excl.p + (n - 1), sizeof(int), hipMemcpyDeviceToHost));
        HIP_CHECK(hipMemcpy(&last_flag, flag.p + (n - 1), sizeof(int), hipMemcpyDeviceToHost));
        const int nruns = last_excl + last_flag;
        f_rk.alloc(static_cast<size_t>(nruns) + 8);
        f_rp.alloc(static_cast<size_t>(nruns) + 8);
        f_rptr.alloc(static_cast<size_t>(ngroups) + 1);
        DBuf<int> mx;
        mx.alloc_zero(1);
        hipLaunchKernelGGL(k_far_run_fill, dim3(grid_for(n)), dim3(kThreads), 0, s, n, flag.p, excl.p, f_pos.p, f_rk.p, f_rp.p);
        hipLaunchKernelGGL(k_far_rptr, dim3(grid_for(ngroups + 1)), dim3(kThreads), 0, s, ngroups, n, nruns, f_gptr.p, excl.p, f_rptr.p, mx.p);
        int h_mx = 0;
        HIP_CHECK(hipMemcpyAsync(&h_mx, mx.p, sizeof(int), hipMemcpyDeviceToHost, s));
        HIP_CHECK(hipStreamSynchronize(s));
        if (h_mx > 0 && h_mx <= kPbRunTabCap && static_cast<long>(n) >= 48L * nruns) {
            view.f_rptr = f_rptr.p;
            view.f_rk = f_rk.p;
            view.f_rp = f_rp.p;
            view.f_maxruns = h_mx;
        }
        if (env_get("HPRLP_TIMING"))
            std::fprintf(stderr, "[timing]   source-side run tables: %d runs of %d entries (%.1f per run), most in one group %d%s\n", nruns, n,
                         static_cast<double>(n) / std::max(nruns, 1), h_mx, view.f_rk ? "" : " -- not used (too many for the producers' LDS table)");
    }
    rcol.release(); rrow.release(); rperm.release();
    view.P = P.p;
    view.rq = rq.p;
    view.n_groups = ngroups;
    view.f_gptr = f_gptr.p;
    view.f_val = f_val.p;
    view.f_pos = f_pos.p;
    view.f_lcol = f_lcol.p;
}

namespace {

__global__ void __launch_bounds__(kThreads) k_compact_cols(long nnz, int rows, const int *__restrict__ rp, const int *__restrict__ rp_c,
                                                          const int *__restrict__ col, int *__restrict__ col_c, int *__restrict__ map_c) {
    const long k = static_cast<long>(blockIdx.x) * kThreads + threadIdx.x;
    if (k >= nnz) return;
    int lo = 0, hi = rows;
    while (hi - lo > 1) {
        const int mid = lo + ((hi - lo) >> 1);
        if (rp[mid] <= k) lo = mid;
        else hi = mid;
    }
    if (rp_c[lo + 1] == rp_c[lo]) return;
    const int q = rp_c[lo] + static_cast<int>(k - rp[lo]);
    col_c[q] = col[k];
    map_c[q] = static_cast<int>(k);
}

__global__ void __launch_bounds__(kThreads) k_compose_perm(long n, int *__restrict__ perm, const int *__restrict__ map) {
    const long i = static_cast<long>(blockIdx.x) * kThreads + threadIdx.x;
    if (i < n && perm[i] >= 0) perm[i] = map[perm[i]];
}

}

void compact_without_rows(long nnz, int rows, const int *rp_dev, const int *rp_c_dev, const int *col_dev, int *col_c, int *map_c, hipStream_t s) {
    if (nnz > 0) hipLaunchKernelGGL(k_compact_cols, dim3(grid_for(nnz)), dim3(kThreads), 0, s, nnz, rows, rp_dev, rp_c_dev, col_dev, col_c, map_c);
    HIP_CHECK(hipStreamSynchronize(s));
}

void DeviceTiled::compose_perms(const int *map_dev, hipStream_t s) {
    if (n_tile > 0) hipLaunchKernelGGL(k_compose_perm, dim3(grid_for(n_tile)), dim3(kThreads), 0, s, n_tile, tperm.p, map_dev);
    if (n_rem > 0 && f_perm.p) hipLaunchKernelGGL(k_compose_perm, dim3(grid_for(n_rem)), dim3(kThreads), 0, s, n_rem, f_perm.p, map_dev);
    HIP_CHECK(hipStreamSynchronize(s));
}

void DeviceTiled::set_side(int rows, const int *rp, const std::vector<int> &long_rows) {
    std::vector<int4> blk, lng;
    int chunk_slots = 0;
    for (size_t q = 0; q < long_rows.size(); ++q) {
        const int i = long_rows[q], len = rp[i + 1] - rp[i];
        if (len > kSplitRow) {
            const int first = chunk_slots;
            for (int k = rp[i]; k < rp[i + 1]; k += kSplitRow) blk.push_back(make_int4(chunk_slots++, 0, k, std::min(kSplitRow, rp[i + 1] - k)));
            lng.push_back(make_int4(static_cast<int>(q), first, chunk_slots, 0));
        } else {
            blk.push_back(make_int4(static_cast<int>(q), 1, rp[i], len));
        }
    }
    side_blk.alloc(blk.size());
    side_blk.upload(blk.data(), blk.size());
    side_rows.alloc(long_rows.size());
    side_rows.upload(long_rows.data(), long_rows.size());
    base.alloc_zero(static_cast<size_t>(rows));
    view.side_blk = side_blk.p;
    view.side_nblk = static_cast<int>(blk.size());
    view.side_rows = side_rows.p;
    view.base = base.p;
    view.side_long = nullptr;
    view.side_nlong = 0;
    view.side_partial = nullptr;
    if (!lng.empty()) {
        side_long.alloc(lng.size());
        side_long.upload(lng.data(), lng.size());
        side_partial.alloc_zero(static_cast<size_t>(chunk_slots) * 2);
        view.side_long = side_long.p;
        view.side_nlong = static_cast<int>(lng.size());
        view.side_partial = side_partial.p;
    }
}

void DeviceTiled::dump_wgtimes() const {
    if (!wgtimes.p || view.grid <= 0) return;
    std::vector<unsigned long long> h(static_cast<size_t>(view.grid) * 8);
    wgtimes.download(h.data(), h.size());
    unsigned long long t0 = ~0ull, t1 = 0;
    for (int w = 0; w < view.grid; ++w) {
        if (h[w * 8] == 0) continue;
        t0 = std::min(t0, h[w * 8]);
        t1 = std::max(t1, h[w * 8 + 7]);
    }
    if (env_get("HPRLP_PB_STAMPS")) {
        double sum[8] = {0, 0, 0, 0, 0, 0, 0, 0}, mx[8] = {0, 0, 0, 0, 0, 0, 0, 0};
        int cnt = 0;
        for (int w = 0; w < view.grid; ++w) {
            if (h[w * 8 + 7] == 0) continue;
            ++cnt;
            for (int i = 0; i < 8; ++i) {
                sum[i] += h[w * 8 + i] / 100.0;
                mx[i] = std::max(mx[i], h[w * 8 + i] / 100.0);
            }
        }
        if (cnt)
            std::fprintf(stderr, "[pb stamps] %d workgroups, mean (max) us: wait+barrier %.1f (%.1f) | stage %.1f (%.1f) | flags+scan %.1f (%.1f) | level 1 %.1f (%.1f) | "
                                 "level 2 %.1f (%.1f) | epilogue %.1f (%.1f) | push %.1f (%.1f) | total %.1f (%.1f)\n",
                         cnt, sum[0] / cnt, mx[0], sum[1] / cnt, mx[1], sum[2] / cnt, mx[2], sum[3] / cnt, mx[3], sum[4] / cnt, mx[4], sum[5] / cnt, mx[5],
                         sum[6] / cnt, mx[6], sum[7] / cnt, mx[7]);
        return;
    }
    if (t1 == 0) return;
    if (const char *f = env_get("HPRLP_WG_TIMES_DUMP")) {
        if (FILE *fp = std::fopen(f, "a")) {
            std::fprintf(fp, "# launch grid %d\n", view.grid);
            for (int w = 0; w < view.grid; ++w) {
                if (h[w * 8] == 0) continue;
                const unsigned long long id = h[w * 8 + 6];
                std::fprintf(fp, "%d %llu %llu %.2f", w, id >> 32, (id >> 8) & 0xffull, (h[w * 8] - t0) / 100.0);
                for (int q = 1; q <= 5; ++q) std::fprintf(fp, " %.2f", h[w * 8 + q] ? (h[w * 8 + q] - t0) / 100.0 : -1.0);
                std::fprintf(fp, " %.2f\n", (h[w * 8 + 7] - t0) / 100.0);
            }
            std::fclose(fp);
        }
    }
    std::fprintf(stderr, "[wg times] %d workgroups, kernel span %.1f us (first start to last end)\n", view.grid, (t1 - t0) / 100.0);
    for (int x = 0; x < 8; ++x) {
        double s_min = 1e30, s_max = 0, e_min = 1e30, e_max = 0, e_sum = 0;
        int cnt = 0, rounds_max = 0;
        for (int w = x; w < view.grid; w += 8) {
            if (h[w * 8] == 0) continue;
            const double st = (h[w * 8] - t0) / 100.0, en = (h[w * 8 + 7] - t0) / 100.0;
            s_min = std::min(s_min, st); s_max = std::max(s_max, st);
            e_min = std::min(e_min, en); e_max = std::max(e_max, en);
            e_sum += en;
            ++cnt;
            int r = 0;
            for (int q = 1; q <= 5; ++q) r += h[w * 8 + q] != 0;
            rounds_max = std::max(rounds_max, r);
        }
        if (cnt) std::fprintf(stderr, "[wg times]   XCD %d: %d workgroups, start %.1f..%.1f us, end %.1f..%.1f us (mean %.1f), up to %d super-blocks each\n", x, cnt,
                              s_min, s_max, e_min, e_max, e_sum / cnt, rounds_max);
    }
    for (int q = 1; q <= 4; ++q) {
        double mn = 1e30, mx = 0, sum = 0;
        int cnt = 0;
        for (int w = 0; w < view.grid; ++w) {
            if (h[w * 8 + q] == 0) continue;
            const double d = (h[w * 8 + q] - h[w * 8 + q - 1]) / 100.0;
            mn = std::min(mn, d); mx = std::max(mx, d); sum += d;
// ... 28 lines not shown
```

Before: 779.7.

## Use run tables in tiled hand-off and compact finite bounds in x-half

Extends the source-side run tables to the non-all-remainder tiled form, so k_tiled_fused's push hand-off can look up product positions with an interleaved binary search over a table held in the tile buffer instead of reading f_pos for every entry. It also adds compact arrays of the finite l and u values with per-64-column rank bases, so the streamed x-half reads only finite bounds through ballot and mbcnt ranking rather than the full l and u arrays. Both aim to cut global memory traffic per iteration. In exchange they add set-up kernels, a host sync, graph invalidation when the buffers move, and extra LDS search work and register pressure in the hot kernels.

Measured after the change: 779.6. No clear change (-0.0%).

```diff
diff --git a/hpr-lp-c_amd/csrc/abi.cpp b/hpr-lp-c_amd/csrc/abi.cpp
--- a/hpr-lp-c_amd/csrc/abi.cpp
+++ b/hpr-lp-c_amd/csrc/abi.cpp
@@ -1213,6 +1213,9 @@
         return d;
     };
     std::string d = one("A", s.A) + "; " + one("A^T", s.AT);
+    if (s.push_into(s.A, s.AT).rk) d += "; hand-off into A: positions from run tables";
+    if (s.push_into(s.AT, s.A).rk) d += "; hand-off into A^T: positions from run tables";
+    if (s.cb_on) d += "; compact finite bounds in the x-half (" + std::to_string(s.n_l_fin) + " of l, " + std::to_string(s.n_u_fin) + " of u)";
     if (s.use_small && !s.comm) d += "; normal iterations in the single-workgroup kernel (k_small_iterations)";
     if (!s.perm_r.empty()) d += "; locality ordering applied at set-up";
     if (!s.env_at_setup.empty()) d += "; switches: " + s.env_at_setup;
diff --git a/hpr-lp-c_amd/csrc/env.cpp b/hpr-lp-c_amd/csrc/env.cpp
--- a/hpr-lp-c_amd/csrc/env.cpp
+++ b/hpr-lp-c_amd/csrc/env.cpp
@@ -32,6 +32,7 @@
     {"HPRLP_HOST_TILING", EnvKind::Hook, "build the tiled copies with the host builder (background threads, default min(16, cores)) instead of on the device"},
     {"HPRLP_HOST_TRANSPOSE", EnvKind::Hook, "build Aᵀ on the host / nonzero threshold of the device transpose (default 4 M)"},
     {"HPRLP_NO_BOUND_CODES", EnvKind::Hook, "the x-half always reads l[j] and u[j], the y-half AL[i] and AU[i] (default: one code byte per column / row says which of them is not a constant; an equality row reads one value)"},
+    {"HPRLP_NO_COMPACT_BOUNDS", EnvKind::Hook, "the tiled kernels' normal x-half reads the finite bounds from l[j] and u[j] (default: from compact arrays of the finite ones, addressed by a rank base per 64 columns)"},
     {"HPRLP_NO_FAR_PUSH", EnvKind::Hook, "always run the remainder pre-pass (k_far_products) instead of the hand-off from the producing half-step's epilogue"},
     {"HPRLP_NO_FAR_WORK", EnvKind::Hook, "the remainder pre-pass with one workgroup per source group also where one group holds several times the mean (default: a work list cuts heavy groups into chunks, tiled.h f_work)"},
     {"HPRLP_NO_PB_LONG_ROWS", EnvKind::Hook, "a matrix kept off the tiled forms for its long rows keeps the stream kernel also where its columns are not popular (default: all-remainder form, Solver::pb_fallback_wanted)"},
@@ -39,6 +40,7 @@
     {"HPRLP_NO_LONG_SIDE", EnvKind::Hook, "a matrix with rows over 1024 entries keeps the stream kernel instead of being tiled with those rows kept aside"},
     {"HPRLP_NO_PB_FALLBACK", EnvKind::Hook, "unstructured large matrices keep the stream kernel instead of the tiled form without dense-tile requirement"},
     {"HPRLP_NO_PB_KERNEL", EnvKind::Hook, "run an all-remainder copy through k_tiled_fused's remainder steps instead of k_pb_fused (A/B)"},
+    {"HPRLP_NO_PUSH_RUNS", EnvKind::Hook, "k_tiled_fused's hand-off reads every entry's position from f_pos (default: looked up in the source group's run table, held in the tile buffer, where the table fits and runs are long)"},
     {"HPRLP_NO_REM2", EnvKind::Hook, "tiled build: no second remainder level"},
     {"HPRLP_NO_SETUP_OVERLAP", EnvKind::Hook, "set-up of a large model in line: no helper threads / copy streams for the value upload, the row blocks, A^T's row pointers and the model vectors (same bits either way)"},
     {"HPRLP_NO_SLAB_CUTS", EnvKind::Hook, "dense rows of a large matrix are not cut at the XCD eighths of the gathered vector (stream kernel)"},
@@ -54,6 +56,7 @@
     {"HPRLP_PRESOLVE_MAX_LINKS", EnvKind::Hook, "run one presolve stage alone / cut the chain after n links (tests, debugging)"},
     {"HPRLP_PRESOLVE_OFF", EnvKind::Hook, "switch presolve reductions / stages off (any subset; diagnostics)"},
     {"HPRLP_PRESOLVE_ONLY", EnvKind::Hook, "run one presolve stage alone / cut the chain after n links (tests, debugging)"},
+    {"HPRLP_PUSH_RUNS_CAP", EnvKind::Hook, "most runs of one source group for which k_tiled_fused's hand-off uses the run table, whatever the runs' length (ceiling: the 2048 its tile buffer holds; default: 2048 where a run holds 48 entries or more on average, else 0 -- tests force the tables with 2048 and the f_pos fall-back with a small value)"},
     {"HPRLP_REORDER_CLUSTER", EnvKind::Hook, "knobs of the HOST reference path of the ordering (hprlp_locality_ordering): nodes per cluster, refinement sweeps, trimming percentage"},
     {"HPRLP_REORDER_HOST", EnvKind::Hook, "run the clustering of the locality ordering on the host (the reference form; default: on the device)"},
     {"HPRLP_REORDER_SWEEPS", EnvKind::Hook, "knobs of the HOST reference path of the ordering (hprlp_locality_ordering): nodes per cluster, refinement sweeps, trimming percentage"},
diff --git a/hpr-lp-c_amd/csrc/kernels.h b/hpr-lp-c_amd/csrc/kernels.h
--- a/hpr-lp-c_amd/csrc/kernels.h
+++ b/hpr-lp-c_amd/csrc/kernels.h
@@ -99,10 +99,15 @@
     bool far_ready = false;
     const unsigned char *lu_code = nullptr;
     int x_mode = 0;
+    const double *l_fin = nullptr, *u_fin = nullptr;
+    const int *l_base = nullptr, *u_base = nullptr;
 };
 constexpr int kXRebuild = 1, kXNoStore = 2;
 constexpr unsigned kLoadL = 1u, kLoadU = 2u, kZeroL = 4u;
 void launch_bound_codes(int n, const double *l, const double *u, unsigned char *code, hipStream_t s);
+void launch_bound_ranks(int n, const unsigned char *code, int *l_base, int *u_base, hipStream_t s);
+void launch_bound_compact(int n, const unsigned char *code, const double *l, const double *u, const int *l_base, const int *u_base,
+                          double *l_fin, double *u_fin, hipStream_t s);
 
 struct YHalfArgs {
     const double *xhat_full;
@@ -132,7 +137,7 @@
 
 bool launch_x_half(const CsrDev &AT, const XHalfArgs &a, bool check, hipStream_t s);
 bool launch_y_half(const CsrDev &A, const YHalfArgs &a, bool check, hipStream_t s);
-FarPush far_push_of(const CsrDev &consumer);
+FarPush far_push_of(const CsrDev &consumer, int tab_cap);
 void launch_x_half_base(const CsrDev &AT_remote, const XHalfArgs &a, const double *base, hipStream_t s);
 void launch_y_half_base(const CsrDev &A_remote, const YHalfArgs &a, const double *base, hipStream_t s);
 
diff --git a/hpr-lp-c_amd/csrc/kernels.hip b/hpr-lp-c_amd/csrc/kernels.hip
--- a/hpr-lp-c_amd/csrc/kernels.hip
+++ b/hpr-lp-c_amd/csrc/kernels.hip
@@ -618,11 +618,41 @@
     return tab_p[lo] + (k - tab_k[lo]);
 }
 
+template <int U>
+__device__ __forceinline__ void run_positions(const int *tab_k, const int *tab_p, int nr, const int (&k)[U], int (&pos)[U]) {
+    int lo[U];
+#pragma unroll
+    for (int u = 0; u < U; ++u) lo[u] = 0;
+    int span = 1;
+    while (2 * span < nr) span *= 2;
+    for (; span > 0; span >>= 1) {
+#pragma unroll
+        for (int u = 0; u < U; ++u) {
+            const int mid = lo[u] + span;
+            if (mid < nr && tab_k[mid] <= k[u]) lo[u] = mid;
+        }
+    }
+#pragma unroll
+    for (int u = 0; u < U; ++u) pos[u] = tab_p[lo[u]] + (k[u] - tab_k[lo[u]]);
+}
+
+template <int CAP, bool INSTEP>
 __device__ __forceinline__ void push_products_runs(const FarPush &f, const double *vals, int *tab, int g, int pb, int pe, int tid) {
     constexpr int NT = kTileThreads, U = 4;
     if (pb >= pe) return;
-    const int r0 = f.rptr[g], nr = f.rptr[g + 1] - r0;
-    int *tab_k = tab, *tab_p = tab + kPbRunTabCap;
+    const int r0 = f.rptr[g], nr = min(f.rptr[g + 1] - r0, CAP);
+    int *tab_k = tab, *tab_p = tab + CAP;
+    auto lookup = [&](int k0, int (&ps)[U]) {
+        if constexpr (INSTEP) {
+            int kk[U];
+#pragma unroll
+            for (int u = 0; u < U; ++u) kk[u] = min(k0 + u * NT, pe - 1);
+            run_positions<U>(tab_k, tab_p, nr, kk, ps);
+        } else {
+#pragma unroll
+            for (int u = 0; u < U; ++u) ps[u] = run_position(tab_k, tab_p, nr, min(k0 + u * NT, pe - 1));
+        }
+    };
     double a4[U];
     uint16_t c4[U];
     auto load_batch = [&](int k0) {
@@ -641,8 +671,7 @@
     }
     lds_barrier();
     int ps[U];
-#pragma unroll
-    for (int u = 0; u < U; ++u) ps[u] = run_position(tab_k, tab_p, nr, min(k + u * NT, pe - 1));
+    lookup(k, ps);
     for (; k < pe; k += U * NT) {
         double prd[U];
         int pc[U];
@@ -656,10 +685,7 @@
 #pragma unroll
         for (int u = 0; u < U; ++u)
             if (k + u * NT < pe) f.P[pc[u]] = prd[u];
-        if (kn < pe) {
-#pragma unroll
-            for (int u = 0; u < U; ++u) ps[u] = run_position(tab_k, tab_p, nr, min(kn + u * NT, pe - 1));
-        }
+        if (kn < pe) lookup(kn, ps);
     }
 }
 
@@ -703,7 +729,8 @@
         epilogue_rows<Epi, PUSH>(epi, acc, racc, r0, nr, tid);
         if constexpr (PUSH) {
             lds_barrier();
-            push_products(epi.push, acc, pb, pe, tid);
+            if (epi.push.rk) push_products_runs<kTileRunTabCap, true>(epi.push, acc, reinterpret_cast<int *>(ytile), sb, pb, pe, tid);
+            else push_products(epi.push, acc, pb, pe, tid);
         }
         if (wg_stamp && ++wg_round <= 5) t.wgtimes[blockIdx.x * 8 + wg_round] = wall_clock64();
     }
@@ -761,7 +788,7 @@
         PB_STAMP(5);
         if constexpr (PUSH) {
             lds_barrier();
-            if (epi.push.rk) push_products_runs(epi.push, acc, reinterpret_cast<int *>(prod), sb, pb, pe, tid);
+            if (epi.push.rk) push_products_runs<kPbRunTabCap, false>(epi.push, acc, reinterpret_cast<int *>(prod), sb, pb, pe, tid);
             else push_products(epi.push, acc, pb, pe, tid);
         }
         PB_STAMP(6);
@@ -990,7 +1017,7 @@
 template <bool LOGTERM>
 static void launch_far_products(const TiledDev &t, const double *vec, int ncols, hipStream_t s) {
     const dim3 grid(((t.f_work ? t.n_work : t.n_groups) + 7) / 8 * 8);
-    if (t.f_rk && t.G <= kPbRowsMax) hipLaunchKernelGGL(k_far_products_runs<LOGTERM>, grid, dim3(kFarThreads), 0, s, t, vec, ncols);
+    if (t.f_rk && t.rem_cap == kPbRemCap && t.G <= kPbRowsMax) hipLaunchKernelGGL(k_far_products_runs<LOGTERM>, grid, dim3(kFarThreads), 0, s, t, vec, ncols);
     else hipLaunchKernelGGL(k_far_products<LOGTERM>, grid, dim3(kFarThreads), 0, s, t, vec, ncols);
 }
 
@@ -1011,6 +1038,8 @@
     const unsigned char *lu_code;
     int x_mode;
     double f1p, f2p;
+    const double *l_fin, *u_fin;
+    const int *l_base, *u_base;
     static constexpr bool kPublishes = true;
     static constexpr bool kSkipsX = !CHECK && STREAMED;
     struct Row {
@@ -1031,8 +1060,23 @@
         double li, ui;
         if (lu_code) {
             const unsigned cd = NT ? __builtin_nontemporal_load(lu_code + r) : lu_code[r];
-            li = (cd & kLoadL) ? ld(l + r) : ((cd & kZeroL) ? 0.0 : -__builtin_huge_val());
-            ui = (cd & kLoadU) ? ld(u + r) : __builtin_huge_val();
+            bool compact = false;
+            if constexpr (kSkipsX) compact = u_base != nullptr;
+            if (compact) {
+                const unsigned lane = __lane_id();
+                const bool own = ((static_cast<unsigned>(r) ^ lane) & 63u) == 0u;
+                const bool need_l = own && (cd & kLoadL), need_u = own && (cd & kLoadU);
+                const unsigned long long ml = __ballot(need_l), mu = __ballot(need_u);
+                const int g = r >> 6;
+                auto below = [](unsigned long long m) {
+                    return static_cast<int>(__builtin_amdgcn_mbcnt_hi(static_cast<unsigned>(m >> 32), __builtin_amdgcn_mbcnt_lo(static_cast<unsigned>(m), 0u)));
+                };
+                li = need_l ? ld(l_fin + (l_base[g] + below(ml))) : ((cd & kZeroL) ? 0.0 : -__builtin_huge_val());
+                ui = need_u ? ld(u_fin + (u_base[g] + below(mu))) : __builtin_huge_val();
+            } else {
+                li = (cd & kLoadL) ? ld(l + r) : ((cd & kZeroL) ? 0.0 : -__builtin_huge_val());
+                ui = (cd & kLoadU) ? ld(u + r) : __builtin_huge_val();
+            }
         } else {
             li = ld(l + r);
             ui = ld(u + r);
@@ -1445,7 +1489,7 @@
     return false;
 }
 
-FarPush far_push_of(const CsrDev &consumer) {
+FarPush far_push_of(const CsrDev &consumer, int tab_cap) {
     FarPush f;
     if (consumer.tiled.valid && consumer.tiled.n_groups > 0) {
         f.gptr = consumer.tiled.f_gptr;
@@ -1453,7 +1497,7 @@
         f.pos = consumer.tiled.f_pos;
         f.lcol = consumer.tiled.f_lcol;
         f.P = consumer.tiled.P;
-        if (consumer.tiled.f_rk) {
+        if (consumer.tiled.f_rk && consumer.tiled.f_maxruns <= tab_cap) {
             f.rptr = consumer.tiled.f_rptr;
             f.rk = consumer.tiled.f_rk;
             f.rp = consumer.tiled.f_rp;
@@ -1468,7 +1512,8 @@
         return launch_fused(AT, e, s, a.far_ready);
     }
     if (AT.tiled.valid) {
-        XEpi<false, true> e{{a.y_full}, a.x, a.x_hat, a.l, a.u, a.c, a.last_x, nullptr, nullptr, nullptr, a.ctrl, nullptr, 0, 0, 0, 0, a.push, a.lu_code, a.x_mode};
+        XEpi<false, true> e{{a.y_full}, a.x, a.x_hat, a.l, a.u, a.c, a.last_x, nullptr, nullptr, nullptr, a.ctrl, nullptr, 0, 0, 0, 0, a.push, a.lu_code, a.x_mode, 0.0, 0.0,
+                            a.l_fin, a.u_fin, a.l_base, a.u_base};
         return launch_fused(AT, e, s, a.far_ready);
     }
     XEpi<false> e{{a.y_full}, a.x, a.x_hat, a.l, a.u, a.c, a.last_x, nullptr, nullptr, nullptr, a.ctrl, nullptr, 0, 0, 0, 0, a.push, a.lu_code};
@@ -2200,6 +2245,67 @@
 }
 void launch_bound_codes(int n, const double *l, const double *u, unsigned char *code, hipStream_t s) {
     if (n > 0) hipLaunchKernelGGL(k_bound_codes, dim3((n + kThreads - 1) / kThreads), dim3(kThreads), 0, s, n, l, u, code);
+}
+
+__global__ void __launch_bounds__(kThreads) k_bound_counts(int n, const unsigned char *code, int *l_cnt, int *u_cnt) {
+    const int j = blockIdx.x * kThreads + threadIdx.x;
+    const unsigned cd = j < n ? code[j] : 0u;
+    const unsigned long long ml = __ballot(cd & kLoadL), mu = __ballot(cd & kLoadU);
+    if ((j & 63) == 0 && j < n) {
+        l_cnt[j >> 6] = __popcll(ml);
+        u_cnt[j >> 6] = __popcll(mu);
+    }
+    if (j == 0) l_cnt[(n + 63) >> 6] = u_cnt[(n + 63) >> 6] = 0;
+}
+constexpr int kScanThreads = 1024;
+__global__ void __launch_bounds__(kScanThreads) k_bound_scan(int n, int *a, int *b) {
+    __shared__ int wsum[kScanThreads / 64];
+    int *v = blockIdx.x ? b : a;
+    const int tid = threadIdx.x, lane = tid & 63, wave = tid >> 6;
+    int carry = 0;
+    for (int i0 = 0; i0 < n; i0 += kScanThreads) {
+        const int i = i0 + tid;
+        const int x = i < n ? v[i] : 0;
+        int inc = x;
+#pragma unroll
+        for (int off = 1; off < 64; off <<= 1) {
+            const int t = __shfl_up(inc, off, 64);
+            if (lane >= off) inc += t;
+        }
+        if (lane == 63) wsum[wave] = inc;
+        __syncthreads();
+        int before = 0, all = 0;
+#pragma unroll
+        for (int w = 0; w < kScanThreads / 64; ++w) {
+            const int sw = wsum[w];
+            if (w < wave) before += sw;
+            all += sw;
+        }
+        if (i < n) v[i] = carry + before + inc - x;
+        carry += all;
+        __syncthreads();
+    }
+}
+__global__ void __launch_bounds__(kThreads) k_bound_compact(int n, const unsigned char *code, const double *l, const double *u, const int *l_base,
+                                                           const int *u_base, double *l_fin, double *u_fin) {
+    const int j = blockIdx.x * kThreads + threadIdx.x;
+    const unsigned cd = j < n ? code[j] : 0u;
+    const unsigned long long ml = __ballot(cd & kLoadL), mu = __ballot(cd & kLoadU);
+    const unsigned long long below = (1ull << (j & 63)) - 1ull;
+    if (cd & kLoadL) l_fin[l_base[j >> 6] + __popcll(ml & below)] = l[j];
+    if (cd & kLoadU) u_fin[u_base[j >> 6] + __popcll(mu & below)] = u[j];
+}
+void launch_bound_ranks(int n, const unsigned char *code, int *l_base, int *u_base, hipStream_t s) {
+    if (n <= 0) return;
+    const int ng = (n + 63) / 64;
+    hipLaunchKernelGGL(k_bound_counts, dim3((ng * 64 + kThreads - 1) / kThreads), dim3(kThreads), 0, s, n, code, l_base, u_base);
+    hipLaunchKernelGGL(k_bound_scan, dim3(2), dim3(kScanThreads), 0, s, ng + 1, l_base, u_base);
+}
+void launch_bound_compact(int n, const unsigned char *code, const double *l, const double *u, const int *l_base, const int *u_base,
+                          double *l_fin, double *u_fin, hipStream_t s) {
+    if (n <= 0) return;
+    const int ng = (n + 63) / 64;
+    hipLaunchKernelGGL(k_bound_compact, dim3((ng * 64 + kThreads - 1) / kThreads), dim3(kThreads), 0, s, n, code, l, u, l_base, u_base, l_fin, u_fin);
 }
 
 __global__ void __launch_bounds__(kThreads) k_row_codes(int m, const double *AL, const double *AU, unsigned char *code) {
diff --git a/hpr-lp-c_amd/csrc/solver.cpp b/hpr-lp-c_amd/csrc/solver.cpp
--- a/hpr-lp-c_amd/csrc/solver.cpp
+++ b/hpr-lp-c_amd/csrc/solver.cpp
@@ -1337,6 +1337,17 @@
     hook_no_far_push = env_get("HPRLP_NO_FAR_PUSH") && env_get("HPRLP_NO_FAR_PUSH")[0] == '1';
     hook_no_bound_codes = env_get("HPRLP_NO_BOUND_CODES") != nullptr;
     hook_store_x = env_get("HPRLP_STORE_X") != nullptr;
+    hook_no_compact_bounds = env_get("HPRLP_NO_COMPACT_BOUNDS") != nullptr;
+    hook_push_runs_cap = -1;
+    if (const char *v = env_get("HPRLP_PUSH_RUNS_CAP")) hook_push_runs_cap = std::max(0, std::atoi(v));
+    if (env_get("HPRLP_NO_PUSH_RUNS")) hook_push_runs_cap = 0;
+}
+
+void Solver::drop_graphs() {
+    if (graphs.empty()) return;
+    HIP_CHECK(hipStreamSynchronize(stream));
+    for (auto &kv : graphs) (void)hipGraphExecDestroy(kv.second);
+    graphs.clear();
 }
 
 void Solver::refresh_bound_codes() {
@@ -1349,6 +1360,45 @@
         if (row_code.n != static_cast<size_t>(m_loc)) row_code.alloc(static_cast<size_t>(m_loc));
         launch_row_codes(m_loc, AL.p, AU.p, row_code.p, stream);
     }
+    refresh_compact_bounds();
+}
+
+void Solver::refresh_compact_bounds() {
+    const bool want = !hook_no_compact_bounds && !hook_no_bound_codes && !comm && !overlap_enabled && AT.view.tiled.valid &&
+                      n_loc > 0 && lu_code.n == static_cast<size_t>(n_loc);
+    if (!want) {
+        if (cb_on) drop_graphs();
+        cb_on = false;
+        return;
+    }
+    const size_t ng = (static_cast<size_t>(n_loc) + 63) / 64;
+    const void *before[4] = {l_fin.p, u_fin.p, l_base.p, u_base.p};
+    if (u_base.n != ng + 1) {
+        HIP_CHECK(hipStreamSynchronize(stream));
+        l_base.alloc(ng + 1);
+        u_base.alloc(ng + 1);
+    }
+    launch_bound_ranks(n_loc, lu_code.p, l_base.p, u_base.p, stream);
+    int cnt[2] = {0, 0};
+    HIP_CHECK(hipMemcpyAsync(&cnt[0], l_base.p + ng, sizeof(int), hipMemcpyDeviceToHost, stream));
+    HIP_CHECK(hipMemcpyAsync(&cnt[1], u_base.p + ng, sizeof(int), hipMemcpyDeviceToHost, stream));
+    HIP_CHECK(hipStreamSynchronize(stream));
+    if (!l_fin.p || static_cast<size_t>(cnt[0]) > l_fin.n) l_fin.alloc(static_cast<size_t>(cnt[0]));
+    if (!u_fin.p || static_cast<size_t>(cnt[1]) > u_fin.n) u_fin.alloc(static_cast<size_t>(cnt[1]));
+    n_l_fin = cnt[0];
+    n_u_fin = cnt[1];
+    launch_bound_compact(n_loc, lu_code.p, l.p, u.p, l_base.p, u_base.p, l_fin.p, u_fin.p, stream);
+    const void *after[4] = {l_fin.p, u_fin.p, l_base.p, u_base.p};
+    if (!cb_on || std::memcmp(before, after, sizeof before) != 0) drop_graphs();
+    cb_on = true;
+}
+
+void Solver::compact_bounds_into(XHalfArgs *xa) const {
+    if (!cb_on) return;
+    xa->l_fin = l_fin.p;
+    xa->u_fin = u_fin.p;
+    xa->l_base = l_base.p;
+    xa->u_base = u_base.p;
 }
 
 void Solver::reset_iterates() {
@@ -1418,7 +1468,11 @@
     const TiledDev &pt = producer.view.tiled;
     if (hook_no_far_push || comm || !pt.valid || pt.n_pieces > 0) return FarPush{};
     if (consumer.view.tiled.valid && consumer.view.tiled.G != pt.R) return FarPush{};
-    return far_push_of(consumer.view);
+    int tab_cap = 0;
+    if (pt.rem_cap == kPbRemCap) tab_cap = consumer.view.tiled.rem_cap == kPbRemCap ? kPbRunTabCap : 0;
+    else if (hook_push_runs_cap >= 0) tab_cap = std::min(hook_push_runs_cap, kTileRunTabCap);
+    else tab_cap = static_cast<long>(consumer.tiled.n_rem) >= 48L * consumer.view.tiled.f_nruns ? kTileRunTabCap : 0;
+    return far_push_of(consumer.view, tab_cap);
 }
 
 int Solver::x_mode_of(int i, int count) const {
@@ -1429,6 +1483,7 @@
 void Solver::launch_normal_pair(bool more_follow, hipEvent_t *ev, int x_mode) {
     XHalfArgs xa{gy.p, x.p, x_hat, l.p, u.p, c.p, last_x.p, nullptr, nullptr, nullptr, ctrl.p, nullptr, 0};
     xa.lu_code = lu_code.p;
+    compact_bounds_into(&xa);
     xa.x_mode = x_mode;
     YHalfArgs ya{gxh.p, y, AL.p, AU.p, last_y.p, nullptr, nullptr, nullptr, ctrl.p, nullptr, 0};
     ya.row_code = row_code.p;
@@ -1935,6 +1990,7 @@
     launch_finalize(f, scal.p, stream);
     const DataBcArgs bc{mb, nc, nb, prm.use_bc_scaling ? 1 : 0, scal.p, AL.p, AU.p, c.p, l.p, u.p, rc, lc, data_part.p, kReduceBlocks};
     launch_data_bc(bc, stream);
+    if (bounds) refresh_compact_bounds();
     FinalizeArgs g{};
     if (bounds) g.item[g.n++] = {data_part.p, kReduceBlocks, S_DATA_NB};
     if (c_) g.item[g.n++] = {data_part.p + kReduceBlocks, kReduceBlocks, S_DATA_NC};
diff --git a/hpr-lp-c_amd/csrc/solver.h b/hpr-lp-c_amd/csrc/solver.h
--- a/hpr-lp-c_amd/csrc/solver.h
+++ b/hpr-lp-c_amd/csrc/solver.h
@@ -98,6 +98,13 @@
     DBuf<unsigned char> row_code;
     DBuf<unsigned char> lu_code;
     void refresh_bound_codes();
+    DBuf<double> l_fin, u_fin;
+    DBuf<int> l_base, u_base;
+    bool cb_on = false;
+    int n_l_fin = 0, n_u_fin = 0;
+    void refresh_compact_bounds();
+    void compact_bounds_into(XHalfArgs *xa) const;
+    void drop_graphs();
     DBuf<double> x, last_x, z_bar, last_y, y_obj, y_temp;
     DBuf<double> gy, gxh, gxb, gyb, gxt, gsn, gsm;
     double *y = nullptr, *x_hat = nullptr, *x_bar = nullptr, *y_bar = nullptr, *x_temp = nullptr;
@@ -183,6 +190,8 @@
     hipEvent_t ev_ready = nullptr, ev_done_x = nullptr, ev_done_y = nullptr;
     std::string env_at_setup, env_ignored_at_setup;
     bool hook_no_far_push = false, hook_no_bound_codes = false, hook_store_x = false;
+    bool hook_no_compact_bounds = false;
+    int hook_push_runs_cap = -1;
     void read_hooks();
     bool overlap_enabled = false, overlap_ready = false, y_exchange_pending = false;
     bool overlap_spmv_first = false;
diff --git a/hpr-lp-c_amd/csrc/tiled.h b/hpr-lp-c_amd/csrc/tiled.h
--- a/hpr-lp-c_amd/csrc/tiled.h
+++ b/hpr-lp-c_amd/csrc/tiled.h
@@ -25,6 +25,7 @@
 constexpr int kPbRemCap = kTileThreads * kPbRemK;
 constexpr int kPbRowsMax = 4096;
 constexpr int kPbRunTabCap = 3072;
+constexpr int kTileRunTabCap = kTileCols;
 constexpr int kTileMaxRow = 1024;
 constexpr int kTileDenseMin = 256;
 static_assert(kTileRemCap % kTileRemK == 0 && kTileRemCap + (kTileThreads / 64) * 3 / 2 <= kTileCols, "tile buffer too small for the remainder scratch");
@@ -133,6 +134,7 @@
     const int *f_rk = nullptr;
     const int *f_rp = nullptr;
     int f_maxruns = 0;
+    int f_nruns = 0;
     const int4 *f_work = nullptr;
     int n_work = 0;
 };
diff --git a/hpr-lp-c_amd/csrc/tiled_build.hip b/hpr-lp-c_amd/csrc/tiled_build.hip
--- a/hpr-lp-c_amd/csrc/tiled_build.hip
+++ b/hpr-lp-c_amd/csrc/tiled_build.hip
@@ -826,8 +826,8 @@
         }
     }
     view.f_rptr = view.f_rk = view.f_rp = nullptr;
-    view.f_maxruns = 0;
-    if (view.rem_cap == kPbRemCap) {
+    view.f_maxruns = view.f_nruns = 0;
+    {
         DBuf<int> flag(static_cast<size_t>(n)), excl(static_cast<size_t>(n));
         hipLaunchKernelGGL(k_far_run_flags, dim3(grid_for(n)), dim3(kThreads), 0, s, n, kout.p, f_pos.p, flag.p);
         size_t bytes = 0;
@@ -851,11 +851,13 @@
         int h_mx = 0;
         HIP_CHECK(hipMemcpyAsync(&h_mx, mx.p, sizeof(int), hipMemcpyDeviceToHost, s));
         HIP_CHECK(hipStreamSynchronize(s));
-        if (h_mx > 0 && h_mx <= kPbRunTabCap && static_cast<long>(n) >= 48L * nruns) {
+        const bool pb = view.rem_cap == kPbRemCap;
+        if (h_mx > 0 && (pb ? h_mx <= kPbRunTabCap && static_cast<long>(n) >= 48L * nruns : h_mx <= kTileRunTabCap)) {
             view.f_rptr = f_rptr.p;
             view.f_rk = f_rk.p;
             view.f_rp = f_rp.p;
             view.f_maxruns = h_mx;
+            view.f_nruns = nruns;
         }
         if (env_get("HPRLP_TIMING"))
             std::fprintf(stderr, "[timing]   source-side run tables: %d runs of %d entries (%.1f per run), most in one group %d%s\n", nruns, n,
```
